# LanceKnight/MolKGNN

Measured on AMD Instinct MI355X. Metric: molecules/sec fwd+bwd, 3-layer MolKGNN on AID 1798, higher is better.
Workload: dtype f32; 1 GPU; AID 1798 full set shape (61832 molecules, ~25 atoms / ~53 directed edges each), 3 layers, hidden_dim 32, kernels 10/20/30/50 per degree, batch 4096 molecules per GPU (102584 atoms), 4 resident batches cycled, fwd+bwd+AdamW, one hipGraph per batch; variant=auto, batch_size_per_gpu=4096, parallelism=dp1

## Files before the change

include/molkgnn_hip.h:

```cpp
#ifndef MOLKGNN_HIP_H
#define MOLKGNN_HIP_H

#include <stddef.h>
#include <stdint.h>

#ifdef __cplusplus
extern "C" {
#endif

#define MKGNN_MAX_DEGREE 4
#define MKGNN_ABI_VERSION 8

#define MKGNN_LOSS_BCE_MEAN 0
#define MKGNN_LOSS_SQERR_MEAN 1
#define MKGNN_LOSS_SQERR_SUM 2

typedef struct mkgnn_kernel_bank {
    int32_t num_kernels;
    int32_t reserved;
    const float* x_center;
    const float* x_support;
    const float* edge_attr_support;
    const float* p_support;
    const float* support_attr_sc_weight;
// ... 14 lines not shown
    int64_t count;
    const int64_t* selected_index;
    const int64_t* nei_index;
    const float* nei_edge_attr;
    const float* p_focal;
    const float* nei_p;
    const float* nei_edge_unit;
} mkgnn_degree_bucket;

typedef struct mkgnn_saved {
    float* pair_state;
    int8_t* chirality;
} mkgnn_saved;

int mkgnn_abi_version(void);
const char* mkgnn_last_error(void);

int mkgnn_row_inv_norm(const float* x, int64_t x_stride, int64_t n_rows, int32_t F,
                       float* inv_norm, void* stream);

int mkgnn_unit_rows8(const float* in, int64_t n_rows, int32_t E, float* out, void* stream);

size_t mkgnn_workspace_bytes(const int32_t num_kernels[MKGNN_MAX_DEGREE], int32_t F, int32_t E,
                             int64_t n_atoms, int64_t n_edges);

#define MKGNN_VARIANT_BLOCK_ROWS 0x100
#define MKGNN_VARIANT_BANK_PREPARED 0x200
#define MKGNN_VARIANT_ROWS_SPLIT 0x400
int mkgnn_rows_presplit(const float* x, int64_t x_stride, int64_t n_rows, int32_t F, float* inv_norm, float* out,
                        int64_t out_stride, void* stream);
int mkgnn_bank_prepare(int32_t count, const mkgnn_kernel_bank* banks, const int32_t* F, int32_t E,
                       void* const* workspaces, const size_t* workspace_bytes, void* stream);
int mkgnn_bank_prepare_deferred(int32_t count, const mkgnn_kernel_bank* banks, const int32_t* F, int32_t E,
                                void* const* workspaces, const size_t* workspace_bytes);
int mkgnn_bank_prepare_flush(void* stream);
int mkgnn_bank_prepare_withdraw(void);
int mkgnn_touch_hint(const void* const* arrays, const size_t* bytes, int32_t count);

int mkgnn_kernelsetconv_forward(const mkgnn_kernel_bank banks[MKGNN_MAX_DEGREE],
                                const mkgnn_degree_bucket buckets[MKGNN_MAX_DEGREE],
                                const float* x, int64_t x_stride, const float* inv_norm,
                                int64_t n_atoms, int32_t F, int32_t E, int32_t is_last_layer,
                                float* out, int64_t out_stride,
                                const mkgnn_saved saved[MKGNN_MAX_DEGREE],
                                void* workspace, size_t workspace_bytes, int32_t variant, void* stream);

#define MKGNN_BACKWARD_DEFER_BANK 0x100
#define MKGNN_BACKWARD_THROUGH_NEIGHBOURS 0x200
#define MKGNN_BACKWARD_ROWS_SPLIT 0x400
int mkgnn_kernelsetconv_backward(const mkgnn_kernel_bank banks[MKGNN_MAX_DEGREE],
                                 const mkgnn_degree_bucket buckets[MKGNN_MAX_DEGREE],
                                 const float* x, int64_t x_stride, const float* inv_norm,
                                 int64_t n_atoms, int32_t F, int32_t E, int32_t is_last_layer,
                                 const float* grad_out, int64_t grad_out_stride,
                                 const mkgnn_saved saved[MKGNN_MAX_DEGREE],
                                 const int32_t* scatter_rowptr, const int32_t* scatter_rows,
                                 float* grad_x, int64_t grad_x_stride,
                                 const mkgnn_kernel_bank_grad grads[MKGNN_MAX_DEGREE],
                                 void* workspace, size_t workspace_bytes, int32_t workspace_from_forward,
                                 int32_t variant, void* stream);

int mkgnn_backward_streams(const mkgnn_kernel_bank banks[MKGNN_MAX_DEGREE],
                           const mkgnn_degree_bucket buckets[MKGNN_MAX_DEGREE],
                           const float* x, int64_t x_stride, int64_t n_atoms, int32_t F, int32_t E);

int mkgnn_rows_split_supported(const mkgnn_kernel_bank banks[MKGNN_MAX_DEGREE],
                               const mkgnn_degree_bucket buckets[MKGNN_MAX_DEGREE],
                               int64_t x_stride, int64_t out_stride, int64_t n_atoms, int32_t F, int32_t E);

int mkgnn_backward_join(void* stream);

int mkgnn_segment_sum_rows(const float* in, int64_t in_stride, const int32_t* rowptr,
                           const int32_t* col, int64_t n_rows, int32_t width,
                           float* out, int64_t out_stride, float* inv_norm, void* stream);

int mkgnn_segment_sum_block_rows(const float* in, int64_t in_stride, const int32_t* rowptr, const int32_t* col,
                                 const int8_t* degree, int64_t n_rows, const int32_t num_kernels[MKGNN_MAX_DEGREE],
                                 int32_t mode, float* out, int64_t out_stride, float* inv_norm, void* stream);

typedef struct mkgnn_readout_params {
    const float* lin1_weight;
    const float* lin1_bias;
    const float* lin2_weight;
    const float* lin2_bias;
    int32_t F, H, G;
} mkgnn_readout_params;

int32_t mkgnn_readout_hidden_stride(int32_t H);
size_t mkgnn_readout_workspace_bytes(int32_t F, int32_t H, int32_t G, int64_t n_atoms, int64_t n_mols);

int mkgnn_readout_forward(const mkgnn_readout_params* params, const float* h, int64_t h_stride,
                          int64_t n_atoms, const int32_t* mol_ptr, int64_t n_mols,
                          const float* keep_scale, float* pre, float* pooled,
                          float* out, int64_t out_stride, void* stream);

int mkgnn_readout_backward(const mkgnn_readout_params* params, const float* h, int64_t h_stride,
                           int64_t n_atoms, const int32_t* mol_ptr, const int32_t* atom_mol, int64_t n_mols,
                           const float* keep_scale, const float* pre, const float* pooled,
                           const float* grad_out, int64_t grad_out_stride,
                           float* grad_h, int64_t grad_h_stride,
                           float* grad_lin1_weight, float* grad_lin1_bias,
                           float* grad_lin2_weight, float* grad_lin2_bias,
                           void* workspace, size_t workspace_bytes, void* stream);

size_t mkgnn_readout_blocks_workspace_bytes(int32_t K, int32_t H, int32_t G, int64_t n_mols);
int mkgnn_readout_blocks_supported(int32_t F, int32_t H, int32_t G, const int32_t num_kernels[MKGNN_MAX_DEGREE]);
int mkgnn_readout_blocks_forward(const mkgnn_readout_params* params, const float* sim, int64_t sim_stride,
                                 const int32_t num_kernels[MKGNN_MAX_DEGREE],
                                 const mkgnn_degree_bucket buckets[MKGNN_MAX_DEGREE], int64_t n_atoms,
                                 const int32_t* in_rowptr, const int32_t* in_col, const int32_t* mol_ptr, int64_t n_mols,
                                 const float* keep_scale, float* z, float* pre, float* pooled, float* gate_sum,
                                 float* out, int64_t out_stride, void* stream);
int mkgnn_readout_blocks_backward(const mkgnn_readout_params* params, const float* sim, int64_t sim_stride,
                                  const int32_t num_kernels[MKGNN_MAX_DEGREE],
                                  const mkgnn_degree_bucket buckets[MKGNN_MAX_DEGREE], int64_t n_atoms,
                                  const int32_t* out_rowptr, const int32_t* out_col, const int32_t* mol_ptr,
                                  const int32_t* atom_mol, int64_t n_mols, const float* gate, const float* gate_sum,
                                  const float* pooled, const float* grad_out, int64_t grad_out_stride,
                                  float* dz, float* grad_sim, int64_t grad_sim_stride,
                                  float* grad_lin1_weight, float* grad_lin1_bias, float* grad_lin2_weight,
                                  float* grad_lin2_bias, void* workspace, size_t workspace_bytes, void* stream);

#define MKGNN_TAIL_MAX_ATOMS 128
#define MKGNN_TAIL_MAX_EDGES 512
typedef struct mkgnn_tail_args {
    const float* sim; int64_t sim_stride;
    int32_t num_kernels[MKGNN_MAX_DEGREE];
    const mkgnn_degree_bucket* buckets;
    const int32_t* in_rowptr; const int32_t* in_col;
    const int32_t* out_rowptr; const int32_t* out_col;
    const int32_t* mol_ptr; const int32_t* atom_mol;
    int64_t n_atoms, n_mols, n_loss_mols;
    mkgnn_readout_params readout;
    const float* head_weight;
    const float* head_bias;
    const float* target;
    float dropout_p;
    int64_t* rng_state; int64_t* rng_used;
    float* emb; int64_t emb_stride;
    float* pred; float* loss;
    float* grad_sim; int64_t grad_sim_stride;
    float *grad_lin1_weight, *grad_lin1_bias, *grad_lin2_weight, *grad_lin2_bias, *grad_head_weight, *grad_head_bias;
    int32_t defer_reduce;
    int32_t loss_kind;
} mkgnn_tail_args;
int mkgnn_tail_supported(int32_t K, int32_t H, int32_t G, const int32_t num_kernels[MKGNN_MAX_DEGREE]);
size_t mkgnn_tail_workspace_bytes(int32_t K, int32_t H, int32_t G, int64_t n_atoms, int64_t n_mols);
int mkgnn_tail_fused(const mkgnn_tail_args* args, void* workspace, size_t workspace_bytes, void* stream);
int mkgnn_tail_fused_readout_dropout(const mkgnn_tail_args* args, float readout_dropout_p, void* workspace, size_t workspace_bytes,
                                     void* stream);
int mkgnn_readout_dropout_mask(const int64_t* rng_pair, int64_t n_rows, int32_t H, float p, float* keep, int64_t keep_stride,
                               void* stream);
int mkgnn_tail_flush(void* stream);
size_t mkgnn_tail_score_workspace_bytes(int32_t K, int32_t H, int32_t G, int64_t n_atoms, int64_t n_mols);
int mkgnn_tail_score(const mkgnn_tail_args* args, void* workspace, size_t workspace_bytes, void* stream);

#define MKGNN_ATOM_CONTRIB_MAX_TASKS 32
typedef struct mkgnn_atom_contrib_args {
    const float* sim; int64_t sim_stride;
    int32_t num_kernels[MKGNN_MAX_DEGREE];
    const mkgnn_degree_bucket* buckets;
    const int32_t* in_rowptr; const int32_t* in_col;
    int64_t n_atoms;
    mkgnn_readout_params readout;
    const float* head_weight; int64_t head_stride; int32_t T;
    float* contrib; int64_t contrib_stride;
} mkgnn_atom_contrib_args;
size_t mkgnn_atom_contributions_workspace_bytes(int32_t K, int32_t H, int32_t G, int64_t n_atoms);
int mkgnn_atom_contributions(const mkgnn_atom_contrib_args* args, void* workspace, size_t workspace_bytes, void* stream);

#define MKGNN_BN_SPLIT_ROWS 2
size_t mkgnn_batchnorm_workspace_bytes(int32_t C);
int mkgnn_batchnorm_forward(const float* x, int64_t x_stride, int64_t n_rows, int32_t C,
                            const float* weight, const float* bias,
                            float* running_mean, float* running_var, float momentum, float eps,
                            int32_t training, float* out, int64_t out_stride,
                            float* save_mean, float* save_invstd, float* inv_norm, int64_t* num_batches_tracked,
                            const int64_t* n_valid_rows, void* workspace, size_t workspace_bytes, void* stream);
typedef struct mkgnn_bn_stats {
    const float* x; int64_t x_stride; int64_t n_rows; int32_t C;
    float* running_mean; float* running_var;
    float momentum;
    int64_t* num_batches_tracked;
    const int64_t* row_key; const int64_t* key_limit;
} mkgnn_bn_stats;
size_t mkgnn_batchnorm_stats_workspace_bytes(int32_t C);
int mkgnn_batchnorm_update_stats(const mkgnn_bn_stats* stats, void* workspace, size_t workspace_bytes, void* stream);
int mkgnn_batchnorm_forward_with_stats(const float* x, int64_t x_stride, int64_t n_rows, int32_t C,
                            const float* weight, const float* bias,
                            float* running_mean, float* running_var, float momentum, float eps,
                            int32_t training, float* out, int64_t out_stride,
                            float* save_mean, float* save_invstd, float* inv_norm, int64_t* num_batches_tracked,
                            const int64_t* n_valid_rows, void* workspace, size_t workspace_bytes,
                            const mkgnn_bn_stats* companion, void* companion_workspace, size_t companion_workspace_bytes,
                            void* stream);
int mkgnn_batchnorm_backward(const float* grad_out, int64_t grad_out_stride, const float* x, int64_t x_stride,
                             int64_t n_rows, int32_t C, const float* weight,
                             const float* save_mean, const float* save_invstd, int32_t training,
                             float* grad_x, int64_t grad_x_stride, float* grad_weight, float* grad_bias,
                             const int64_t* n_valid_rows, void* workspace, size_t workspace_bytes, void* stream);

size_t mkgnn_rf_workspace_bytes(int64_t n_atoms);
int mkgnn_rf_count(const int64_t* edge_index, int64_t n_atoms, int64_t n_edges,
                   void* workspace, size_t workspace_bytes, int64_t* counts, void* stream);
int mkgnn_rf_fill(const int64_t* edge_index, const float* p, const float* edge_attr,
                  int64_t n_atoms, int64_t n_edges, int32_t E, const void* workspace,
                  const mkgnn_degree_bucket out[MKGNN_MAX_DEGREE], void* stream);

size_t mkgnn_plan_workspace_bytes(int64_t n_atoms, int64_t n_edges, int64_t n_rows);

size_t mkgnn_index_workspace_bytes(int64_t n_atoms, int64_t n_edges, int64_t n_rows);
int mkgnn_index_build(const int64_t* edge_index, const float* p, const float* edge_attr, int64_t n_atoms, int64_t n_edges,
                      int32_t E, const mkgnn_degree_bucket out[MKGNN_MAX_DEGREE],
                      int32_t* scatter_rowptr, int32_t* scatter_rows, int32_t* in_rowptr, int32_t* in_col,
                      int32_t* in_col_packed, int32_t* out_rowptr, int32_t* out_col, int8_t* deg8, int64_t* counts,
                      void* workspace, size_t workspace_bytes, void* rf_ready_event, void* stream);

int mkgnn_expand_batch(const int32_t* bond_ij, const uint8_t* bond_attr, int64_t n_bonds, int32_t E,
                       const int32_t* mol_ptr, int64_t n_molecules, int64_t n_atoms,
                       int64_t* edge_index, float* edge_attr, int64_t* batch, int32_t* atom_molecule, void* stream);
int mkgnn_plan_build(const mkgnn_degree_bucket buckets[MKGNN_MAX_DEGREE], int64_t n_atoms, const int64_t* edge_index,
                     int64_t n_edges, int32_t* scatter_rowptr, int32_t* scatter_rows, int32_t* in_rowptr, int32_t* in_col,
                     int32_t* in_col_packed, int32_t* out_rowptr, int32_t* out_col, int8_t* deg8, void* workspace,
                     size_t workspace_bytes, void* stream);

size_t mkgnn_bce_head_workspace_bytes(int64_t n_rows, int32_t H);
int mkgnn_bce_head_forward(const float* emb, int64_t emb_stride, int64_t n_rows, int32_t H,
                           const float* weight, const float* bias, const float* target,
                           float* pred, float* loss, void* workspace, size_t workspace_bytes, void* stream);
int mkgnn_bce_head_backward(const float* emb, int64_t emb_stride, int64_t n_rows, int32_t H,
                            const float* weight, const float* target, const float* pred, const float* grad_loss,
                            float* grad_emb, int64_t grad_emb_stride, float* grad_weight, float* grad_bias,
                            void* workspace, size_t workspace_bytes, void* stream);

int mkgnn_bce_head_dropout_forward(const float* emb, int64_t emb_stride, int64_t n_rows, int32_t H,
                                   const float* weight, const float* bias, const float* target, float dropout_p,
                                   int64_t* rng_state, int64_t* rng_used, float* pred, float* loss,
                                   void* workspace, size_t workspace_bytes, void* stream);
int mkgnn_bce_head_dropout_backward(const float* emb, int64_t emb_stride, int64_t n_rows, int32_t H,
                                    const float* weight, const float* target, const float* pred,
                                    const float* grad_loss, float dropout_p, const int64_t* rng_used,
                                    float* grad_emb, int64_t grad_emb_stride, float* grad_weight, float* grad_bias,
                                    void* workspace, size_t workspace_bytes, void* stream);

int mkgnn_bce_head_fused(const float* emb, int64_t emb_stride, int64_t n_rows, int32_t H,
                         const float* weight, const float* bias, const float* target, float dropout_p,
                         int64_t* rng_state, int64_t* rng_used, float* pred, float* loss,
                         float* grad_emb, int64_t grad_emb_stride, float* grad_weight, float* grad_bias,
                         void* workspace, size_t workspace_bytes, void* stream);

int mkgnn_head_loss_forward(int32_t loss_kind, const float* emb, int64_t emb_stride, int64_t n_rows, int32_t H,
                            const float* weight, const float* bias, const float* target,
                            float* pred, float* loss, void* workspace, size_t workspace_bytes, void* stream);
int mkgnn_head_loss_backward(int32_t loss_kind, const float* emb, int64_t emb_stride, int64_t n_rows, int32_t H,
                             const float* weight, const float* target, const float* pred, const float* grad_loss,
                             float* grad_emb, int64_t grad_emb_stride, float* grad_weight, float* grad_bias,
                             void* workspace, size_t workspace_bytes, void* stream);
int mkgnn_head_loss_dropout_forward(int32_t loss_kind, const float* emb, int64_t emb_stride, int64_t n_rows, int32_t H,
                                    const float* weight, const float* bias, const float* target, float dropout_p,
                                    int64_t* rng_state, int64_t* rng_used, float* pred, float* loss,
                                    void* workspace, size_t workspace_bytes, void* stream);
int mkgnn_head_loss_dropout_backward(int32_t loss_kind, const float* emb, int64_t emb_stride, int64_t n_rows, int32_t H,
                                     const float* weight, const float* target, const float* pred,
                                     const float* grad_loss, float dropout_p, const int64_t* rng_used,
                                     float* grad_emb, int64_t grad_emb_stride, float* grad_weight, float* grad_bias,
                                     void* workspace, size_t workspace_bytes, void* stream);
int mkgnn_head_loss_fused(int32_t loss_kind, const float* emb, int64_t emb_stride, int64_t n_rows, int32_t H,
                          const float* weight, const float* bias, const float* target, float dropout_p,
                          int64_t* rng_state, int64_t* rng_used, float* pred, float* loss,
                          float* grad_emb, int64_t grad_emb_stride, float* grad_weight, float* grad_bias,
                          void* workspace, size_t workspace_bytes, void* stream);

#define MKGNN_TASK_HEAD_MAX_TASKS 32
size_t mkgnn_task_head_workspace_bytes(int64_t n_rows, int32_t H, int32_t T);
int mkgnn_task_head_forward(int32_t loss_kind, const float* emb, int64_t emb_stride, int64_t n_rows, int32_t H, int32_t T,
                            const float* weight, const float* bias, const float* target, const int32_t* task,
                            const int32_t* row_ids, int64_t n_task, float dropout_p, int64_t* rng_state, int64_t* rng_used,
                            float* pred, float* loss, void* workspace, size_t workspace_bytes, void* stream);
int mkgnn_task_head_backward(int32_t loss_kind, const float* emb, int64_t emb_stride, int64_t n_rows, int32_t H, int32_t T,
                             const float* weight, const float* target, const int32_t* task, const int32_t* row_ids,
                             int64_t n_task, const float* pred, const float* grad_loss, float dropout_p,
                             const int64_t* rng_used, float* grad_emb, int64_t grad_emb_stride, float* grad_weight,
                             float* grad_bias, void* workspace, size_t workspace_bytes, void* stream);
int mkgnn_task_head_fused(int32_t loss_kind, const float* emb, int64_t emb_stride, int64_t n_rows, int32_t H, int32_t T,
                          const float* weight, const float* bias, const float* target, const int32_t* task,
                          const int32_t* row_ids, int64_t n_task, float dropout_p, int64_t* rng_state, int64_t* rng_used,
                          float* pred, float* loss, float* grad_emb, int64_t grad_emb_stride, float* grad_weight,
                          float* grad_bias, void* workspace, size_t workspace_bytes, void* stream);

int mkgnn_task_scores(const float* emb, int64_t emb_stride, int64_t n_rows, int32_t H, int32_t T,
                      const float* weight, const float* bias, float* pred, int64_t pred_row_stride, int64_t pred_task_stride,
                      void* stream);

#define MKGNN_EMBED_COSINE_MAX_QUERIES 32
int mkgnn_embed_cosine(const float* emb, int64_t emb_stride, int64_t n_rows, int32_t H, const float* queries, int64_t query_stride,
                       int32_t Q, float* sim, int64_t sim_row_stride, int64_t sim_query_stride, void* stream);

typedef struct mkgnn_copy_item { float* dst; const float* src; int64_t numel; } mkgnn_copy_item;
int mkgnn_flat_copy(const mkgnn_copy_item* items, int32_t n_items, void* stream);

typedef struct mkgnn_adamw_tensor {
    float* param;
    const float* grad;
    float* state;
    int64_t numel;
    int32_t group;
// ... 150 lines not shown
```

molkgnn_amd/_lib.py:

```python
from __future__ import annotations

import ctypes as C
import os
from typing import Optional, Sequence

import torch

_HERE = os.path.dirname(os.path.abspath(__file__))
LIB_PATH = os.environ.get("MKGNN_LIB") or os.path.join(_HERE, "libmolkgnn_hip.so")
MAX_DEGREE = 4
ABI_VERSION = 8
LOSS_BCE_MEAN, LOSS_SQERR_MEAN, LOSS_SQERR_SUM = 0, 1, 2
TASK_HEAD_MAX_TASKS, TASK_HEAD_MAX_H = 32, 64
EMBED_COSINE_MAX_QUERIES, EMBED_COSINE_MAX_H = 32, 64
MAX_COSINE_MAX_REFS, MAX_COSINE_MAX_H = 1 << 20, 64
MAX_COSINE_ROWS, MAX_COSINE_TILE, MAX_COSINE_MAX_PARTS, MAX_COSINE_TARGET_BLOCKS = 128, 32, 256, 2048
SELECT_ROWS_PASS = 1024


def max_cosine_split(n_rows: int, R: int):
    row_blocks = -(-int(n_rows) // MAX_COSINE_ROWS)
    tiles = -(-int(R) // MAX_COSINE_TILE)
    want = min(-(-MAX_COSINE_TARGET_BLOCKS // row_blocks), tiles, MAX_COSINE_MAX_PARTS)
    per_part = -(-tiles // want)
# ... 3 lines not shown
class KernelBank(C.Structure):
    _fields_ = [("num_kernels", C.c_int32), ("reserved", C.c_int32),
                ("x_center", C.c_void_p), ("x_support", C.c_void_p),
                ("edge_attr_support", C.c_void_p), ("p_support", C.c_void_p),
                ("support_attr_sc_weight", C.c_void_p), ("center_attr_sc_weight", C.c_void_p),
                ("edge_attr_support_sc_weight", C.c_void_p)]


class KernelBankGrad(C.Structure):
    _fields_ = [("x_center", C.c_void_p), ("x_support", C.c_void_p), ("edge_attr_support", C.c_void_p),
                ("support_attr_sc_weight", C.c_void_p), ("center_attr_sc_weight", C.c_void_p),
                ("edge_attr_support_sc_weight", C.c_void_p)]


class DegreeBucket(C.Structure):
    _fields_ = [("count", C.c_int64), ("selected_index", C.c_void_p), ("nei_index", C.c_void_p),
                ("nei_edge_attr", C.c_void_p), ("p_focal", C.c_void_p), ("nei_p", C.c_void_p), ("nei_edge_unit", C.c_void_p)]


class Saved(C.Structure):
    _fields_ = [("pair_state", C.c_void_p), ("chirality", C.c_void_p)]


class ReadoutParams(C.Structure):
    _fields_ = [("lin1_weight", C.c_void_p), ("lin1_bias", C.c_void_p), ("lin2_weight", C.c_void_p),
                ("lin2_bias", C.c_void_p), ("F", C.c_int32), ("H", C.c_int32), ("G", C.c_int32)]


class TailArgs(C.Structure):
    _fields_ = [("sim", C.c_void_p), ("sim_stride", C.c_int64), ("num_kernels", C.c_int32 * 4), ("buckets", C.c_void_p),
                ("in_rowptr", C.c_void_p), ("in_col", C.c_void_p), ("out_rowptr", C.c_void_p), ("out_col", C.c_void_p),
                ("mol_ptr", C.c_void_p), ("atom_mol", C.c_void_p), ("n_atoms", C.c_int64), ("n_mols", C.c_int64),
                ("n_loss_mols", C.c_int64), ("readout", ReadoutParams), ("head_weight", C.c_void_p), ("head_bias", C.c_void_p),
                ("target", C.c_void_p), ("dropout_p", C.c_float), ("rng_state", C.c_void_p), ("rng_used", C.c_void_p),
                ("emb", C.c_void_p), ("emb_stride", C.c_int64), ("pred", C.c_void_p), ("loss", C.c_void_p),
                ("grad_sim", C.c_void_p), ("grad_sim_stride", C.c_int64), ("grad_lin1_weight", C.c_void_p),
                ("grad_lin1_bias", C.c_void_p), ("grad_lin2_weight", C.c_void_p), ("grad_lin2_bias", C.c_void_p),
                ("grad_head_weight", C.c_void_p), ("grad_head_bias", C.c_void_p), ("defer_reduce", C.c_int32),
                ("loss_kind", C.c_int32)]


TAIL_MAX_ATOMS, TAIL_MAX_EDGES = 128, 512
ATOM_CONTRIB_MAX_TASKS = 32


class AtomContribArgs(C.Structure):
    _fields_ = [("sim", C.c_void_p), ("sim_stride", C.c_int64), ("num_kernels", C.c_int32 * 4), ("buckets", C.c_void_p),
                ("in_rowptr", C.c_void_p), ("in_col", C.c_void_p), ("n_atoms", C.c_int64), ("readout", ReadoutParams),
                ("head_weight", C.c_void_p), ("head_stride", C.c_int64), ("T", C.c_int32), ("contrib", C.c_void_p),
                ("contrib_stride", C.c_int64)]


class CopyItem(C.Structure):
    _fields_ = [("dst", C.c_void_p), ("src", C.c_void_p), ("numel", C.c_int64)]


class AdamWTensor(C.Structure):
    _fields_ = [("param", C.c_void_p), ("grad", C.c_void_p), ("state", C.c_void_p), ("numel", C.c_int64),
                ("group", C.c_int32), ("reserved", C.c_int32), ("active", C.c_void_p)]


class AdamWGroup(C.Structure):
    _fields_ = [("lr_device", C.c_void_p), ("lr", C.c_float), ("beta1", C.c_float), ("beta2", C.c_float),
                ("eps", C.c_float), ("weight_decay", C.c_float), ("maximize", C.c_int32), ("grad_scale", C.c_float)]


class ShardView(C.Structure):
    _fields_ = [("x", C.c_void_p), ("p", C.c_void_p), ("edge_src", C.c_void_p), ("edge_dst", C.c_void_p),
                ("edge_attr", C.c_void_p), ("y", C.c_void_p), ("mol_atom_ptr", C.c_void_p), ("mol_edge_ptr", C.c_void_p),
                ("mol_deg_ptr", C.c_void_p), ("n_molecules", C.c_int64), ("x_dim", C.c_int32), ("p_dim", C.c_int32),
                ("e_dim", C.c_int32), ("reserved", C.c_int32)]


class ResidentShardView(C.Structure):
    _fields_ = [("x", C.c_void_p), ("p", C.c_void_p), ("bond_ij", C.c_void_p), ("bond_attr", C.c_void_p), ("y", C.c_void_p),
                ("mol_atom_ptr", C.c_void_p), ("mol_bond_ptr", C.c_void_p), ("mol_deg", C.c_void_p), ("n_molecules", C.c_int64),
                ("x_dim", C.c_int32), ("p_dim", C.c_int32), ("e_dim", C.c_int32), ("reserved", C.c_int32)]


class ResidentShardPackedView(C.Structure):
    _fields_ = [("x_rec", C.c_void_p), ("x_col", C.c_void_p), ("p", C.c_void_p), ("bond_ij", C.c_void_p), ("bond_attr", C.c_void_p),
                ("y", C.c_void_p), ("mol_atom_ptr", C.c_void_p), ("mol_bond_ptr", C.c_void_p), ("mol_deg", C.c_void_p),
                ("n_molecules", C.c_int64), ("x_dim", C.c_int32), ("p_dim", C.c_int32), ("e_dim", C.c_int32), ("rec_bytes", C.c_int32)]


PACKED_MAX_X_DIM = 160
TOPK_MAX_K = 1024
GATHER_BAD_ID, GATHER_MISFIT = 1, 2
Int64x6 = C.c_int64 * 6
Banks4 = KernelBank * MAX_DEGREE
BankGrads4 = KernelBankGrad * MAX_DEGREE
Buckets4 = DegreeBucket * MAX_DEGREE
Saved4 = Saved * MAX_DEGREE
Int32x4 = C.c_int32 * MAX_DEGREE

MOLECULE_MAX_LAYERS = 4
MOLECULE_MAX_ATOMS = 64
MOLECULE_MAX_MOLS = 16
MOLECULE_HEAD, MOLECULE_BACKWARD, MOLECULE_GRAD_EMB, MOLECULE_SQERR, MOLECULE_SUM = 1, 2, 4, 8, 16
MOLECULE_READOUT_DROPOUT = 32


class MoleculeLayer(C.Structure):
    _fields_ = [("bank", Banks4), ("grad", BankGrads4), ("saved", Saved4), ("F", C.c_int32), ("reserved", C.c_int32),
                ("sim_out", C.c_void_p), ("sim_stride", C.c_int64)]


class BnStats(C.Structure):
    _fields_ = [("x", C.c_void_p), ("x_stride", C.c_int64), ("n_rows", C.c_int64), ("C", C.c_int32),
                ("running_mean", C.c_void_p), ("running_var", C.c_void_p), ("momentum", C.c_float),
                ("num_batches_tracked", C.c_void_p), ("row_key", C.c_void_p), ("key_limit", C.c_void_p)]


class MoleculeNet(C.Structure):
    _fields_ = [("num_layers", C.c_int32), ("E", C.c_int32), ("layer", MoleculeLayer * MOLECULE_MAX_LAYERS),
                ("bn_weight", C.c_void_p), ("bn_bias", C.c_void_p), ("bn_running_mean", C.c_void_p),
                ("bn_running_var", C.c_void_p), ("bn_num_batches_tracked", C.c_void_p),
                ("bn_eps", C.c_float), ("bn_momentum", C.c_float), ("bn_training", C.c_int32), ("reserved", C.c_int32),
                ("grad_bn_weight", C.c_void_p), ("grad_bn_bias", C.c_void_p),
                ("readout", ReadoutParams),
                ("grad_lin1_weight", C.c_void_p), ("grad_lin1_bias", C.c_void_p), ("grad_lin2_weight", C.c_void_p),
                ("grad_lin2_bias", C.c_void_p),
                ("ffn_weight", C.c_void_p), ("ffn_bias", C.c_void_p), ("grad_ffn_weight", C.c_void_p),
                ("grad_ffn_bias", C.c_void_p), ("head_dropout", C.c_float), ("readout_dropout", C.c_float),
                ("rng_state", C.c_void_p), ("rng_used", C.c_void_p), ("edge_stats", C.POINTER(BnStats))]


class MoleculeBatch(C.Structure):
    _fields_ = [("n_atoms", C.c_int64), ("n_mols", C.c_int64), ("n_chunks", C.c_int64), ("max_chunk_atoms", C.c_int64),
                ("chunk_mol_ptr", C.c_void_p), ("mol_atom_ptr", C.c_void_p), ("atom_degree", C.c_void_p),
                ("atom_rank", C.c_void_p), ("buckets", Buckets4), ("x", C.c_void_p), ("x_stride", C.c_int64)]


EXPORTS = ("mkgnn_abi_version", "mkgnn_last_error", "mkgnn_row_inv_norm", "mkgnn_unit_rows8", "mkgnn_workspace_bytes",
           "mkgnn_kernelsetconv_forward", "mkgnn_kernelsetconv_backward", "mkgnn_segment_sum_rows",
           "mkgnn_readout_hidden_stride", "mkgnn_readout_workspace_bytes", "mkgnn_readout_forward",
           "mkgnn_readout_backward", "mkgnn_batchnorm_workspace_bytes", "mkgnn_batchnorm_forward",
           "mkgnn_batchnorm_backward", "mkgnn_bce_head_workspace_bytes", "mkgnn_bce_head_forward",
           "mkgnn_bce_head_backward", "mkgnn_rf_workspace_bytes", "mkgnn_rf_count", "mkgnn_rf_fill", "mkgnn_adamw_step", "mkgnn_adamw_state_floats",
           "mkgnn_bce_head_dropout_forward", "mkgnn_bce_head_dropout_backward", "mkgnn_segment_sum_block_rows",
           "mkgnn_plan_workspace_bytes", "mkgnn_plan_build", "mkgnn_backward_join", "mkgnn_backward_streams", "mkgnn_bank_prepare", "mkgnn_bank_prepare_deferred", "mkgnn_bank_prepare_flush", "mkgnn_bank_prepare_withdraw", "mkgnn_touch_hint", "mkgnn_expand_batch", "mkgnn_bce_head_fused", "mkgnn_collate_compact", "mkgnn_collate_compact_bytes",
           "mkgnn_readout_blocks_supported", "mkgnn_readout_blocks_forward", "mkgnn_readout_blocks_backward",
           "mkgnn_readout_blocks_workspace_bytes", "mkgnn_molecule_supported", "mkgnn_molecule_workspace_bytes",
           "mkgnn_molecule_step", "mkgnn_batchnorm_stats_workspace_bytes", "mkgnn_batchnorm_update_stats",
           "mkgnn_batchnorm_forward_with_stats", "mkgnn_index_workspace_bytes", "mkgnn_index_build",
           "mkgnn_rows_split_supported", "mkgnn_rows_presplit", "mkgnn_tail_supported", "mkgnn_tail_workspace_bytes", "mkgnn_tail_fused", "mkgnn_tail_flush", "mkgnn_flat_copy",
           "mkgnn_tail_fused_readout_dropout", "mkgnn_readout_dropout_mask", "mkgnn_tail_score", "mkgnn_tail_score_workspace_bytes",
           "mkgnn_head_loss_forward", "mkgnn_head_loss_backward", "mkgnn_head_loss_dropout_forward",
           "mkgnn_head_loss_dropout_backward", "mkgnn_head_loss_fused", "mkgnn_gather_compact",
           "mkgnn_gather_compact_workspace_bytes", "mkgnn_gather_compact_packed", "mkgnn_topk_update", "mkgnn_topk_workspace_bytes",
           "mkgnn_task_head_workspace_bytes", "mkgnn_task_head_forward", "mkgnn_task_head_backward", "mkgnn_task_head_fused",
           "mkgnn_task_scores", "mkgnn_topk_tasks_workspace_bytes", "mkgnn_topk_update_tasks", "mkgnn_embed_cosine",
           "mkgnn_atom_contributions", "mkgnn_atom_contributions_workspace_bytes", "mkgnn_embed_max_cosine",
           "mkgnn_embed_max_cosine_workspace_bytes", "mkgnn_select_rows")

_lib: Optional[C.CDLL] = None
TORCH_LIB_PATH = os.path.join(os.path.dirname(LIB_PATH), "libmolkgnn_torch.so")
_torch_ops_loaded = False


def load_torch_ops():
    global _torch_ops_loaded
    import torch
    if not _torch_ops_loaded:
        load()
        if not os.path.exists(TORCH_LIB_PATH):
            raise MolKGNNLibraryError(f"{TORCH_LIB_PATH} is missing: build it with `make -C molkgnn_amd/csrc torch`")
        torch.ops.load_library(TORCH_LIB_PATH)
        if int(torch.ops.molkgnn.abi_version()) != ABI_VERSION:
            raise MolKGNNLibraryError("libmolkgnn_torch.so was built against another ABI version")
        _torch_ops_loaded = True
    return torch.ops.molkgnn


class MolKGNNLibraryError(RuntimeError):
    pass


def load() -> C.CDLL:
    global _lib
    if _lib is not None:
        return _lib
    if not os.path.exists(LIB_PATH):
        raise MolKGNNLibraryError(
            f"{LIB_PATH} is missing: build it with `make -C molkgnn_amd/csrc` "
            "(python -c 'import __graft_entry__ as g; g.build()'). There is no fallback path.")
    lib = C.CDLL(LIB_PATH)
    for name in EXPORTS:
        if not hasattr(lib, name):
            raise MolKGNNLibraryError(f"{LIB_PATH} does not export {name}")
    lib.mkgnn_abi_version.restype = C.c_int
    lib.mkgnn_last_error.restype = C.c_char_p
    lib.mkgnn_row_inv_norm.restype = C.c_int
    lib.mkgnn_row_inv_norm.argtypes = [C.c_void_p, C.c_int64, C.c_int64, C.c_int32, C.c_void_p, C.c_void_p]
    lib.mkgnn_unit_rows8.restype = C.c_int
    lib.mkgnn_unit_rows8.argtypes = [C.c_void_p, C.c_int64, C.c_int32, C.c_void_p, C.c_void_p]
    lib.mkgnn_workspace_bytes.restype = C.c_size_t
    lib.mkgnn_workspace_bytes.argtypes = [Int32x4, C.c_int32, C.c_int32, C.c_int64, C.c_int64]
    lib.mkgnn_kernelsetconv_forward.restype = C.c_int
    lib.mkgnn_kernelsetconv_forward.argtypes = [
        Banks4, Buckets4, C.c_void_p, C.c_int64, C.c_void_p, C.c_int64, C.c_int32, C.c_int32, C.c_int32,
        C.c_void_p, C.c_int64, Saved4, C.c_void_p, C.c_size_t, C.c_int32, C.c_void_p]
    lib.mkgnn_kernelsetconv_backward.restype = C.c_int
    lib.mkgnn_kernelsetconv_backward.argtypes = [
        Banks4, Buckets4, C.c_void_p, C.c_int64, C.c_void_p, C.c_int64, C.c_int32, C.c_int32, C.c_int32,
        C.c_void_p, C.c_int64, Saved4, C.c_void_p, C.c_void_p, C.c_void_p, C.c_int64, BankGrads4,
        C.c_void_p, C.c_size_t, C.c_int32, C.c_int32, C.c_void_p]
    lib.mkgnn_backward_streams.restype = C.c_int
    lib.mkgnn_backward_streams.argtypes = [Banks4, Buckets4, C.c_void_p, C.c_int64, C.c_int64, C.c_int32, C.c_int32]
    lib.mkgnn_tail_supported.restype = C.c_int
    lib.mkgnn_tail_supported.argtypes = [C.c_int32, C.c_int32, C.c_int32, Int32x4]
    lib.mkgnn_tail_workspace_bytes.restype = C.c_size_t
    lib.mkgnn_tail_workspace_bytes.argtypes = [C.c_int32, C.c_int32, C.c_int32, C.c_int64, C.c_int64]
    lib.mkgnn_tail_fused.restype = C.c_int
    lib.mkgnn_tail_fused.argtypes = [C.POINTER(TailArgs), C.c_void_p, C.c_size_t, C.c_void_p]
    lib.mkgnn_tail_score_workspace_bytes.restype = C.c_size_t
    lib.mkgnn_tail_score_workspace_bytes.argtypes = [C.c_int32, C.c_int32, C.c_int32, C.c_int64, C.c_int64]
    lib.mkgnn_tail_score.restype = C.c_int
    lib.mkgnn_tail_score.argtypes = [C.POINTER(TailArgs), C.c_void_p, C.c_size_t, C.c_void_p]
    lib.mkgnn_atom_contributions_workspace_bytes.restype = C.c_size_t
    lib.mkgnn_atom_contributions_workspace_bytes.argtypes = [C.c_int32, C.c_int32, C.c_int32, C.c_int64]
    lib.mkgnn_atom_contributions.restype = C.c_int
    lib.mkgnn_atom_contributions.argtypes = [C.POINTER(AtomContribArgs), C.c_void_p, C.c_size_t, C.c_void_p]
    lib.mkgnn_tail_fused_readout_dropout.restype = C.c_int
    lib.mkgnn_tail_fused_readout_dropout.argtypes = [C.POINTER(TailArgs), C.c_float, C.c_void_p, C.c_size_t, C.c_void_p]
    lib.mkgnn_readout_dropout_mask.restype = C.c_int
    lib.mkgnn_readout_dropout_mask.argtypes = [C.c_void_p, C.c_int64, C.c_int32, C.c_float, C.c_void_p, C.c_int64, C.c_void_p]
    lib.mkgnn_flat_copy.restype = C.c_int
    lib.mkgnn_flat_copy.argtypes = [C.c_void_p, C.c_int32, C.c_void_p]
    lib.mkgnn_tail_flush.restype = C.c_int
    lib.mkgnn_tail_flush.argtypes = [C.c_void_p]
    lib.mkgnn_rows_presplit.restype = C.c_int
    lib.mkgnn_rows_presplit.argtypes = [C.c_void_p, C.c_int64, C.c_int64, C.c_int32, C.c_void_p, C.c_void_p, C.c_int64, C.c_void_p]
    lib.mkgnn_rows_split_supported.restype = C.c_int
    lib.mkgnn_rows_split_supported.argtypes = [Banks4, Buckets4, C.c_int64, C.c_int64, C.c_int64, C.c_int32, C.c_int32]
    lib.mkgnn_bank_prepare.restype = C.c_int
    lib.mkgnn_bank_prepare.argtypes = [C.c_int32, C.c_void_p, C.c_void_p, C.c_int32, C.c_void_p, C.c_void_p, C.c_void_p]
    lib.mkgnn_bank_prepare_deferred.restype = C.c_int
    lib.mkgnn_bank_prepare_deferred.argtypes = [C.c_int32, C.c_void_p, C.c_void_p, C.c_int32, C.c_void_p, C.c_void_p]
    lib.mkgnn_bank_prepare_flush.restype = C.c_int
    lib.mkgnn_bank_prepare_flush.argtypes = [C.c_void_p]
    lib.mkgnn_bank_prepare_withdraw.restype = C.c_int
    lib.mkgnn_bank_prepare_withdraw.argtypes = []
    lib.mkgnn_touch_hint.restype = C.c_int
    lib.mkgnn_touch_hint.argtypes = [C.c_void_p, C.c_void_p, C.c_int32]
    lib.mkgnn_collate_compact_bytes.restype = C.c_size_t
    lib.mkgnn_collate_compact_bytes.argtypes = [Int64x6, C.c_int64, C.c_int32, C.c_int32, C.c_int32, C.c_int32]
    lib.mkgnn_collate_compact.restype = C.c_int
    lib.mkgnn_collate_compact.argtypes = [C.POINTER(ShardView), C.c_int64, C.c_int64, Int64x6, C.c_int32, C.c_void_p, C.c_size_t]
    lib.mkgnn_gather_compact_workspace_bytes.restype = C.c_size_t
    lib.mkgnn_gather_compact_workspace_bytes.argtypes = [C.c_int64]
    lib.mkgnn_gather_compact.restype = C.c_int
    lib.mkgnn_gather_compact.argtypes = [C.POINTER(ResidentShardView), C.c_void_p, C.c_int64, Int64x6, C.c_int32, C.c_void_p,
                                         C.c_size_t, C.c_void_p, C.c_void_p]
    lib.mkgnn_gather_compact_packed.restype = C.c_int
    lib.mkgnn_gather_compact_packed.argtypes = [C.POINTER(ResidentShardPackedView), C.c_void_p, C.c_int64, Int64x6, C.c_int32,
                                                C.c_void_p, C.c_size_t, C.c_void_p, C.c_void_p]
    lib.mkgnn_topk_workspace_bytes.restype = C.c_size_t
    lib.mkgnn_topk_workspace_bytes.argtypes = [C.c_int32, C.c_int32]
    lib.mkgnn_topk_update.restype = C.c_int
    lib.mkgnn_topk_update.argtypes = [C.c_void_p, C.c_void_p, C.c_int32, C.c_void_p, C.c_void_p, C.c_int32, C.c_void_p, C.c_void_p,
                                      C.c_void_p, C.c_void_p, C.c_size_t, C.c_void_p]
    lib.mkgnn_topk_tasks_workspace_bytes.restype = C.c_size_t
    lib.mkgnn_topk_tasks_workspace_bytes.argtypes = [C.c_int32, C.c_int32, C.c_int32]
    lib.mkgnn_topk_update_tasks.restype = C.c_int
    lib.mkgnn_topk_update_tasks.argtypes = [C.c_void_p, C.c_int64, C.c_int64, C.c_void_p, C.c_int32, C.c_int32, C.c_void_p, C.c_void_p,
                                            C.c_int32, C.c_void_p, C.c_void_p, C.c_void_p, C.c_void_p, C.c_size_t, C.c_void_p]
    lib.mkgnn_expand_batch.restype = C.c_int
    lib.mkgnn_expand_batch.argtypes = [C.c_void_p, C.c_void_p, C.c_int64, C.c_int32, C.c_void_p, C.c_int64, C.c_int64,
                                       C.c_void_p, C.c_void_p, C.c_void_p, C.c_void_p, C.c_void_p]
    lib.mkgnn_backward_join.restype = C.c_int
    lib.mkgnn_backward_join.argtypes = [C.c_void_p]
    lib.mkgnn_segment_sum_rows.restype = C.c_int
    lib.mkgnn_segment_sum_rows.argtypes = [C.c_void_p, C.c_int64, C.c_void_p, C.c_void_p, C.c_int64, C.c_int32,
                                           C.c_void_p, C.c_int64, C.c_void_p, C.c_void_p]
    P, I64, I32, F32 = C.c_void_p, C.c_int64, C.c_int32, C.c_float
    lib.mkgnn_readout_hidden_stride.restype = I32
    lib.mkgnn_readout_hidden_stride.argtypes = [I32]
    lib.mkgnn_readout_workspace_bytes.restype = C.c_size_t
    lib.mkgnn_readout_workspace_bytes.argtypes = [I32, I32, I32, I64, I64]
    lib.mkgnn_readout_forward.restype = C.c_int
    lib.mkgnn_readout_forward.argtypes = [C.POINTER(ReadoutParams), P, I64, I64, P, I64, P, P, P, P, I64, P]
    lib.mkgnn_readout_backward.restype = C.c_int
    lib.mkgnn_readout_backward.argtypes = [C.POINTER(ReadoutParams), P, I64, I64, P, P, I64, P, P, P, P, I64, P, I64,
                                           P, P, P, P, P, C.c_size_t, P]
    lib.mkgnn_readout_blocks_workspace_bytes.restype = C.c_size_t
    lib.mkgnn_readout_blocks_workspace_bytes.argtypes = [I32, I32, I32, I64]
    lib.mkgnn_readout_blocks_supported.restype = C.c_int
    lib.mkgnn_readout_blocks_supported.argtypes = [I32, I32, I32, Int32x4]
    lib.mkgnn_readout_blocks_forward.restype = C.c_int
    lib.mkgnn_readout_blocks_forward.argtypes = [C.POINTER(ReadoutParams), P, I64, Int32x4, Buckets4, I64, P, P, P, I64, P, P, P, P, P, P, I64, P]
    lib.mkgnn_readout_blocks_backward.restype = C.c_int
    lib.mkgnn_readout_blocks_backward.argtypes = [C.POINTER(ReadoutParams), P, I64, Int32x4, Buckets4, I64, P, P, P, P, I64, P, P, P,
                                                  P, I64, P, P, I64, P, P, P, P, P, C.c_size_t, P]
    lib.mkgnn_batchnorm_workspace_bytes.restype = C.c_size_t
    lib.mkgnn_batchnorm_workspace_bytes.argtypes = [I32]
    lib.mkgnn_batchnorm_forward.restype = C.c_int
    lib.mkgnn_batchnorm_forward.argtypes = [P, I64, I64, I32, P, P, P, P, F32, F32, I32, P, I64, P, P, P, P, P, P, C.c_size_t, P]
    lib.mkgnn_batchnorm_stats_workspace_bytes.restype = C.c_size_t
    lib.mkgnn_batchnorm_stats_workspace_bytes.argtypes = [I32]
    lib.mkgnn_batchnorm_update_stats.restype = C.c_int
    lib.mkgnn_batchnorm_update_stats.argtypes = [C.POINTER(BnStats), P, C.c_size_t, P]
    lib.mkgnn_batchnorm_forward_with_stats.restype = C.c_int
    lib.mkgnn_batchnorm_forward_with_stats.argtypes = [P, I64, I64, I32, P, P, P, P, F32, F32, I32, P, I64, P, P, P, P, P, P, C.c_size_t,
                                                       C.POINTER(BnStats), P, C.c_size_t, P]
    lib.mkgnn_batchnorm_backward.restype = C.c_int
    lib.mkgnn_batchnorm_backward.argtypes = [P, I64, P, I64, I64, I32, P, P, P, I32, P, I64, P, P, P, P, C.c_size_t, P]
    lib.mkgnn_bce_head_forward.restype = C.c_int
    lib.mkgnn_bce_head_forward.argtypes = [P, I64, I64, I32, P, P, P, P, P, P, C.c_size_t, P]
    lib.mkgnn_bce_head_backward.restype = C.c_int
    lib.mkgnn_bce_head_backward.argtypes = [P, I64, I64, I32, P, P, P, P, P, I64, P, P, P, C.c_size_t, P]
    lib.mkgnn_bce_head_dropout_forward.restype = C.c_int
    lib.mkgnn_bce_head_dropout_forward.argtypes = [P, I64, I64, I32, P, P, P, C.c_float, P, P, P, P, P, C.c_size_t, P]
    lib.mkgnn_bce_head_dropout_backward.restype = C.c_int
    lib.mkgnn_bce_head_dropout_backward.argtypes = [P, I64, I64, I32, P, P, P, P, C.c_float, P, P, I64, P, P, P, C.c_size_t, P]
    lib.mkgnn_bce_head_fused.restype = C.c_int
    lib.mkgnn_bce_head_fused.argtypes = [P, I64, I64, I32, P, P, P, C.c_float, P, P, P, P, P, I64, P, P, P, C.c_size_t, P]
    for name, args in (("mkgnn_head_loss_forward", lib.mkgnn_bce_head_forward.argtypes),
                       ("mkgnn_head_loss_backward", lib.mkgnn_bce_head_backward.argtypes),
                       ("mkgnn_head_loss_dropout_forward", lib.mkgnn_bce_head_dropout_forward.argtypes),
                       ("mkgnn_head_loss_dropout_backward", lib.mkgnn_bce_head_dropout_backward.argtypes),
                       ("mkgnn_head_loss_fused", lib.mkgnn_bce_head_fused.argtypes)):
        getattr(lib, name).restype = C.c_int
        getattr(lib, name).argtypes = [I32] + list(args)
    lib.mkgnn_bce_head_workspace_bytes.restype = C.c_size_t
    lib.mkgnn_bce_head_workspace_bytes.argtypes = [I64, I32]
    lib.mkgnn_task_head_workspace_bytes.restype = C.c_size_t
    lib.mkgnn_task_head_workspace_bytes.argtypes = [I64, I32, I32]
    lib.mkgnn_task_head_forward.restype = C.c_int
    lib.mkgnn_task_head_forward.argtypes = [I32, P, I64, I64, I32, I32, P, P, P, P, P, I64, C.c_float, P, P, P, P, P, C.c_size_t, P]
    lib.mkgnn_task_head_backward.restype = C.c_int
    lib.mkgnn_task_head_backward.argtypes = [I32, P, I64, I64, I32, I32, P, P, P, P, I64, P, P, C.c_float, P, P, I64, P, P, P,
                                             C.c_size_t, P]
    lib.mkgnn_task_head_fused.restype = C.c_int
    lib.mkgnn_task_head_fused.argtypes = [I32, P, I64, I64, I32, I32, P, P, P, P, P, I64, C.c_float, P, P, P, P, P, I64, P, P, P,
                                          C.c_size_t, P]
    lib.mkgnn_task_scores.restype = C.c_int
    lib.mkgnn_task_scores.argtypes = [P, I64, I64, I32, I32, P, P, P, I64, I64, P]
    lib.mkgnn_embed_cosine.restype = C.c_int
    lib.mkgnn_embed_cosine.argtypes = [P, I64, I64, I32, P, I64, I32, P, I64, I64, P]
    lib.mkgnn_embed_max_cosine_workspace_bytes.restype = C.c_size_t
    lib.mkgnn_embed_max_cosine_workspace_bytes.argtypes = [I64, I32]
    lib.mkgnn_embed_max_cosine.restype = C.c_int
    lib.mkgnn_embed_max_cosine.argtypes = [P, I64, I64, I32, P, I64, I32, P, P, P, C.c_size_t, P]
    lib.mkgnn_select_rows.restype = C.c_int
    lib.mkgnn_select_rows.argtypes = [P, P, P, I32, P, P, P, P, P, P]
    lib.mkgnn_rf_workspace_bytes.restype = C.c_size_t
    lib.mkgnn_rf_workspace_bytes.argtypes = [I64]
    lib.mkgnn_rf_count.restype = C.c_int
    lib.mkgnn_rf_count.argtypes = [P, I64, I64, P, C.c_size_t, P, P]
    lib.mkgnn_rf_fill.restype = C.c_int
    lib.mkgnn_rf_fill.argtypes = [P, P, P, I64, I64, I32, P, Buckets4, P]
    lib.mkgnn_segment_sum_block_rows.restype = C.c_int
    lib.mkgnn_segment_sum_block_rows.argtypes = [P, I64, P, P, P, I64, Int32x4, I32, P, I64, P, P]
    lib.mkgnn_plan_workspace_bytes.restype = C.c_size_t
    lib.mkgnn_plan_workspace_bytes.argtypes = [I64, I64, I64]
    lib.mkgnn_plan_build.restype = C.c_int
    lib.mkgnn_plan_build.argtypes = [Buckets4, I64, P, I64, P, P, P, P, P, P, P, P, P, C.c_size_t, P]
    lib.mkgnn_index_workspace_bytes.restype = C.c_size_t
    lib.mkgnn_index_workspace_bytes.argtypes = [I64, I64, I64]
    lib.mkgnn_index_build.restype = C.c_int
    lib.mkgnn_index_build.argtypes = [P, P, P, I64, I64, I32, Buckets4, P, P, P, P, P, P, P, P, P, P, C.c_size_t, P, P]
    lib.mkgnn_adamw_step.restype = C.c_int
    lib.mkgnn_adamw_state_floats.restype = C.c_int64
    lib.mkgnn_adamw_state_floats.argtypes = [I64]
    lib.mkgnn_adamw_step.argtypes = [P, I32, P, I32, P]
    lib.mkgnn_molecule_supported.restype = C.c_int
    lib.mkgnn_molecule_supported.argtypes = [C.POINTER(MoleculeNet), I32]
    lib.mkgnn_molecule_workspace_bytes.restype = C.c_size_t
    lib.mkgnn_molecule_workspace_bytes.argtypes = [C.POINTER(MoleculeNet), I32, I64, I64]
    lib.mkgnn_molecule_step.restype = C.c_int
    lib.mkgnn_molecule_step.argtypes = [C.POINTER(MoleculeNet), C.POINTER(MoleculeBatch), I32, P, P, P, P, P, P, C.c_size_t, P]
    if lib.mkgnn_abi_version() != ABI_VERSION:
        raise MolKGNNLibraryError(f"ABI version {lib.mkgnn_abi_version()} != {ABI_VERSION}: rebuild the library")
    _lib = lib
    return lib


def check(rc: int, what: str) -> None:
    if rc != 0:
        msg = load().mkgnn_last_error()
        raise MolKGNNLibraryError(f"{what}: {msg.decode() if msg else 'error'}")


# ... 13 lines not shown
```

molkgnn_amd/csrc/kgnn_bwd_stream.hip:

```cpp
#include <stdio.h>
#include <stdlib.h>
#include <string.h>

#include <type_traits>

#include "kgnn_launch.h"
#include "kgnn_split.h"

namespace mkgnn {

typedef float f32x4 __attribute__((ext_vector_type(4)));

#ifdef MKGNN_BWD_STAMPS
__device__ unsigned long long* g_bank_stream_stamps = nullptr;
#define MKGNN_BPHASE(i) do { __builtin_amdgcn_sched_barrier(0); const unsigned long long t_ = __builtin_readcyclecounter(); phase[i] += t_ - t_phase; t_phase = t_; __builtin_amdgcn_sched_barrier(0); } while (0)
#else
#define MKGNN_BPHASE(i) do { } while (0)
#endif

namespace bs {

template <int I> using IC = std::integral_constant<int, I>;
template <int B, int E, typename Fn> __device__ __forceinline__ void static_for(Fn&& fn) {
    if constexpr (B < E) { fn(IC<B>{}); static_for<B + 1, E>(fn); }
}
template <int N> __device__ __forceinline__ void wait_vmcnt() {
    static_assert(N >= 0 && N <= 63, "s_waitcnt vmcnt is a 6-bit field");
    asm volatile("s_waitcnt vmcnt(%0)" ::"n"(N) : "memory");
}
#define MKGNN_DMA_CASE(SZ, O) else if constexpr (OFF == O) __builtin_amdgcn_global_load_lds(g, l, SZ, O, 0)
template <int OFF> __device__ __forceinline__ void dma16(const void* src, float* lds_wave_base) {
    const auto g = (const __attribute__((address_space(1))) void*)((const char*)src - OFF);
    const auto l = (__attribute__((address_space(3))) void*)((char*)lds_wave_base - OFF);
    if constexpr (OFF == 0) __builtin_amdgcn_global_load_lds(g, l, 16, 0, 0);
    MKGNN_DMA_CASE(16, 16); MKGNN_DMA_CASE(16, 32); MKGNN_DMA_CASE(16, 48);
    else static_assert(OFF < 0, "add the offset to the list");
}
template <int OFF> __device__ __forceinline__ void dma4(const void* src, float* lds_wave_base) {
    const auto g = (const __attribute__((address_space(1))) void*)((const char*)src - OFF);
    const auto l = (__attribute__((address_space(3))) void*)((char*)lds_wave_base - OFF);
    if constexpr (OFF == 0) __builtin_amdgcn_global_load_lds(g, l, 4, 0, 0);
    MKGNN_DMA_CASE(4, 4); MKGNN_DMA_CASE(4, 8); MKGNN_DMA_CASE(4, 12);
    else static_assert(OFF < 0, "add the offset to the list");
}
constexpr int SITE_ROWS = 0, SITE_BONDS = 16, SITE_COEF_G = 32, SITE_COEF_I = 48;
constexpr int SITE_IDS = 0, SITE_IDS4 = 4, SITE_INV = 8, SITE_INV4 = 12;
__device__ __forceinline__ float lds_read_raw(uint32_t byte_addr) {
    float v;
    asm volatile("ds_read_b32 %0, %1" : "=v"(v) : "v"(byte_addr) : "memory");
    return v;
}
template <int OFF> __device__ __forceinline__ float lds_read_raw_at(uint32_t byte_addr) {
    static_assert(OFF >= 0 && OFF < 65536, "ds_read offset field");
    float v;
    asm volatile("ds_read_b32 %0, %1 offset:%2" : "=v"(v) : "v"(byte_addr), "n"(OFF) : "memory");
    return v;
}

template <int OFF> __device__ __forceinline__ void lds_read_h16(uint32_t& dst, uint32_t byte_addr) {
    static_assert(OFF >= 0 && OFF < 65536, "ds_read offset field");
    asm volatile("ds_read_u16 %0, %1 offset:%2" : "=v"(dst) : "v"(byte_addr), "n"(OFF) : "memory");
}

template <typename V> __device__ __forceinline__ void lds_fence(V& v) { asm volatile("s_waitcnt lgkmcnt(0)" : "+v"(v) : : "memory"); }

template <int D, int A> __device__ __forceinline__ int perm_entry(int p) {
    if constexpr (D == 1) return 0;
    else {
        constexpr uint32_t packed = [] {
            uint32_t v = 0;
            for (int q = 0; q < PermC<D>::P; ++q) v |= (uint32_t)PermC<D>::t[q][A] << (2 * q);
            return v;
        }();
        return (int)((packed >> (2 * p)) & 3u);
    }
}

template <int D> struct Traits {
    static constexpr int NS = (D == 1) ? 1 : (D == 4 ? 4 : 2);
    static constexpr int NSTREAM = 4 / NS;
    static constexpr int RING = (D == 1) ? 2 : (D == 2 ? 3 : (D == 3 ? 4 : 5));
    static constexpr int S1 = D + 1;
    static constexpr int OFF_INV = 16 * S1, OFF_BOND = 32 * S1, META = OFF_BOND + 128 * D;
    static constexpr int COEF = 512;
};

__host__ __device__ constexpr int lds_floats(int D, int KC) {
    const int NS = (D == 1) ? 1 : (D == 4 ? 4 : 2);
    const int RING = (D == 1) ? 2 : (D == 2 ? 3 : (D == 3 ? 4 : 5));
    const int META = 32 * (D + 1) + 128 * D;
    const int FPC = 4 * KC;
    return (4 / NS) * (RING * 16 * FPC * 4 + 2 * META) + 4 * 512;
}

template <int KC, int NS> constexpr int pieces_of(int role) { return (KC - role + NS - 1) / NS; }

template <int D, int KC> constexpr int batch_size(int sd, int role) {
    using T = Traits<D>;
    int n = pieces_of<KC, T::NS>(role);
    if (sd == 0) n += 2;
    if (role == 0) {
        if (sd < D) n += 1;
        if (sd == 0) n += 2 * (T::S1 == 5 ? 2 : 1);
    }
    return n;
}
template <int D, int KC> constexpr int young_batches(int s, int role) {
    using T = Traits<D>;
    int n = 0;
    for (int j = 1; j <= T::RING - 2; ++j) n += batch_size<D, KC>((s + 64 * T::S1 - j + T::RING) % T::S1, role);
    return n;
}

}

typedef unsigned short pk_u16 __attribute__((ext_vector_type(2)));
#ifndef MKGNN_PREP_RPB
#define MKGNN_PREP_RPB 4
#endif
constexpr int PREP_RPB = MKGNN_PREP_RPB;
template <int NSRC, bool CH>
__device__ __forceinline__ void coef_prepare_body(const BankStreamArgs& a, const int di) {
    const BankStreamDeg& g = a.deg[di];
    const int tid = threadIdx.x;
    const int64_t blk = (int64_t)blockIdx.x - g.prep_blk0;
    const int64_t nrec = ((g.n + 15) / 16) * g.nct;
    const int atom = tid >> 4, k = tid & 15;
    const float w_s = g.mix[0], w_c = g.mix[1], w_e = g.mix[2], w_sum = g.mix[3];
    const int8_t* chp = g.chir ? g.chir : (const int8_t*)g.pair;
    float gv[PREP_RPB], S[PREP_RPB], C[PREP_RPB], Ed[PREP_RPB];
    int idx[PREP_RPB], ch[PREP_RPB];
    bool ok[PREP_RPB];
    const int D = di + 1;
    constexpr int nsrc = NSRC;
    int64_t src[PREP_RPB][NSRC];
#pragma unroll
    for (int r = 0; r < PREP_RPB; ++r) {
        const int64_t rec = blk * PREP_RPB + r;
        const int64_t rc = rec < nrec ? rec : nrec - 1;
        const int64_t tile = rc / g.nct;
        const int ct = (int)(rc - tile * g.nct);
        const int64_t n = tile * 16 + atom;
        const int64_t nc = n < g.n ? n : g.n - 1;
        const int l = ct * g.kpt + k;
        ok[r] = rec < nrec && n < g.n && k < g.kpt && l < g.L;
#pragma unroll
        for (int s = 0; s < NSRC; ++s) src[r][s] = a.through_nei ? g.nei[nc * D + s] : g.sel[nc];
    }
#pragma unroll
    for (int r = 0; r < PREP_RPB; ++r) {
        const int64_t rec = blk * PREP_RPB + r;
        const int64_t rc = rec < nrec ? rec : nrec - 1;
        const int64_t tile = rc / g.nct;
        const int ct = (int)(rc - tile * g.nct);
        const int64_t n = tile * 16 + atom;
        const int64_t nc = n < g.n ? n : g.n - 1;
        const int l = ct * g.kpt + k, lc = l < g.L ? l : g.L - 1;
        const size_t o = (size_t)nc * g.L + lc;
        float gs4[NSRC];
#pragma unroll
        for (int s = 0; s < NSRC; ++s) gs4[s] = a.gout[src[r][s] * a.gs + g.off + lc];
        gv[r] = gs4[0];
#pragma unroll
        for (int s = 1; s < NSRC; ++s) gv[r] += gs4[s];
        const mkgnn_f32x4 pr = pair_load(g.pair, o);
        idx[r] = pair_index(pr);
        ch[r] = CH ? (int)chp[o] : 1;
        S[r] = pr[0]; C[r] = pr[1]; Ed[r] = pr[2];
    }
    float p0 = 0.f, p1 = 0.f, p2 = 0.f;
    constexpr int NEM = (PREP_RPB + 1) / 2;
    pk_u16 em[NEM];
#pragma unroll
    for (int i = 0; i < NEM; ++i) em[i] = pk_u16{0, 0};
#pragma unroll
    for (int r = 0; r < PREP_RPB; ++r) {
        const int64_t rec = blk * PREP_RPB + r;
        float gg = ok[r] ? (CH ? gv[r] * (float)ch[r] : gv[r]) : 0.f;
        if (rec < nrec) {
            float* out = g.coefq + (size_t)rec * 512;
            out[tid] = gg;
        }
        const unsigned short eb = (unsigned short)((__float_as_uint(gg) >> 23) & 0xffu);
        em[r >> 1][r & 1] = eb;
        if (ok[r]) {
            const float sc = (S[r] * w_s + C[r] * w_c + Ed[r] * w_e) / w_sum;
            p0 = fmaf(gg * (w_s / w_sum), S[r] - sc, p0);
            p1 = fmaf(gg * (w_c / w_sum), C[r] - sc, p1);
            p2 = fmaf(gg * (w_e / w_sum), Ed[r] - sc, p2);
        }
    }
    __shared__ float red[3][4];
    __shared__ uint32_t emx[NEM][4][16];
    p0 = wave_sum(p0); p1 = wave_sum(p1); p2 = wave_sum(p2);
#pragma unroll
    for (int o = 32; o >= 16; o >>= 1)
#pragma unroll
        for (int i = 0; i < NEM; ++i)
            em[i] = __builtin_elementwise_max(em[i], __builtin_bit_cast(pk_u16, __shfl_xor(__builtin_bit_cast(uint32_t, em[i]), o, 64)));
    if ((tid & 63) == 0) { red[0][tid >> 6] = p0; red[1][tid >> 6] = p1; red[2][tid >> 6] = p2; }
    if ((tid & 63) < 16) {
#pragma unroll
        for (int i = 0; i < NEM; ++i) emx[i][tid >> 6][tid & 15] = __builtin_bit_cast(uint32_t, em[i]);
    }
    __syncthreads();
    {
        pk_u16 mx[NEM];
#pragma unroll
        for (int i = 0; i < NEM; ++i) {
            mx[i] = __builtin_bit_cast(pk_u16, emx[i][0][k]);
#pragma unroll
            for (int w = 1; w < 4; ++w) mx[i] = __builtin_elementwise_max(mx[i], __builtin_bit_cast(pk_u16, emx[i][w][k]));
        }
#pragma unroll
        for (int r = 0; r < PREP_RPB; ++r) {
            const int64_t rec = blk * PREP_RPB + r;
            const int me = mx[r >> 1][r & 1];
            if (rec < nrec) ((int*)(g.coefq + (size_t)rec * 512))[256 + tid] = (ok[r] ? idx[r] : 0) | (me << 8);
        }
    }
    if (tid < 3) g.theta_slab[(size_t)blk * 4 + tid] = (red[tid][0] + red[tid][1]) + (red[tid][2] + red[tid][3]);
}

__global__ void __launch_bounds__(256) coef_prepare_kernel(BankStreamArgs a) {
    int di = 0;
#pragma unroll
    for (int k = 1; k < 4; ++k) if (a.deg[k].prep_blocks > 0 && (int)blockIdx.x >= a.deg[k].prep_blk0) di = k;
    const int nsrc = a.through_nei ? di + 1 : 1;
    if (a.deg[di].chir) {
        switch (nsrc) {
            case 1: coef_prepare_body<1, true>(a, di); break;
            case 2: coef_prepare_body<2, true>(a, di); break;
            case 3: coef_prepare_body<3, true>(a, di); break;
            default: coef_prepare_body<4, true>(a, di); break;
        }
        return;
    }
    switch (nsrc) {
        case 1: coef_prepare_body<1, false>(a, di); break;
        case 2: coef_prepare_body<2, false>(a, di); break;
        case 3: coef_prepare_body<3, false>(a, di); break;
        default: coef_prepare_body<4, false>(a, di); break;
    }
}

constexpr int BANK_COEF_EXP = 18;
template <int D, int KC, int SP>
__device__ __forceinline__ void bank_stream_body(const BankStreamArgs& a, const BankStreamDeg& dg, const int cp, const int rank,
                                                 const int count, float* lds) {
    using namespace bs;
    using T = Traits<D>;
    constexpr int NS = T::NS, NSTREAM = T::NSTREAM, RING = T::RING, S1 = T::S1, META = T::META;
    constexpr int FPC = 4 * KC;
    constexpr bool SWZ = (KC % 2 == 0);
    constexpr int RF = 4 * FPC;
    constexpr int SLOT = 16 * RF;
    constexpr int NP = SLOT / 256;
    static_assert(NP == KC, "piece count");
    constexpr bool HS = (D == 4);
    constexpr int NBS = HS ? 2 : D;
    const int tid = threadIdx.x, lane = tid & 63;
    const int wave = __builtin_amdgcn_readfirstlane(tid >> 6);
    const int stream = wave / NS, role = wave % NS;
    const int half = HS ? (role & 1) : 0;
    const int ct = HS ? cp * 2 + (role >> 1) : cp * NS + role;
    const bool ct_ok = ct < dg.nct;
    const int ctc = ct_ok ? ct : dg.nct - 1;
    const int ci = lane & 15, kq = lane >> 4;
    const int L = dg.L, kpt = dg.kpt;
    float* const ring = lds + (size_t)stream * (RING * SLOT + 2 * META);
    float* const meta = ring + RING * SLOT;
    float* const cbuf = lds + (size_t)NSTREAM * (RING * SLOT + 2 * META) + (size_t)wave * T::COEF;

    const int64_t ntiles = (dg.n + 15) / 16;
    const int64_t nstreams = (int64_t)count * NSTREAM;
    const int64_t sg = (int64_t)rank * NSTREAM + stream;
    const int64_t tile_first = sg * ntiles / nstreams;
    const int64_t tile_end = (sg + 1) * ntiles / nstreams;
    const int64_t iters = (ntiles + nstreams - 1) / nstreams;
    const int64_t tile_hi = (tile_end > tile_first ? tile_end : (tile_first + 1 < ntiles ? tile_first + 1 : ntiles)) - 1;
    auto tile_at = [&](int64_t i) -> int64_t {
        const int64_t t = tile_first + i;
        return t > tile_hi ? tile_hi : t;
    };
    const float w_s = dg.mix[0], w_c = dg.mix[1], w_e = dg.mix[2], w_sum = dg.mix[3];
    const float ws_n = w_s / w_sum / (float)D, wc_n = w_c / w_sum, we_n = w_e / w_sum / (float)D;
    const uint32_t xs = (uint32_t)a.xs;
    const int F = a.F;

    auto issue_rows = [&](auto sdc, const float* drec, float* buf) {
        constexpr int sd = decltype(sdc)::value;
        const uint32_t ids_b = (uint32_t)(uintptr_t)(drec + 16 * sd);
        static_for<0, NS>([&](auto rc) {
            constexpr int r = decltype(rc)::value;
            constexpr int NMINE = pieces_of<KC, NS>(r);
            if constexpr (NMINE > 0) if (role == r) {
                uint32_t id[NMINE];
                int cc[NMINE];
                static_for<0, NMINE>([&](auto kc) {
                    constexpr int k = decltype(kc)::value;
                    const int g = 64 * (r + NS * k) + lane;
                    const int row = g / FPC;
                    int c = g - row * FPC;
                    if constexpr (SWZ) c ^= (row & 1) * 4;
                    cc[k] = c;
                    id[k] = __float_as_uint(lds_read_raw(ids_b + 4u * row));
                });
                static_for<0, NMINE>([&](auto kc) { lds_fence(id[decltype(kc)::value]); });
                static_for<0, NMINE>([&](auto kc) {
                    constexpr int k = decltype(kc)::value;
                    dma16<SITE_ROWS>(a.x + (id[k] * xs + (4 * cc[k] < F ? 4u * cc[k] : 0u)), buf + (r + NS * k) * 256);
                });
            }
        });
    };
    auto issue_bonds = [&](int64_t t, int sd, float* mrec) {
        if (lane < 32) {
            int64_t n = t * 16 + (lane >> 1);
            if (n >= dg.n) n = dg.n - 1;
            dma16<SITE_BONDS>(dg.e_unit + ((uint32_t)(n * D + sd) * 8u + 4u * (lane & 1)), mrec + T::OFF_BOND + sd * 128);
        }
    };
    auto issue_ids = [&](int64_t t, float* mrec) {
        int64_t n = t * 16 + ci;
        if (n >= dg.n) n = dg.n - 1;
        const void* src = (kq < D) ? (const void*)(dg.nei + n * D + kq) : (const void*)(dg.sel + n);
        if (S1 >= 4 || kq < S1) dma4<SITE_IDS>(src, mrec);
        if constexpr (S1 == 5) {
            if (kq == 0) dma4<SITE_IDS4>(dg.sel + n, mrec + 64);
        }
    };
    auto issue_inv = [&](float* mrec) {
        const uint32_t rec_b = (uint32_t)(uintptr_t)mrec;
        uint32_t idq = __float_as_uint(lds_read_raw(rec_b + 4u * (16 * ((S1 >= 4 || kq < S1) ? kq : 0) + ci)));
        [[maybe_unused]] uint32_t id4 = 0;
        if constexpr (S1 == 5) id4 = __float_as_uint(lds_read_raw(rec_b + 4u * (64 + ci)));
        lds_fence(idq);
        if constexpr (S1 == 5) lds_fence(id4);
        if (S1 >= 4 || kq < S1) dma4<SITE_INV>(a.inv + idq, mrec + T::OFF_INV);
        if constexpr (S1 == 5) {
            if (kq == 0) dma4<SITE_INV4>(a.inv + id4, mrec + T::OFF_INV + 64);
        }
    };
    auto issue_coef = [&](int64_t t, float* cb) {
        const float* src = dg.coefq + ((size_t)(t * dg.nct + ctc) * 512 + 4 * lane);
        dma16<SITE_COEF_G>(src, cb);
        dma16<SITE_COEF_I>(src + 256, cb + 256);
    };

    f32x4 acc[NBS][KC];
    f32x4 accC[KC];
    f32x4 accE[NBS];
#pragma unroll
    for (int t = 0; t < KC; ++t) {
        accC[t] = f32x4{0.f, 0.f, 0.f, 0.f};
#pragma unroll
        for (int b = 0; b < NBS; ++b) acc[b][t] = f32x4{0.f, 0.f, 0.f, 0.f};
    }
#pragma unroll
    for (int b = 0; b < NBS; ++b) accE[b] = f32x4{0.f, 0.f, 0.f, 0.f};

    [[maybe_unused]] float G = __uint_as_float(230u << 23);
    [[maybe_unused]] const int wexp = (int)((__float_as_uint(fmaxf(fabsf(ws_n), fabsf(wc_n))) >> 23) & 0xffu) + 1 - 127;

    if (role == 0) issue_ids(tile_at(0), meta);
    wait_vmcnt<0>();
    __syncthreads();
    static_for<0, RING>([&](auto kc) {
        constexpr int k = decltype(kc)::value;
        issue_rows(kc, meta, ring + k * SLOT);
        if (role == 0 && k < D) issue_bonds(tile_at(0), k, meta);
    });
    issue_coef(tile_at(0), cbuf);
    if (role == 0) {
        issue_inv(meta);
        issue_ids(tile_at(1), meta + META);
    }
    wait_vmcnt<0>();
    __builtin_amdgcn_s_barrier();

    int buf = 0;
#ifdef MKGNN_BWD_STAMPS
    const unsigned long long t_start = __builtin_readcyclecounter();
    unsigned long long phase[8] = {0, 0, 0, 0, 0, 0, 0, 0}, t_phase = t_start;
#endif
    for (int64_t it = 0; it < iters; ++it) {
        const bool real = tile_first + it < tile_end;
        const uint32_t mrec_b = (uint32_t)(uintptr_t)(meta + (it & 1) * META);
        const uint32_t cb_b = (uint32_t)(uintptr_t)cbuf;
        float gq[4];
        int iq[4];
        [[maybe_unused]] int rec_exp = 0;
        {
            float raw[8];
            const uint32_t cl_b = cb_b + 4u * (kq * 16 + ci);
            static_for<0, 4>([&](auto qc) {
// ... 127 lines not shown
                        xb.lo = __builtin_bit_cast(h16x4, u32x2{hx[4] | (hx[5] << 16), hx[6] | (hx[7] << 16)});
                        if constexpr (s < D) {
#pragma unroll
                            for (int b = 0; b < NBS; ++b) acc[b][t] = __builtin_amdgcn_mfma_f32_16x16x16f16(avs[b].lo, xb.hi, acc[b][t], 0, 0, 0);
#pragma unroll
                            for (int b = 0; b < NBS; ++b) acc[b][t] = __builtin_amdgcn_mfma_f32_16x16x16f16(avs[b].hi, xb.lo, acc[b][t], 0, 0, 0);
#pragma unroll
                            for (int b = 0; b < NBS; ++b) acc[b][t] = __builtin_amdgcn_mfma_f32_16x16x16f16(avs[b].hi, xb.hi, acc[b][t], 0, 0, 0);
                        } else {
                            accC[t] = split_mfma(avs[0], xb, accC[t]);
                        }
                    });
                } else if constexpr (SP) {
                    float bxp[2][4];
                    read_bx(IC<0>{}, bxp[0]);
                    static_for<0, KC>([&](auto tc) {
                        constexpr int t = decltype(tc)::value;
                        float (&bx)[4] = bxp[t & 1];
                        asm volatile("s_waitcnt lgkmcnt(0)" : "+v"(bx[0]), "+v"(bx[1]), "+v"(bx[2]), "+v"(bx[3]) : : "memory");
                        if constexpr (t + 1 < KC) read_bx(IC<t + 1>{}, bxp[(t + 1) & 1]);
                        const SplitReg xb = split_scaled(f32x4{bx[0], bx[1], bx[2], bx[3]}, rsc);
                        if constexpr (s < D) {
#pragma unroll
                            for (int b = 0; b < NBS; ++b) acc[b][t] = __builtin_amdgcn_mfma_f32_16x16x16f16(avs[b].lo, xb.hi, acc[b][t], 0, 0, 0);
#pragma unroll
                            for (int b = 0; b < NBS; ++b) acc[b][t] = __builtin_amdgcn_mfma_f32_16x16x16f16(avs[b].hi, xb.lo, acc[b][t], 0, 0, 0);
#pragma unroll
                            for (int b = 0; b < NBS; ++b) acc[b][t] = __builtin_amdgcn_mfma_f32_16x16x16f16(avs[b].hi, xb.hi, acc[b][t], 0, 0, 0);
                        } else {
                            accC[t] = split_mfma(avs[0], xb, accC[t]);
                        }
                    });
                } else {
                    static_for<0, KC>([&](auto tc) {
                        constexpr int t = decltype(tc)::value;
                        float bx[4];
                        read_bx(tc, bx);
                        asm volatile("s_waitcnt lgkmcnt(0)" : "+v"(bx[0]), "+v"(bx[1]), "+v"(bx[2]), "+v"(bx[3]) : : "memory");
                        if constexpr (s < D) {
#pragma unroll
                            for (int b = 0; b < NBS; ++b)
#pragma unroll
                                for (int q = 0; q < 4; ++q) acc[b][t] = __builtin_amdgcn_mfma_f32_16x16x4f32(av[b][q], bx[q], acc[b][t], 0, 0, 0);
                        } else {
#pragma unroll
                            for (int q = 0; q < 4; ++q) accC[t] = __builtin_amdgcn_mfma_f32_16x16x4f32(ac[q], bx[q], accC[t], 0, 0, 0);
                        }
                    });
                }
            }
            MKGNN_BPHASE(2);
            if constexpr (RING == 2) {
                wait_vmcnt<0>();
            } else {
                static_for<0, NS>([&](auto rc) {
                    constexpr int r = decltype(rc)::value;
                    constexpr int n_young = young_batches<D, KC>(s, r);
                    if (role == r) wait_vmcnt<n_young>();
                });
            }
            MKGNN_BPHASE(3);
            if constexpr (NS > 1) __builtin_amdgcn_s_barrier();
            MKGNN_BPHASE(4);
            constexpr int sd = (s + RING) % S1;
            const int64_t itd = it + (s + RING) / S1;
            float* const drec = meta + (itd & 1) * META;
            issue_rows(IC<sd>{}, drec, ring + buf * SLOT);
            if constexpr (sd == 0) issue_coef(tile_at(itd), cbuf);
            if (role == 0) {
                if constexpr (sd < D) issue_bonds(tile_at(itd), sd, drec);
                if constexpr (sd == 0) {
                    issue_inv(drec);
                    issue_ids(tile_at(itd + 1), meta + ((itd + 1) & 1) * META);
                }
            }
            buf = (buf + 1 == RING) ? 0 : buf + 1;
            MKGNN_BPHASE(5);
        });
    }
    wait_vmcnt<0>();
    MKGNN_BPHASE(3);

    if constexpr (SP) {
        const float ug_col = split_unscale_of<0>(G);
        float ug[4];
#pragma unroll
        for (int r = 0; r < 4; ++r) ug[r] = __shfl(ug_col, 4 * kq + r, 64);
#pragma unroll
        for (int t = 0; t < KC; ++t)
#pragma unroll
            for (int r = 0; r < 4; ++r) {
                accC[t][r] *= ug[r];
#pragma unroll
                for (int b = 0; b < NBS; ++b) acc[b][t][r] *= ug[r];
            }
    }
    float* const slab = dg.slab + (size_t)sg * bank_floats(D, L, F, a.E);
    const size_t o_sup = (size_t)L * F, o_edg = o_sup + (size_t)L * D * F;
#pragma unroll
    for (int r = 0; r < 4; ++r) {
        const int i = kq * 4 + r, l = ct * kpt + i;
        if (ct_ok && i < kpt && l < L) {
#pragma unroll
            for (int t = 0; t < KC; ++t) {
                const int f = 16 * t + ci;
                if (f < F) {
                    if (!HS || half == 0) slab[(size_t)l * F + f] = accC[t][r];
#pragma unroll
                    for (int b = 0; b < NBS; ++b) slab[o_sup + (size_t)(l * D + (HS ? 2 * half + b : b)) * F + f] = acc[b][t][r];
                }
            }
            if (ci < a.E) {
#pragma unroll
                for (int b = 0; b < NBS; ++b) slab[o_edg + (size_t)(l * D + (HS ? 2 * half + b : b)) * a.E + ci] = accE[b][r];
            }
        }
    }
#ifdef MKGNN_BWD_STAMPS
    MKGNN_BPHASE(6);
    if (g_bank_stream_stamps && lane == 0) {
        unsigned long long* o = g_bank_stream_stamps + ((size_t)blockIdx.x * 4 + wave) * 16;
        o[0] = t_start; o[1] = __builtin_readcyclecounter(); o[2] = (unsigned long long)(D * 16 + cp); o[3] = (unsigned long long)iters;
        for (int i = 0; i < 8; ++i) o[4 + i] = phase[i];
    }
#endif
}

template <int KC, int SP = 0>
__global__ void __launch_bounds__(256, (KC >= 8 ? 1 : 2)) kc_backward_bank_stream(BankStreamArgs a) {
    extern __shared__ __align__(16) float lds[];
    const int grp = a.blk_group[blockIdx.x];
    const int rank = a.blk_rank[blockIdx.x];
    const int di = a.grp_degree[grp];
    const int cp = a.grp_cp[grp];
    const int count = a.grp_count[grp];
    switch (di) {
        case 0: bank_stream_body<1, KC, SP>(a, a.deg[0], cp, rank, count, lds); break;
        case 1: bank_stream_body<2, KC, SP>(a, a.deg[1], cp, rank, count, lds); break;
        case 2: bank_stream_body<3, KC, SP>(a, a.deg[2], cp, rank, count, lds); break;
        default: bank_stream_body<4, KC, SP>(a, a.deg[3], cp, rank, count, lds); break;
    }
}

extern "C" int mkgnn_debug_set_bank_stream_stamps(void* device_ptr) {
#ifdef MKGNN_BWD_STAMPS
    return (int)hipMemcpyToSymbol(HIP_SYMBOL(g_bank_stream_stamps), &device_ptr, sizeof(void*));
#else
    (void)device_ptr;
    return -1;
#endif
}

bool bank_stream_rows_split_supported(int F) { return (F + 15) / 16 <= 7 && bwd_split_mode() != 0; }
bool bank_stream_supported(int d, int F, int E, int L, int64_t n_atoms, int64_t x_stride, const float* e_unit) {
    return stream_forward_supported(d, F, E, L, n_atoms, x_stride, x_stride, e_unit);
}

void plan_backward_bank_stream(const BwdArgs a4[4], const bool use[4], const float* const e_unit[4], float* const coefq[4],
                               int nchunk_out[4], int ntheta_out[4], bool through_nei, BankStreamLaunch* out) {
    BankStreamArgs& a = out->a;
    memset(out, 0, sizeof(*out));
    int KC = 0, ng = 0, prep_blocks = 0;
    constexpr int MG = FUSED_MAX_GROUPS;
    double cost[MG];
    int64_t tiles_of[MG], cap[MG];
    int nstream_of[MG], deg_of[MG];
    size_t lds_fl = 0;
    for (int i = 0; i < 4; ++i) {
        nchunk_out[i] = 0; ntheta_out[i] = 0;
        if (!use[i]) continue;
        const BwdArgs& s = a4[i];
        const int d = i + 1;
        a.x = s.x; a.xs = s.xs; a.inv = s.inv; a.gout = s.gout; a.gs = s.gs; a.F = s.F; a.E = s.E;
        a.through_nei = through_nei ? 1 : 0;
        KC = (s.F + 15) / 16;
        BankStreamDeg& g = a.deg[i];
        g.sel = s.sel; g.nei = s.nei; g.e_unit = e_unit[i]; g.pair = s.pair; g.chir = s.chir; g.mix = s.mix;
        g.coefq = coefq[i]; g.slab = s.slab; g.theta_slab = s.theta_slab;
        g.n = s.n; g.L = s.L; g.off = s.off;
        g.nct = (s.L + 15) / 16;
        g.kpt = (s.L + g.nct - 1) / g.nct;
        g.cs = stream_column_parts(d, s.L);
        const int64_t ntiles = (s.n + 15) / 16;
        g.prep_blk0 = prep_blocks;
        g.prep_blocks = (int)((ntiles * g.nct + PREP_RPB - 1) / PREP_RPB);
        prep_blocks += g.prep_blocks;
        ntheta_out[i] = g.prep_blocks;
        const int nstream = d == 1 ? 4 : (d == 4 ? 1 : 2);
        const size_t fl = (size_t)bs::lds_floats(d, KC);
        if (fl > lds_fl) lds_fl = fl;
        for (int cp = 0; cp < g.cs; ++cp) {
            const int nbs = d == 4 ? 2 : d;
            cost[ng] = (d * nbs + 1) * 4.0 * KC + 4.0 * d * nbs + 12.0 * d + 60.0;
            if (KC <= 7 && bwd_split_mode() != 0) {
                static const double sp7[4] = {196.0, 317.0, 503.0, 535.0}, sp2[4] = {126.0, 193.0, 298.0, 338.0};
                cost[ng] = sp2[i] + (sp7[i] - sp2[i]) * (KC - 2) / 5.0;
            }
            tiles_of[ng] = ntiles;
            cap[ng] = (ntiles + nstream - 1) / nstream;
            nstream_of[ng] = nstream;
            deg_of[ng] = i;
            a.grp_degree[ng] = (uint8_t)i;
            a.grp_cp[ng] = (uint8_t)cp;
            ++ng;
        }
    }
    if (ng == 0) return;
    auto finish = [&](int g, int blocks) {
        const int64_t streams = (int64_t)blocks * nstream_of[g];
        return 40.0 + (double)((tiles_of[g] + streams - 1) / streams) * cost[g];
    };
    int count[MG], nb = 0;
    for (int g = 0; g < ng; ++g) { count[g] = 1; ++nb; }
    auto parts_of = [&](int g) {
        int n = 0;
        for (int h = 0; h < ng; ++h) if (deg_of[h] == deg_of[g]) ++n;
        return n;
    };
    const int env_blocks = switches().bank_stream_blocks;
    const int max_blocks = grid_cap(g_grid_caps.bank, env_blocks > 8 && env_blocks <= FUSED_MAX_BLOCKS ? env_blocks : 320);
    while (nb < max_blocks) {
        int worst = -1;
        double t_worst = -1.0;
        for (int g = 0; g < ng; ++g) {
            if (count[g] >= cap[g] || (int64_t)(count[g] + 1) * nstream_of[g] > SLAB_CHUNKS) continue;
            const double t = finish(g, count[g]);
            if (t > t_worst) { t_worst = t; worst = g; }
        }
        if (worst < 0) break;
        const int np = parts_of(worst);
        if (nb + np > max_blocks) break;
        for (int h = 0; h < ng; ++h) if (deg_of[h] == deg_of[worst]) ++count[h];
        nb += np;
    }
    int given[MG] = {};
    for (int b = 0; b < nb; ++b) {
        int pick = -1;
        double best = -1e30;
        for (int g = 0; g < ng; ++g) {
            if (given[g] >= count[g]) continue;
            const double lag = (double)count[g] * (b + 1) / nb - given[g];
            if (lag > best) { best = lag; pick = g; }
        }
        a.blk_group[b] = (uint8_t)pick;
        ++given[pick];
    }
    {
        int per_xcd[MG][8] = {};
        for (int b = 0; b < nb; ++b) ++per_xcd[a.blk_group[b]][b & 7];
        int next[MG][8];
        for (int g = 0; g < ng; ++g) {
            int run = 0;
            for (int x = 0; x < 8; ++x) { next[g][x] = run; run += per_xcd[g][x]; }
        }
        for (int b = 0; b < nb; ++b) a.blk_rank[b] = (uint16_t)next[a.blk_group[b]][b & 7]++;
    }
    for (int g = 0; g < ng; ++g) {
        a.grp_count[g] = (uint16_t)count[g];
        nchunk_out[deg_of[g]] = count[g] * nstream_of[g];
    }
    note_plan(2, nb, ng, tiles_of, count, nstream_of);
    out->nb = nb; out->prep_blocks = prep_blocks; out->KC = KC; out->lds_bytes = lds_fl * 4;
}

hipError_t launch_coef_prepare(const BankStreamLaunch& p, hipStream_t st) {
    if (p.prep_blocks == 0) return hipSuccess;
    coef_prepare_kernel<<<p.prep_blocks, 256, 0, st>>>(p.a);
    return hipGetLastError();
}

template <int KC, int SP = 0> static hipError_t launch_bank_kc(const BankStreamLaunch& p, hipStream_t st) {
    if (p.lds_bytes > 64 * 1024) {
        static PerDeviceOnce attr_set;
        if (const int slot = attr_set.pending(); slot >= 0) {
            hipError_t e = hipFuncSetAttribute((const void*)kc_backward_bank_stream<KC, SP>, hipFuncAttributeMaxDynamicSharedMemorySize,
                                               (KC >= 8 ? 128 : 80) * 1024);
            if (e != hipSuccess) return e;
            attr_set.set(slot);
        }
    }
    kc_backward_bank_stream<KC, SP><<<p.nb, 256, p.lds_bytes, st>>>(p.a);
    return hipGetLastError();
}

hipError_t launch_backward_bank_stream(const BankStreamLaunch& p, hipStream_t st) {
    if (p.nb == 0) return hipSuccess;
    if (p.lds_bytes > (size_t)(p.KC >= 8 ? 128 : 80) * 1024) return hipErrorInvalidValue;
    g_last_plan[2].launches.fetch_add(1);
    if (p.x_split) {
        if (!(p.KC <= 7 && bwd_split_mode() != 0)) return hipErrorInvalidValue;
        switch (p.KC) {
            case 1: return launch_bank_kc<1, 2>(p, st);
            case 2: return launch_bank_kc<2, 2>(p, st);
            case 3: return launch_bank_kc<3, 2>(p, st);
            case 4: return launch_bank_kc<4, 2>(p, st);
            case 5: return launch_bank_kc<5, 2>(p, st);
            case 6: return launch_bank_kc<6, 2>(p, st);
            default: return launch_bank_kc<7, 2>(p, st);
        }
    }
    if (p.KC <= 7 && bwd_split_mode() != 0) {
        switch (p.KC) {
            case 1: return launch_bank_kc<1, true>(p, st);
            case 2: return launch_bank_kc<2, true>(p, st);
            case 3: return launch_bank_kc<3, true>(p, st);
            case 4: return launch_bank_kc<4, true>(p, st);
            case 5: return launch_bank_kc<5, true>(p, st);
            case 6: return launch_bank_kc<6, true>(p, st);
            default: return launch_bank_kc<7, true>(p, st);
        }
    }
    switch (p.KC) {
        case 1: return launch_bank_kc<1>(p, st);
        case 2: return launch_bank_kc<2>(p, st);
        case 3: return launch_bank_kc<3>(p, st);
        case 4: return launch_bank_kc<4>(p, st);
        case 5: return launch_bank_kc<5>(p, st);
        case 6: return launch_bank_kc<6>(p, st);
        case 7: return launch_bank_kc<7>(p, st);
        case 8: return launch_bank_kc<8>(p, st);
        case 9: return launch_bank_kc<9>(p, st);
        case 10: return launch_bank_kc<10>(p, st);
        default: return hipErrorInvalidValue;
    }
}

}
```

molkgnn_amd/csrc/kgnn_capi.hip:

```cpp
#include <stdarg.h>
#include <stdio.h>
#include <string.h>

#include <mutex>

#include "kgnn_launch.h"
#include "kgnn_split.h"

using namespace mkgnn;

static thread_local char g_err[512] = "";

namespace mkgnn {
int api_fail(const char* fmt, ...) {
    va_list ap;
    va_start(ap, fmt);
    vsnprintf(g_err, sizeof(g_err), fmt, ap);
    va_end(ap);
    return 1;
}
int api_hip_fail(const char* what, hipError_t e) { return api_fail("%s: %s", what, hipGetErrorString(e)); }
}

struct DegreeStreams {
// ... 475 lines not shown
        return api_fail("%s: workspace of %zu bytes, need %zu", who, workspace_bytes, w.fwd_end);
    const bool block_rows_only = (variant & MKGNN_VARIANT_BLOCK_ROWS) != 0;
    const bool bank_prepared = (variant & MKGNN_VARIANT_BANK_PREPARED) != 0;
    const bool rows_split = (variant & MKGNN_VARIANT_ROWS_SPLIT) != 0;
    variant &= ~(MKGNN_VARIANT_BLOCK_ROWS | MKGNN_VARIANT_BANK_PREPARED | MKGNN_VARIANT_ROWS_SPLIT);
    if (variant < 0 || variant > 3) return api_fail("%s: variant %d", who, variant);
    const ConvShape shape = conv_shape(banks, buckets, F, E, n_atoms, x, x_stride, out_stride);
    const FwdDispatch plan = plan_conv_forward(shape, variant);
    if (rows_split && (variant == 1 || variant == 3 || !rows_split_covered(shape, plan)))
        return api_fail("%s: MKGNN_VARIANT_ROWS_SPLIT needs the streamed kernels with split-fp16 products for every degree "
                        "(mkgnn_rows_split_supported(..) tells)", who);
    if (const int g = plan.overflow_groups)
        return api_fail("%s: the banks need %d column groups, the %s launch holds %d", who, g, plan.overflow_launch, FUSED_MAX_GROUPS);
    if (const int d = plan.refused_degree)
        return api_fail("%s: MFMA variant does not cover degree %d with F=%d E=%d L=%d stride=%lld", who, d, F, E, L[d - 1], (long long)x_stride);
    hipStream_t st = (hipStream_t)stream; char* ws = (char*)workspace;
    hipError_t e = bank_prepared ? hipSuccess : launch_bank_prepare(banks, w, ws, F, E, st);
    if (e != hipSuccess) return api_hip_fail("bank_prepare", e);
    if (n_atoms > 0 && K > 0 && !block_rows_only) {
        const int64_t K4 = (K + 3) / 4 * 4;
        if (K4 == out_stride) e = hipMemsetAsync(out, 0, (size_t)n_atoms * out_stride * 4, st);
        else e = hipMemset2DAsync(out, (size_t)out_stride * 4, 0, (size_t)(K4 <= out_stride ? K4 : K) * 4, (size_t)n_atoms, st);
        if (e != hipSuccess) return api_hip_fail("output memset", e);
    }
    FusedFwdArgs fa; memset(&fa, 0, sizeof(fa));
    fa.x = x; fa.xs = x_stride; fa.inv = inv_norm; fa.out = out; fa.os = out_stride;
    fa.K = K; fa.F = F; fa.E = E; fa.last = is_last_layer ? 1 : 0; fa.n_atoms = n_atoms;
    fa.bf16 = variant == 3 ? 1 : 0;
    fa.x_split = rows_split ? 1 : 0;
    bool use_stream[4], use_bank[4], any_fused = false;
    int off = 0;
    for (int i = 0; i < 4; ++i) {
        const int d = i + 1; FwdArgs a;
        a.x = x; a.xs = x_stride; a.inv = inv_norm;
        a.sel = buckets[i].selected_index; a.nei = buckets[i].nei_index; a.e_nei = buckets[i].nei_edge_attr;
        a.p_focal = buckets[i].p_focal; a.p_nei = buckets[i].nei_p;
        a.n = buckets[i].count; a.F = F; a.E = E; a.L = L[i]; a.last = is_last_layer ? 1 : 0;
        a.cen = (const float*)(ws + w.bank[i].cen); a.sup = (const float*)(ws + w.bank[i].sup);
        a.edg = (const float*)(ws + w.bank[i].edg); a.chir = (const int8_t*)(ws + w.bank[i].chir);
        a.mix = (const float*)(ws + w.bank[i].mix);
        a.padded = (const float*)(ws + w.bank[i].padded); a.edge_padded = (const float*)(ws + w.bank[i].edge_padded);
        a.n_atoms = n_atoms;
        a.out = out; a.os = out_stride; a.off = off; a.K = K;
        a.pair = saved ? saved[i].pair_state : nullptr;
        a.chir_out = (saved && d == 4 && is_last_layer) ? saved[i].chirality : nullptr;
        off += L[i];
        use_stream[i] = plan.deg[i] == FWD_STREAMED; use_bank[i] = plan.deg[i] == FWD_LDS_BANK;
        if (use_stream[i] || use_bank[i]) {
            FusedDeg& g = fa.deg[i];
            g.sel = a.sel; g.nei = a.nei; g.e_nei = a.e_nei; g.e_unit = buckets[i].nei_edge_unit; g.p_focal = a.p_focal; g.p_nei = a.p_nei;
            g.padded = a.padded; g.edge_padded = a.edge_padded; g.chir = a.chir; g.mix = a.mix;
            g.eqflag = (const int8_t*)(ws + w.eqflag);
            g.signflag = (const int8_t*)(ws + w.signflag);
            g.pair = a.pair; g.chir_out = a.chir_out;
            g.n = a.n; g.L = a.L; g.off = a.off;
            any_fused = true;
        } else if (plan.deg[i] == FWD_GENERIC) {
            e = launch_forward_generic(d, a, st);
            if (e != hipSuccess) return api_hip_fail("kernelconv forward launch", e);
        }
    }
    if (any_fused) {
        e = launch_forward_fused(fa, use_stream, use_bank, st);
        if (e != hipSuccess) return api_hip_fail("fused kernelconv forward launch", e);
    }
    return 0;
}

int mkgnn_kernelsetconv_backward(const mkgnn_kernel_bank banks[MKGNN_MAX_DEGREE],
                                 const mkgnn_degree_bucket buckets[MKGNN_MAX_DEGREE], const float* x, int64_t x_stride,
                                 const float* inv_norm, int64_t n_atoms, int32_t F, int32_t E, int32_t is_last_layer,
                                 const float* grad_out, int64_t grad_out_stride,
                                 const mkgnn_saved saved[MKGNN_MAX_DEGREE], const int32_t* scatter_rowptr,
                                 const int32_t* scatter_rows, float* grad_x, int64_t grad_x_stride,
                                 const mkgnn_kernel_bank_grad grads[MKGNN_MAX_DEGREE], void* workspace,
                                 size_t workspace_bytes, int32_t workspace_from_forward, int32_t variant, void* stream) {
    const char* who = "mkgnn_kernelsetconv_backward";
    const bool defer_bank = (variant & MKGNN_BACKWARD_DEFER_BANK) != 0;
    const bool through_nei = (variant & MKGNN_BACKWARD_THROUGH_NEIGHBOURS) != 0;
    const bool rows_split = (variant & MKGNN_BACKWARD_ROWS_SPLIT) != 0;
    variant &= ~(MKGNN_BACKWARD_DEFER_BANK | MKGNN_BACKWARD_THROUGH_NEIGHBOURS | MKGNN_BACKWARD_ROWS_SPLIT);
    if (variant < 0 || variant > 2) return api_fail("%s: variant %d (0 = automatic, 1 = generic kernels, 2 = fast kernels)", who, variant);
    int64_t n_edges = 0;
    if (int rc = check_common(who, banks, buckets, x, x_stride, inv_norm, n_atoms, F, E, 0, &n_edges)) return rc;
    if (!saved || !grads) return api_fail("%s: saved/grads is null", who);
    int32_t L[4], K = 0;
    for (int i = 0; i < 4; ++i) { L[i] = banks[i].num_kernels; K += L[i]; }
    if (grad_out_stride < K || (n_atoms && !grad_out)) return api_fail("%s: bad grad_out", who);
    if (grad_x && grad_x_stride < F) return api_fail("%s: bad grad_x stride", who);
    if (grad_x && n_atoms && n_edges > 0 && (!scatter_rowptr || !scatter_rows)) return api_fail("%s: scatter CSR is null", who);
    WorkspaceLayout w = make_layout(L, F, E, n_atoms, n_edges);
    if (workspace_bytes < w.total || !workspace) return api_fail("%s: workspace of %zu bytes, need %zu", who, workspace_bytes, w.total);
    for (int i = 0; i < 4; ++i) {
        if (buckets[i].count > 0 && L[i] > 0 && !saved[i].pair_state) return api_fail("%s: degree %d has no saved forward state", who, i + 1);
        if (i == 3 && is_last_layer && buckets[i].count > 0 && !saved[i].chirality)
            return api_fail("%s: degree-4 chirality signs were not saved", who);
    }
    const BwdDispatch plan = plan_conv_backward(conv_shape(banks, buckets, F, E, n_atoms, x, x_stride, 0, grad_x, grad_x_stride), variant);
    if (const int d = plan.refused_degree)
        return api_fail("%s: the fast kernels do not cover degree %d with F=%d E=%d L=%d stride=%lld", who, d, F, E, L[d - 1], (long long)x_stride);
    if (through_nei && !plan.through_nei_ok)
        return api_fail("%s: MKGNN_BACKWARD_THROUGH_NEIGHBOURS needs the streamed kernels for every degree "
                        "(mkgnn_backward_streams(..) tells)", who);
    if (rows_split && !plan.rows_split_ok)
        return api_fail("%s: MKGNN_BACKWARD_ROWS_SPLIT needs the streamed kernels with split-fp16 products for every degree "
                        "(mkgnn_rows_split_supported(..) tells)", who);
    const bool fuse_bank = plan.bank_fused, rows_streamed = plan.rows_streamed, streamed = plan.bank_streamed;
    hipStream_t st = (hipStream_t)stream; char* ws = (char*)workspace;
    BwdArgs bank_a[4];
    BankReduceArgs reduce[4];
    bool bank_use[4];
    const float* e_unit4[4]; float* coefq4[4];
    int off = 0; int64_t base = 0;
    size_t coef_off = w.coefq_off[0];
    for (int i = 0; i < 4; ++i) {
        BwdArgs& a = bank_a[i];
        a.x = x; a.xs = x_stride; a.inv = inv_norm;
        a.sel = buckets[i].selected_index; a.nei = buckets[i].nei_index; a.e_nei = buckets[i].nei_edge_attr;
        a.n = buckets[i].count; a.F = F; a.E = E; a.L = L[i];
        a.cen = (const float*)(ws + w.bank[i].cen); a.sup = (const float*)(ws + w.bank[i].sup);
        a.edg = (const float*)(ws + w.bank[i].edg); a.mix = (const float*)(ws + w.bank[i].mix);
        a.gout = grad_out; a.gs = grad_out_stride; a.off = off;
        a.pair = saved[i].pair_state;
        a.chir = (i == 3 && is_last_layer) ? saved[i].chirality : nullptr;
        a.contrib = (float*)(ws + w.contrib); a.contrib_base = base; a.CS = (F + 3) / 4 * 4;
        a.slab = (float*)(ws + w.slab_off[i]);
        a.padded = (const float*)(ws + w.bank[i].padded);
        a.nchunk = (int)(a.n < BWD_BANK_BLOCKS ? (a.n > 0 ? a.n : 1) : BWD_BANK_BLOCKS);
        a.theta_slab = (float*)(ws + w.theta_off[i]);
        BankReduceArgs& r = reduce[i];
        r.slab = a.slab; r.F = F; r.E = E; r.L = L[i];
        r.cen = a.cen; r.sup = a.sup; r.edg = a.edg;
        r.icen = (const float*)(ws + w.bank[i].icen); r.isup = (const float*)(ws + w.bank[i].isup);
        r.iedg = (const float*)(ws + w.bank[i].iedg);
        r.g = grads[i];
        off += L[i]; base += buckets[i].count * (i + 2);
        bank_use[i] = fuse_bank && plan.deg[i] >= BWD_MFMA_LDS;
        e_unit4[i] = buckets[i].nei_edge_unit; coefq4[i] = nullptr;
        if (!bank_use[i]) continue;
        coefq4[i] = (float*)(ws + coef_off);
        coef_off += (size_t)((buckets[i].count + 15) / 16) * ((L[i] + 15) / 16) * 512 * 4;
    }
    const bool any_bank = bank_use[0] || bank_use[1] || bank_use[2] || bank_use[3];
    hipError_t e = hipSuccess;
    if (!workspace_from_forward) {
        e = launch_bank_prepare(banks, w, ws, F, E, st);
        if (e != hipSuccess) return api_hip_fail("bank_prepare", e);
    }
    int slot_of[4];
    degree_slots(banks, buckets, slot_of);
    ForkJoin fj;
    e = fj.begin(st, !g_time_bwd.load());
    if (e != hipSuccess) return api_hip_fail("stream fork", e);
    bool bank_on_main = false;
    for (int i = 0; i < 4; ++i) {
        const int d = i + 1;
        const BwdArgs& a = bank_a[i];
        hipStream_t dst = fj.stream(fj.two_way ? 0 : slot_of[i], &e);
        if (e != hipSuccess) return api_hip_fail("stream fork", e);
        int nchunk = a.n > 0 ? a.nchunk : 0;
        int ntheta = -1;
        if (plan.deg[i] == BWD_ZERO_FILL) {
            e = hipMemsetAsync(a.contrib + (size_t)a.contrib_base * a.CS, 0, (size_t)a.n * (d + 1) * a.CS * sizeof(float), dst);
            if (e != hipSuccess) return api_hip_fail("contribution rows memset", e);
        } else if (plan.deg[i] == BWD_GENERIC) {
            e = launch_backward_generic(d, a, dst);
            bank_on_main = true;
        } else if (plan.deg[i] >= BWD_LDS_PAIR) {
            const bool rows_mfma = plan.deg[i] != BWD_LDS_PAIR;
            hipStream_t st_rows = dst, st_bank = dst;
            if (fj.two_way && !rows_mfma) bank_on_main = true;
            if (fj.two_way && rows_mfma) {
                st_rows = st;
                if (!fuse_bank) {
                    st_bank = fj.stream(1, &e);
                    if (e != hipSuccess) return api_hip_fail("stream fork", e);
                }
            }
            if (rows_mfma && !rows_streamed && (grad_x || !fuse_bank)) {
                e = launch_backward_rows_mfma(d, a, &ntheta, st_rows);
                if (e != hipSuccess) return api_hip_fail("kernelconv backward launch", e);
            }
            if (!fuse_bank) e = launch_backward_lds(d, a, &nchunk, &ntheta, !rows_mfma, st_bank);
        }
        if (e != hipSuccess) return api_hip_fail("kernelconv backward launch", e);
        BankReduceArgs& r = reduce[i];
        r.nchunk = nchunk;
        if (ntheta >= 0) { r.theta_src = a.theta_slab; r.theta_stride = 4; r.theta_count = ntheta; }
        else {
            r.theta_src = a.slab + (size_t)L[i] * F + (size_t)L[i] * d * F + (size_t)L[i] * d * E;
            r.theta_stride = bank_floats(d, L[i], F, E); r.theta_count = nchunk;
        }
    }
    BankStreamLaunch bsl;
    int nchunk4[4] = {0, 0, 0, 0}, ntheta4[4] = {0, 0, 0, 0};
    if (streamed) {
        plan_backward_bank_stream(bank_a, bank_use, e_unit4, coefq4, nchunk4, ntheta4, through_nei, &bsl);
        bsl.x_split = rows_split ? 1 : 0;
        { BwdTimer t(st, 0); e = launch_coef_prepare(bsl, st); }
        if (e != hipSuccess) return api_hip_fail("coefficient pre-pass launch", e);
        e = fj.refork(1);
        if (e != hipSuccess) return api_hip_fail("stream fork", e);
    }
    if (rows_streamed && any_bank && grad_x) {
        BwdTimer t(st, 1);
        e = launch_backward_rows_stream(bank_a, bank_use, streamed ? coefq4 : nullptr, st);
        if (e != hipSuccess) return api_hip_fail("streamed rows launch", e);
    }
    if (any_bank) {
        hipStream_t st_bank = fj.stream(1, &e);
        if (e != hipSuccess) return api_hip_fail("stream fork", e);
        if (st_bank != st) {
            e = launch_pending_tail_reduce(st_bank);
            if (e != hipSuccess) return api_hip_fail("deferred tail reduction launch", e);
        }
        {
            BwdTimer t(st_bank, 2);
            if (streamed) e = launch_backward_bank_stream(bsl, st_bank);
            else e = launch_backward_bank_fused(bank_a, bank_use, nchunk4, ntheta4, st_bank);
        }
        if (e != hipSuccess) return api_hip_fail("fused bank gradient launch", e);
        for (int i = 0; i < 4; ++i)
            if (bank_use[i]) {
                reduce[i].nchunk = nchunk4[i];
                reduce[i].theta_src = bank_a[i].theta_slab; reduce[i].theta_stride = 4; reduce[i].theta_count = ntheta4[i];
            }
    }
    const bool split = fj.two_way && !bank_on_main && fj.used[0];
    if (!split) {
        e = fj.end();
        if (e != hipSuccess) return api_hip_fail("stream join", e);
    }
    hipStream_t st_reduce = st;
    if (split) {
        st_reduce = fj.stream(1, &e);
        if (e != hipSuccess) return api_hip_fail("stream fork", e);
    }
    { BwdTimer t(st_reduce, 3); e = launch_bank_reduce_all(reduce, st_reduce); }
    if (e != hipSuccess) return api_hip_fail("bank gradient reduce launch", e);
    if (grad_x && n_edges == 0) {
        if (n_atoms) e = hipMemset2DAsync(grad_x, (size_t)grad_x_stride * sizeof(float), 0, (size_t)F * sizeof(float), (size_t)n_atoms, st);
        if (e != hipSuccess) return api_hip_fail("zero input gradient", e);
    } else if (grad_x) {
        BwdTimer t(st, 4);
        e = launch_backward_gather((const float*)(ws + w.contrib), (F + 3) / 4 * 4, base, scatter_rowptr, scatter_rows, x,
                                   x_stride, inv_norm, n_atoms, F, grad_x, grad_x_stride, variant != 1, st, rows_split);
        if (e != hipSuccess) return api_hip_fail("backward gather launch", e);
    }
    if (split && defer_bank && fj.used[0] && !fj.used[1] && !fj.used[2]) {
        fj.p->deferred = true;
    } else if (split) {
        e = fj.end();
        if (e != hipSuccess) return api_hip_fail("stream join", e);
    }
    return 0;
}

int mkgnn_backward_streams(const mkgnn_kernel_bank banks[MKGNN_MAX_DEGREE], const mkgnn_degree_bucket buckets[MKGNN_MAX_DEGREE],
                           const float* x, int64_t x_stride, int64_t n_atoms, int32_t F, int32_t E) {
    if (!banks || !buckets) return 0;
    return plan_conv_backward(conv_shape(banks, buckets, F, E, n_atoms, x, x_stride, 0), 0).covers ? 1 : 0;
}

int mkgnn_rows_split_supported(const mkgnn_kernel_bank banks[MKGNN_MAX_DEGREE], const mkgnn_degree_bucket buckets[MKGNN_MAX_DEGREE],
                               int64_t x_stride, int64_t out_stride, int64_t n_atoms, int32_t F, int32_t E) {
    if (!banks || !buckets || F < 1 || E < 1) return 0;
    const ConvShape s = conv_shape(banks, buckets, F, E, n_atoms, nullptr, x_stride, out_stride);
    return rows_split_covered(s, plan_conv_forward(s, 0)) ? 1 : 0;
}

int mkgnn_backward_join(void* stream) {
    DegreeStreams* p = degree_streams();
    if (!p || !p->deferred) return 0;
    p->deferred = false;
    hipError_t e = hipEventRecord(p->join[0], p->aux[0]);
    if (e == hipSuccess) e = hipStreamWaitEvent((hipStream_t)stream, p->join[0], 0);
    return e == hipSuccess ? 0 : api_hip_fail("mkgnn_backward_join", e);
}

int mkgnn_segment_sum_rows(const float* in, int64_t in_stride, const int32_t* rowptr, const int32_t* col, int64_t n_rows,
                           int32_t width, float* out, int64_t out_stride, float* inv_norm, void* stream) {
    if (n_rows < 0 || width <= 0 || width > 16384 || in_stride < width || out_stride < width)
        return api_fail("mkgnn_segment_sum_rows: bad shape");
    if (n_rows && (!in || !rowptr || !out)) return api_fail("mkgnn_segment_sum_rows: null pointer");
    hipError_t e = launch_segment_sum(in, in_stride, rowptr, col, n_rows, width, out, out_stride, inv_norm, (hipStream_t)stream);
    return e == hipSuccess ? 0 : api_hip_fail("mkgnn_segment_sum_rows", e);
}

int mkgnn_segment_sum_block_rows(const float* in, int64_t in_stride, const int32_t* rowptr, const int32_t* col,
                                 const int8_t* degree, int64_t n_rows, const int32_t num_kernels[MKGNN_MAX_DEGREE],
                                 int32_t mode, float* out, int64_t out_stride, float* inv_norm, void* stream) {
    const char* who = "mkgnn_segment_sum_block_rows";
    if (mode < 1 || mode > 3) return api_fail("%s: mode %d (1 = block-row sources, 2 = block-row destinations, 3 = 1 with pre-split output)", who, mode);
    if (mode == 3 && !inv_norm) return api_fail("%s: mode 3 (pre-split rows) needs inv_norm", who);
    if (!num_kernels) return api_fail("%s: num_kernels is null", who);
    int width = 0;
    for (int i = 0; i < MKGNN_MAX_DEGREE; ++i) {
        if (num_kernels[i] < 0 || num_kernels[i] > 255) return api_fail("%s: num_kernels[%d] = %d outside 0..255", who, i, num_kernels[i]);
        width += num_kernels[i];
    }
    if (n_rows < 0 || width <= 0 || in_stride < width || out_stride < width) return api_fail("%s: bad shape", who);
    if (n_rows == 0) return 0;
    if (!in || !rowptr || !col || !out || (mode == 2 && !degree)) return api_fail("%s: null pointer", who);
    if (!segment_sum_blocks_supported(in, in_stride, n_rows, width, out, out_stride))
        return api_fail("%s: needs 16-byte aligned rows (strides multiples of 4 floats), at most 255 columns and fewer than 2^28 rows", who);
    hipError_t e = launch_segment_sum_blocks(in, in_stride, rowptr, col, degree, n_rows, width, num_kernels, mode, out, out_stride,
                                             inv_norm, (hipStream_t)stream);
    return e == hipSuccess ? 0 : api_hip_fail(who, e);
}

}
```

molkgnn_amd/csrc/kgnn_launch.h:

```cpp
#pragma once
#include "kgnn_common.h"
#include "kgnn_switches.h"

#include <atomic>

namespace mkgnn {

struct PrepArgs {
    mkgnn_kernel_bank bank[MKGNN_MAX_DEGREE];
    float* cen[MKGNN_MAX_DEGREE];
    float* sup[MKGNN_MAX_DEGREE];
    float* edg[MKGNN_MAX_DEGREE];
    float* icen[MKGNN_MAX_DEGREE];
    float* isup[MKGNN_MAX_DEGREE];
    float* iedg[MKGNN_MAX_DEGREE];
    int8_t* chir[MKGNN_MAX_DEGREE];
    float* mix[MKGNN_MAX_DEGREE];
    float* padded[MKGNN_MAX_DEGREE];
    float* edge_padded[MKGNN_MAX_DEGREE];
    int row_start[MKGNN_MAX_DEGREE + 1];
    int F, E;
};

struct FwdArgs {
    const float* x; int64_t xs; const float* inv;
    const int64_t* sel; const int64_t* nei; const float* e_nei; const float* p_focal; const float* p_nei;
    int64_t n; int F, E, L, last;
    const float* cen; const float* sup; const float* edg; const int8_t* chir; const float* mix;
    float* out; int64_t os; int off, K;
    float* pair; int8_t* chir_out;
    const float* padded; const float* edge_padded;
    int64_t n_atoms;
};

#ifdef MKGNN_EXP_MAX_BLOCKS
constexpr int FUSED_MAX_BLOCKS = MKGNN_EXP_MAX_BLOCKS;
#else
constexpr int FUSED_MAX_BLOCKS = 512;
#endif
constexpr int FUSED_MAX_GROUPS = 16;

struct FusedDeg {
    const int64_t* sel; const int64_t* nei; const float* e_nei; const float* e_unit; const float* p_focal; const float* p_nei;
    const float* padded; const float* edge_padded; const int8_t* chir; const float* mix; const int8_t* eqflag; const int8_t* signflag;
    float* pair; int8_t* chir_out;
    int64_t n;
    int L, off;
    int nct;
    int kpt;
    int cs;
    int nloc;
    int ics;
};

struct FusedFwdArgs {
    const float* x; int64_t xs; const float* inv;
    float* out; int64_t os;
    int K, F, E, last;
    int64_t n_atoms;
    int bf16;
    int x_split;
    int FPB;
    FusedDeg deg[MKGNN_MAX_DEGREE];
    uint8_t grp_degree[FUSED_MAX_GROUPS];
    uint8_t grp_cp[FUSED_MAX_GROUPS];
    uint16_t grp_count[FUSED_MAX_GROUPS];
    uint8_t blk_group[FUSED_MAX_BLOCKS];
    uint16_t blk_rank[FUSED_MAX_BLOCKS];
    unsigned long long* stamps;
};

struct BwdArgs {
    const float* x; int64_t xs; const float* inv;
    const int64_t* sel; const int64_t* nei; const float* e_nei;
    int64_t n; int F, E, L;
    const float* cen; const float* sup; const float* edg; const float* mix;
    const float* gout; int64_t gs; int off;
    const float* pair; const int8_t* chir;
    float* contrib; int64_t contrib_base;
    int CS;
    float* slab; int nchunk;
    const float* padded;
    float* theta_slab;
    int theta_in_bank;
};

struct BankReduceArgs {
    const float* slab; int nchunk; int F, E, L;
    const float* theta_src; size_t theta_stride; int theta_count;
    const float* cen; const float* sup; const float* edg;
    const float* icen; const float* isup; const float* iedg;
    mkgnn_kernel_bank_grad g;
};

hipError_t launch_row_inv_norm(const float* x, int64_t stride, int64_t n, int F, float* inv, hipStream_t st);
constexpr int PREP_MANY_MAX = 4;
constexpr int TOUCH_MAX = 16, TOUCH_BLOCKS = 512;
struct TouchArgs { const char* ptr[TOUCH_MAX]; uint32_t bytes[TOUCH_MAX]; int count; };
bool take_touch_hint(TouchArgs& out);
#ifdef __HIPCC__
__device__ __forceinline__ void touch_body(const TouchArgs& t, uint32_t b, uint32_t nb) {
    uint32_t acc = 0;
    const uint32_t stride = nb * 256u;
    for (int k = 0; k < t.count; ++k) {
        const uint4* const p = (const uint4*)t.ptr[k];
        const uint32_t n16 = t.bytes[k] >> 4;
        for (uint32_t i = b * 256u + threadIdx.x; i < n16; i += 8u * stride) {
            uint4 v[8];
#pragma unroll
            for (int u = 0; u < 8; ++u) {
                const uint32_t j = i + (uint32_t)u * stride;
                v[u] = p[j < n16 ? j : n16 - 1u];
            }
#pragma unroll
            for (int u = 0; u < 8; ++u) acc ^= v[u].x ^ v[u].y ^ v[u].z ^ v[u].w;
        }
    }
    asm volatile("" :: "v"(acc));
}
#endif
struct PrepManyArgs { PrepArgs layer[PREP_MANY_MAX]; int task_start[PREP_MANY_MAX + 1]; int count; int prep_blocks; TouchArgs touch; };
hipError_t launch_bank_prepare_many(int count, const mkgnn_kernel_bank* banks , const WorkspaceLayout* w,
                                    char* const* ws, const int* F, int E, hipStream_t st, const TouchArgs* touch = nullptr);
void build_bank_prepare_many(int count, const mkgnn_kernel_bank* banks, const WorkspaceLayout* w, char* const* ws, const int* F,
                             int E, PrepManyArgs* out);
hipError_t launch_bank_prepare_args(const PrepManyArgs& m, hipStream_t st);
bool take_pending_prepare(PrepManyArgs& out);
hipError_t launch_bank_prepare(const mkgnn_kernel_bank banks[4], const WorkspaceLayout& w, char* ws, int F, int E,
                               hipStream_t st);
hipError_t launch_forward_generic(int d, const FwdArgs& a, hipStream_t st);
bool mfma_forward_supported(int d, int F, int E, int L);
int fused_group_count(int d, int F, int L);
hipError_t launch_forward_fused(FusedFwdArgs& a, const bool use_stream[4], const bool use_bank[4], hipStream_t st);
bool stream_forward_supported(int d, int F, int E, int L, int64_t n_atoms, int64_t x_stride, int64_t out_stride, const float* e_unit);
hipError_t launch_forward_stream(FusedFwdArgs& a, const bool use[4], hipStream_t st);
int stream_tiles_per_part(int d);
int stream_column_parts(int d, int L);
bool stream_rows_split_supported(int F);
bool stream_forward_bf16_supported(int F);
int stream_forward_groups(const int L[4], const bool use[4]);
hipError_t launch_unit_rows8(const float* in, int64_t n_rows, int E, float* out, hipStream_t st);
hipError_t launch_backward_generic(int d, const BwdArgs& a, hipStream_t st);
struct BankReduceAllArgs { BankReduceArgs deg[4]; int blk_start[4]; };
hipError_t launch_bank_reduce_all(const BankReduceArgs r[4], hipStream_t st);
bool lds_backward_supported(int d, int F, int E, int L, int64_t xs, bool x_aligned);
hipError_t launch_backward_lds(int d, const BwdArgs& a, int* nchunk_out, int* ntheta_out, bool rows_too, hipStream_t st);
int bank_blocks_for(int d, int64_t n);
hipError_t launch_backward_bank_fused(const BwdArgs a4[4], const bool use[4], int nchunk_out[4], int ntheta_out[4], hipStream_t st);
bool bank_stream_supported(int d, int F, int E, int L, int64_t n_atoms, int64_t x_stride, const float* e_unit);
bool bank_stream_rows_split_supported(int F);
struct BankStreamDeg {
    const int64_t* sel; const int64_t* nei; const float* e_unit;
    const float* pair; const int8_t* chir;
    const float* mix;
    float* coefq;
    float* slab;
    float* theta_slab;
    int64_t n;
    int L, off, nct, kpt, cs;
    int prep_blk0, prep_blocks;
};

struct BankStreamArgs {
    const float* x; int64_t xs; const float* inv;
    const float* gout; int64_t gs;
    int F, E;
    int through_nei;
    BankStreamDeg deg[MKGNN_MAX_DEGREE];
    uint8_t grp_degree[FUSED_MAX_GROUPS];
    uint8_t grp_cp[FUSED_MAX_GROUPS];
    uint16_t grp_count[FUSED_MAX_GROUPS];
    uint8_t blk_group[FUSED_MAX_BLOCKS];
    uint16_t blk_rank[FUSED_MAX_BLOCKS];
};

struct TailMidArgs {
    const float* z; float* dz;
    const int32_t *rin, *cin, *rout, *cout;
    const int32_t *mol_ptr, *atom_mol;
    int64_t n_atoms, n_mols, n_loss;
    const float *b1, *w2, *b2, *wh, *bh, *y;
    int H, G;
    float drop_p; const int64_t* rng;
    float* emb; int64_t es;
    float* pred;
    float* slab; int slab_stride;
    int mg;
    float rdrop_p;
};
constexpr int TAIL_MAX_BLOCKS = 768;
constexpr int TAIL_B1 = 0, TAIL_W2 = 32, TAIL_B2 = 32 + 1024, TAIL_WH = TAIL_B2 + 32, TAIL_BH = TAIL_WH + 32, TAIL_LOSS = TAIL_BH + 1,
              TAIL_SLAB = (TAIL_LOSS + 1 + 3) / 4 * 4;
hipError_t launch_pending_tail_reduce(hipStream_t st, bool* launched = nullptr);
int tail_group_size(int64_t n_loss_mols);
int tail_middle_blocks(int64_t n_loss_mols);
hipError_t launch_tail_middle(const TailMidArgs& a, int nb, int loss_kind, hipStream_t st);
hipError_t launch_tail_score(const TailMidArgs& a, int nb, hipStream_t st);

struct AtomContribArgs {
    const float* z;
    const int32_t *rin, *cin; int64_t n;
    const float *b1, *w2, *b2;
    const float* wh; int64_t wh_stride;
    int H, G, T;
    float* out; int64_t os;
};
constexpr int ATOM_CONTRIB_MAX_BLOCKS = 1024;
hipError_t launch_atom_contrib(const AtomContribArgs& a, hipStream_t st);

struct BankStreamLaunch { BankStreamArgs a; int nb, prep_blocks, KC; size_t lds_bytes; int x_split; };
void plan_backward_bank_stream(const BwdArgs a4[4], const bool use[4], const float* const e_unit[4], float* const coefq[4],
                               int nchunk_out[4], int ntheta_out[4], bool through_nei, BankStreamLaunch* out);
hipError_t launch_coef_prepare(const BankStreamLaunch& p, hipStream_t st);
hipError_t launch_backward_bank_stream(const BankStreamLaunch& p, hipStream_t st);
bool rows_stream_supported(int d, int F, int E, int L);
hipError_t launch_backward_rows_stream(const BwdArgs a4[4], const bool use[4], float* const coefq[4], hipStream_t st);
bool mfma_backward_supported(int d, int F, int E, int L, int64_t xs, bool x_aligned, int64_t n_atoms);
hipError_t launch_backward_rows_mfma(int d, const BwdArgs& a, int* ntheta_out, hipStream_t st);
hipError_t launch_backward_gather(const float* contrib, int64_t cs, int64_t n_contrib_rows, const int32_t* rowptr,
                                  const int32_t* rows, const float* x, int64_t xs, const float* inv, int64_t n, int F,
                                  float* gx, int64_t gxs, bool allow_fast, hipStream_t st, bool x_split = false);
bool segment_sum_blocks_supported(const float* in, int64_t is, int64_t n, int width, const float* out, int64_t os);
hipError_t launch_segment_sum_blocks(const float* in, int64_t is, const int32_t* rowptr, const int32_t* col, const int8_t* deg8,
                                     int64_t n, int width, const int32_t L[4], int mode, float* out, int64_t os,
                                     float* inv_norm, hipStream_t st);
bool try_segment_sum_aligned(const float* in, int64_t is, const int32_t* rowptr, const int32_t* col, int64_t n, int width,
                             float* out, int64_t os, float* inv_norm, hipStream_t st, hipError_t* err);
bool try_backward_gather_aligned(const float* contrib, int64_t cs, const int32_t* rowptr, const int32_t* rows, const float* x,
                                 int64_t xs, const float* inv, int64_t n, int F, float* gx, int64_t gxs, hipStream_t st,
                                 hipError_t* err, bool x_split = false);
bool try_rows_presplit(const float* x, int64_t xs, int64_t n, int width, float* inv, float* out, int64_t os, hipStream_t st, hipError_t* err);
bool try_row_inv_norm_aligned(const float* x, int64_t xs, int64_t n, int width, float* inv, hipStream_t st, hipError_t* err);
hipError_t launch_segment_sum(const float* in, int64_t is, const int32_t* rowptr, const int32_t* col, int64_t n,
                              int width, float* out, int64_t os, float* inv_norm, hipStream_t st);

struct PerDeviceOnce {
    std::atomic<bool> done[16];
    PerDeviceOnce() { for (auto& d : done) d.store(false); }
    int pending() {
        int dev = 0;
        if (hipGetDevice(&dev) != hipSuccess || dev < 0 || dev >= 16) return 0;
        return done[dev].load(std::memory_order_acquire) ? -1 : dev;
    }
    void set(int dev) { if (dev >= 0 && dev < 16) done[dev].store(true, std::memory_order_release); }
};

struct GridCaps { std::atomic<int> fwd{0}, rows{0}, bank{0}; };
extern GridCaps g_grid_caps;
struct PlanInfo { std::atomic<int> blocks{0}, min_iters{0}, max_iters{0}, launches{0}; };
extern PlanInfo g_last_plan[3];
inline int grid_cap(const std::atomic<int>& cap, int dflt) {
    const int c = cap.load(std::memory_order_relaxed);
    return (c >= 8 && c <= FUSED_MAX_BLOCKS) ? c : dflt;
}
inline void note_plan(int which, int blocks, int ng, const int64_t* tiles_of, const int* count, const int* nstream_of) {
    int lo = 1 << 30, hi = 0;
    for (int g = 0; g < ng; ++g) {
        const int64_t streams = (int64_t)count[g] * nstream_of[g];
        const int it = (int)((tiles_of[g] + streams - 1) / streams);
        if (it < lo) lo = it;
        if (it > hi) hi = it;
    }
    g_last_plan[which].blocks.store(blocks); g_last_plan[which].min_iters.store(ng ? lo : 0); g_last_plan[which].max_iters.store(hi);
}

int api_fail(const char* fmt, ...);
int api_hip_fail(const char* what, hipError_t e);

int bwd_split_mode();

}
```

molkgnn_amd/csrc/kgnn_readout.hip:

```cpp
#include <hip/hip_runtime.h>
#include <cstdint>
#include "kgnn_common.h"
#include <mutex>

#include "kgnn_launch.h"
#include "kgnn_philox.h"
#include "../../include/molkgnn_hip.h"

namespace mkgnn {

typedef mkgnn_f32x4 f32x4;

struct ReadoutArgs {
    const float* h; int64_t hs; int64_t n;
    const int32_t* mol_ptr; const int32_t* atom_mol; int64_t nmol;
    const float *w1, *b1, *w2, *b2;
    int F, H, G;
    const float* keep;
    float* pre;
    float* pooled;
    float* out; int64_t os;
    const float* gout; int64_t gos;
    float* dA;
    float* gh; int64_t ghs;
// ... 816 lines not shown
    }
    if (K != p->F) return api_fail("%s: lin1 takes %d columns, the blocks hold %d", who, p->F, K);
    if (sim_stride < K || sim_stride % 4 || !sim || ((uintptr_t)sim & 15)) return api_fail("%s: sim rows must be 16-byte aligned", who);
    if (n_bucketed > n_atoms) return api_fail("%s: the buckets hold more atoms than the batch", who);
    b.w1 = p->lin1_weight; b.H = p->H; b.K = K; b.HP = d.HP; b.FP = d.FP;
    return 0;
}

static hipError_t project_blocks(BlockProjArgs& b, const ReadoutDims& d, int64_t n_focal, const float* sim, int64_t sim_stride,
                                 int64_t n_atoms, float* z, hipStream_t st) {
    b.sim = sim; b.ss = sim_stride; b.n = n_atoms; b.z = z;
    if (n_focal < n_atoms) {
        const hipError_t e = hipMemsetAsync(z, 0, (size_t)n_atoms * d.HP * 4, st);
        if (e != hipSuccess) return e;
    }
    int64_t grid = 0;
    for (int i = 0; i < MKGNN_MAX_DEGREE; ++i) if (b.L[i] > 0) grid += ((b.cnt[i] + 15) / 16 + 3) / 4;
    if (grid > 0) {
        const size_t lds = ((size_t)d.HP * 68 + 4 * 16 * (d.HP + 4)) * 4;
        if (d.NT == 2) block_project_mfma_kernel<2><<<(unsigned)grid, 256, lds, st>>>(b);
        else block_project_mfma_kernel<4><<<(unsigned)grid, 256, lds, st>>>(b);
    }
    return hipSuccess;
}

size_t mkgnn_readout_blocks_workspace_bytes(int32_t K, int32_t H, int32_t G, int64_t n_mols) {
    ReadoutDims d;
    if (!blocks_dims(K, H, G, d) || n_mols < 0) return 0;
    return readout_ws(d, H, G, n_mols).total;
}

int mkgnn_readout_blocks_supported(int32_t F, int32_t H, int32_t G, const int32_t num_kernels[MKGNN_MAX_DEGREE]) {
    ReadoutDims d;
    if (!num_kernels || !blocks_dims(F, H, G, d)) return 0;
    int K = 0;
    for (int i = 0; i < MKGNN_MAX_DEGREE; ++i) { if (num_kernels[i] < 0 || num_kernels[i] > 64) return 0; K += num_kernels[i]; }
    return K == F;
}

int mkgnn_readout_blocks_forward(const mkgnn_readout_params* p, const float* sim, int64_t sim_stride,
                                 const int32_t num_kernels[MKGNN_MAX_DEGREE], const mkgnn_degree_bucket buckets[MKGNN_MAX_DEGREE],
                                 int64_t n_atoms, const int32_t* in_rowptr, const int32_t* in_col, const int32_t* mol_ptr,
                                 int64_t n_mols, const float* keep_scale, float* z, float* pre, float* pooled, float* gate_sum,
                                 float* out, int64_t out_stride, void* stream) {
    const char* who = "mkgnn_readout_blocks_forward";
    ReadoutDims d;
    if (!p || !blocks_dims(p->F, p->H, p->G, d)) return api_fail("%s: shape outside K<=255, H<=64, G<=64", who);
    if (!p->lin1_weight || !p->lin2_weight) return api_fail("%s: weight pointer is null", who);
    if (n_atoms < 1 || n_mols < 1 || n_atoms >= (int64_t)1 << 31) return api_fail("%s: bad sizes", who);
    if (!in_rowptr || !in_col || !mol_ptr || !z || !pre || !pooled || !out || out_stride < p->G)
        return api_fail("%s: null pointer or bad out stride", who);
    BlockProjArgs b{};
    int64_t n_focal = 0;
    if (int rc = check_blocks(who, p, num_kernels, buckets, n_atoms, sim_stride, sim, b, d, &n_focal)) return rc;
    hipStream_t st = (hipStream_t)stream;
    hipError_t e = project_blocks(b, d, n_focal, sim, sim_stride, n_atoms, z, st);
    if (e != hipSuccess) return api_hip_fail(who, e);
    e = launch_segment_sum(z, d.HP, in_rowptr, in_col, n_atoms, d.HP, pre, d.HP, nullptr, st);
    if (e != hipSuccess) return api_hip_fail(who, e);
    ReadoutArgs a = readout_args(p, nullptr, 0, n_atoms, mol_ptr, nullptr, n_mols, keep_scale, pre, pooled);
    a.out = out; a.os = out_stride; a.pre_bias = p->lin1_bias; a.gsum = gate_sum;
    const int pgrid = (int)((n_mols + 3) / 4 < 2048 ? (n_mols + 3) / 4 : 2048);
    readout_pool_kernel<<<pgrid, 256, 0, st>>>(a, d.HP);
    e = hipGetLastError();
    return e == hipSuccess ? 0 : api_hip_fail(who, e);
}

int mkgnn_readout_blocks_backward(const mkgnn_readout_params* p, const float* sim, int64_t sim_stride,
                                  const int32_t num_kernels[MKGNN_MAX_DEGREE], const mkgnn_degree_bucket buckets[MKGNN_MAX_DEGREE],
                                  int64_t n_atoms, const int32_t* out_rowptr, const int32_t* out_col, const int32_t* mol_ptr,
                                  const int32_t* atom_mol, int64_t n_mols, const float* gate, const float* gate_sum,
                                  const float* pooled, const float* grad_out, int64_t grad_out_stride, float* dz,
                                  float* grad_sim, int64_t grad_sim_stride, float* grad_lin1_weight, float* grad_lin1_bias,
                                  float* grad_lin2_weight, float* grad_lin2_bias, void* ws, size_t ws_bytes, void* stream) {
    const char* who = "mkgnn_readout_blocks_backward";
    ReadoutDims d;
    if (!p || !blocks_dims(p->F, p->H, p->G, d)) return api_fail("%s: shape outside K<=255, H<=64, G<=64", who);
    if (n_atoms < 1 || n_mols < 1 || n_atoms >= (int64_t)1 << 31) return api_fail("%s: bad sizes", who);
    if (!out_rowptr || !out_col || !mol_ptr || !atom_mol || !gate || !gate_sum || !pooled || !grad_out || grad_out_stride < p->G || !dz)
        return api_fail("%s: null pointer or bad grad_out stride", who);
    BlockProjArgs b{};
    int64_t n_focal = 0;
    if (int rc = check_blocks(who, p, num_kernels, buckets, n_atoms, sim_stride, sim, b, d, &n_focal)) return rc;
    if (grad_sim && grad_sim_stride < b.K) return api_fail("%s: bad grad_sim stride", who);
    const ReadoutWs w = readout_ws(d, p->H, p->G, n_mols);
    if (!ws || ws_bytes < w.total) return api_fail("%s: workspace too small (%zu < %zu)", who, ws_bytes, w.total);
    hipStream_t st = (hipStream_t)stream;
    ReadoutArgs a = readout_args(p, nullptr, 0, n_atoms, mol_ptr, atom_mol, n_mols, nullptr, (float*)gate, (float*)pooled);
    a.gsum = (float*)gate_sum;
    a.gout = grad_out; a.gos = grad_out_stride;
    a.dA = (float*)((char*)ws + w.dA);
    a.slab_atoms = (float*)((char*)ws + w.slab_atoms); a.slab_atoms_stride = w.slab_atoms_stride;
    a.slab_mol = (float*)((char*)ws + w.slab_mol); a.slab_mol_stride = w.slab_mol_stride;
    a.nblk_mol = (int)((n_mols + 15) / 16 < RO_MOL_BLOCKS ? (n_mols + 15) / 16 : RO_MOL_BLOCKS);
    readout_bwd_mol_kernel<<<a.nblk_mol, 256, 0, st>>>(a, d.HP);
    DzArgs z{};
    z.dA = a.dA; z.gate = gate; z.atom_mol = atom_mol; z.rowptr = out_rowptr; z.col = out_col; z.n = n_atoms; z.dz = dz;
    const int rpb = 256 / (d.HP / 4);
    const int nb_dz = (int)((n_atoms + rpb - 1) / rpb < DZ_BLOCKS ? (n_atoms + rpb - 1) / rpb : DZ_BLOCKS);
    if (d.NT == 2) readout_dz_gather_kernel<8><<<nb_dz, 256, 0, st>>>(z);
    else readout_dz_gather_kernel<16><<<nb_dz, 256, 0, st>>>(z);
    hipError_t e = hipSuccess;
    b.sim = sim; b.ss = sim_stride; b.n = n_atoms; b.dz = dz; b.dsim = grad_sim; b.dss = grad_sim_stride;
    int64_t tiles_all = 0;
    for (int i = 0; i < MKGNN_MAX_DEGREE; ++i) if (b.L[i] > 0) tiles_all += (b.cnt[i] + 15) / 16;
    int tpw = (int)((tiles_all + 4 * (2 * RO_ATOM_BLOCKS - 4) - 1) / (4 * (2 * RO_ATOM_BLOCKS - 4)));
    if (tpw < 1) tpw = 1;
    int64_t nb_of[MKGNN_MAX_DEGREE], nb = 0;
    for (int i = 0; i < MKGNN_MAX_DEGREE; ++i) {
        const int64_t tiles = (b.cnt[i] + 15) / 16, per = 4 * (int64_t)tpw;
        nb_of[i] = b.L[i] > 0 ? (tiles + per - 1) / per : 0;
        nb += nb_of[i];
    }
    if (nb > 2 * RO_ATOM_BLOCKS) return api_fail("%s: internal: %lld blocks for %d slabs", who, (long long)nb, 2 * RO_ATOM_BLOCKS);
    b.slab = a.slab_atoms; b.slab_stride = a.slab_atoms_stride;
    if (nb > 0) {
        const size_t img = (size_t)4 * (16 * (d.HP + 4) + 16 * 68);
        const size_t lds = ((size_t)d.HP * 68 + (img > 4096 ? img : 4096)) * 4;
        if (d.NT == 2) block_project_bwd_mfma_kernel<2><<<(unsigned)nb, 256, lds, st>>>(b, tpw);
        else block_project_bwd_mfma_kernel<4><<<(unsigned)nb, 256, lds, st>>>(b, tpw);
    }
    SlabReduceArgs r{};
    int blk = 0;
    auto add = [&](const float* src, int stride, int count, int src_cols, int rows, int cols, float* dst, int dst_stride) {
        if (!dst || count < 1 || rows * cols < 1) return;
        SlabSeg& sg = r.seg[r.nseg++];
        sg.src = src; sg.stride = stride; sg.count = count; sg.src_cols = src_cols; sg.dst_rows = rows; sg.dst_cols = cols;
        sg.dst = dst; sg.blk_start = blk; sg.dst_stride = dst_stride;
        blk += (rows * cols + 31) / 32;
    };
    bool absent = false;
    {
        int64_t b0 = 0;
        for (int i = 0; i < MKGNN_MAX_DEGREE; ++i) {
            if (b.L[i] > 0 && nb_of[i] == 0) absent = true;
            if (nb_of[i] > 0)
                add(a.slab_atoms + (size_t)b0 * a.slab_atoms_stride + b.off[i], a.slab_atoms_stride, (int)nb_of[i], d.FP, p->H, b.L[i],
                    grad_lin1_weight ? grad_lin1_weight + b.off[i] : nullptr, b.K);
            b0 += nb_of[i];
        }
    }
    if (absent && grad_lin1_weight) {
        e = hipMemsetAsync(grad_lin1_weight, 0, (size_t)p->H * b.K * 4, st);
        if (e != hipSuccess) return api_hip_fail(who, e);
    }
    add(a.slab_mol + p->G * p->H + p->G, a.slab_mol_stride, a.nblk_mol, d.HP, 1, p->H, grad_lin1_bias, 0);
    add(a.slab_mol, a.slab_mol_stride, a.nblk_mol, p->H, p->G, p->H, grad_lin2_weight, 0);
    add(a.slab_mol + p->G * p->H, a.slab_mol_stride, a.nblk_mol, p->G, 1, p->G, grad_lin2_bias, 0);
    if (blk > 0) slab_reduce_kernel<<<blk, 256, 0, st>>>(r);
    e = hipGetLastError();
    return e == hipSuccess ? 0 : api_hip_fail(who, e);
}

struct TailWs { size_t z, dz, slab_atoms, slab_tail, total; int slab_atoms_stride; };
static TailWs tail_ws(const ReadoutDims& d, int64_t n_atoms, int64_t n_mols) {
    TailWs w;
    auto up = [](size_t v) { return (v + 255) / 256 * 256; };
    w.slab_atoms_stride = d.HP * d.FP + d.HP;
    w.z = 0;
    w.dz = up(w.z + (size_t)n_atoms * 32 * 4);
    w.slab_atoms = up(w.dz + (size_t)n_atoms * 32 * 4);
    w.slab_tail = up(w.slab_atoms + (size_t)2 * RO_ATOM_BLOCKS * w.slab_atoms_stride * 4);
    w.total = up(w.slab_tail + (size_t)(n_mols < TAIL_MAX_BLOCKS ? n_mols : TAIL_MAX_BLOCKS) * TAIL_SLAB * 4);
    return w;
}

int mkgnn_tail_supported(int32_t K, int32_t H, int32_t G, const int32_t num_kernels[MKGNN_MAX_DEGREE]) {
    ReadoutDims d;
    if (!num_kernels || !blocks_dims(K, H, G, d) || H > 32 || G > 32) return 0;
    return mkgnn_readout_blocks_supported(K, H, G, num_kernels);
}

size_t mkgnn_tail_workspace_bytes(int32_t K, int32_t H, int32_t G, int64_t n_atoms, int64_t n_mols) {
    ReadoutDims d;
    if (!blocks_dims(K, H, G, d) || n_atoms < 1 || n_mols < 1) return 0;
    return tail_ws(d, n_atoms, n_mols).total;
}

static int project_into_workspace(const char* who, const mkgnn_readout_params* ro, const int32_t num_kernels[MKGNN_MAX_DEGREE],
                                  const mkgnn_degree_bucket* buckets, const float* sim, int64_t sim_stride, int64_t n_atoms,
                                  size_t total, void* ws, size_t ws_bytes, hipStream_t st, BlockProjArgs& b, const ReadoutDims& d) {
    int64_t n_focal = 0;
    if (int rc = check_blocks(who, ro, num_kernels, buckets, n_atoms, sim_stride, sim, b, d, &n_focal)) return rc;
    if (!ws || ws_bytes < total) return api_fail("%s: workspace too small (%zu < %zu)", who, ws_bytes, total);
    hipError_t e = launch_pending_tail_reduce(st);
    if (e == hipSuccess) e = project_blocks(b, d, n_focal, sim, sim_stride, n_atoms, (float*)ws, st);
    return e == hipSuccess ? 0 : api_hip_fail(who, e);
}

extern "C++" template <typename Own>
static int tail_project(const char* who, const mkgnn_tail_args* p, Own&& own, size_t (*need)(int32_t, int32_t, int32_t, int64_t, int64_t),
                        void* ws, size_t ws_bytes, hipStream_t st, BlockProjArgs& b, ReadoutDims& d) {
    if (!p) return api_fail("%s: null argument", who);
    const mkgnn_readout_params* ro = &p->readout;
    if (!mkgnn_tail_supported(ro->F, ro->H, ro->G, p->num_kernels) || !blocks_dims(ro->F, ro->H, ro->G, d))
        return api_fail("%s: K=%d H=%d G=%d outside the fused tail (the block-row readout's shapes with H, G <= 32)", who, ro->F, ro->H, ro->G);
    if (p->n_atoms < 1 || p->n_mols < 1 || p->n_loss_mols < 1 || p->n_loss_mols > p->n_mols || p->n_atoms >= (int64_t)1 << 31)
        return api_fail("%s: bad sizes", who);
    if (int rc = own()) return rc;
    if (p->emb && p->emb_stride < ro->G) return api_fail("%s: bad emb stride", who);
    return project_into_workspace(who, ro, p->num_kernels, p->buckets, p->sim, p->sim_stride, p->n_atoms,
                                  need(ro->F, ro->H, ro->G, p->n_atoms, p->n_mols), ws, ws_bytes, st, b, d);
}

static int tail_fused(const char* who, const mkgnn_tail_args* p, float rp, void* ws, size_t ws_bytes, void* stream) {
    hipStream_t st = (hipStream_t)stream;
    BlockProjArgs b{};
    ReadoutDims d;
    auto own = [&]() {
        const mkgnn_readout_params* ro = &p->readout;
        if (!p->in_rowptr || !p->in_col || !p->out_rowptr || !p->out_col || !p->mol_ptr || !p->atom_mol || !ro->lin1_weight ||
            !ro->lin2_weight || !p->head_weight || !p->target || !p->pred || !p->loss || !p->grad_sim)
            return api_fail("%s: null pointer", who);
        if (p->dropout_p < 0.f || p->dropout_p >= 1.f) return api_fail("%s: dropout probability %g outside [0, 1)", who, (double)p->dropout_p);
        if (p->dropout_p > 0.f && (!p->rng_state || !p->rng_used)) return api_fail("%s: dropout needs rng_state and rng_used", who);
        if (!(rp >= 0.f && rp < 1.f)) return api_fail("%s: readout dropout probability %g outside [0, 1)", who, (double)rp);
        if (rp > 0.f && (!p->rng_state || !p->rng_used)) return api_fail("%s: readout dropout needs rng_state and rng_used", who);
        if (p->loss_kind < MKGNN_LOSS_BCE_MEAN || p->loss_kind > MKGNN_LOSS_SQERR_SUM) return api_fail("%s: unknown loss kind %d", who, (int)p->loss_kind);
        if (p->grad_sim_stride < ro->F) return api_fail("%s: bad grad_sim stride", who);
        return 0;
    };
    if (int rc = tail_project(who, p, own, mkgnn_tail_workspace_bytes, ws, ws_bytes, st, b, d)) return rc;
    const mkgnn_readout_params* ro = &p->readout;
    const TailWs w = tail_ws(d, p->n_atoms, p->n_mols);
    float* const z = (float*)((char*)ws + w.z);
    float* const dz = (float*)((char*)ws + w.dz);
    hipError_t e = hipSuccess;
    TailMidArgs m{};
    m.z = z; m.dz = dz; m.rin = p->in_rowptr; m.cin = p->in_col; m.rout = p->out_rowptr; m.cout = p->out_col;
    m.mol_ptr = p->mol_ptr; m.atom_mol = p->atom_mol; m.n_atoms = p->n_atoms; m.n_mols = p->n_mols; m.n_loss = p->n_loss_mols;
    m.b1 = ro->lin1_bias; m.w2 = ro->lin2_weight; m.b2 = ro->lin2_bias; m.wh = p->head_weight; m.bh = p->head_bias; m.y = p->target;
    m.H = ro->H; m.G = ro->G; m.drop_p = p->dropout_p; m.rng = p->rng_state; m.rdrop_p = rp;
    m.emb = p->emb; m.es = p->emb_stride; m.pred = p->pred;
    m.slab = (float*)((char*)ws + w.slab_tail); m.slab_stride = TAIL_SLAB;
    m.mg = tail_group_size(p->n_loss_mols);
    const int nbm = tail_middle_blocks(p->n_loss_mols);
    e = launch_tail_middle(m, nbm, p->loss_kind, st);
    if (e != hipSuccess) return api_hip_fail(who, e);
    b.dz = dz; b.dsim = p->grad_sim; b.dss = p->grad_sim_stride;
    int64_t tiles_all = 0;
    for (int i = 0; i < MKGNN_MAX_DEGREE; ++i) if (b.L[i] > 0) tiles_all += (b.cnt[i] + 15) / 16;
    int tpw = (int)((tiles_all + 4 * (2 * RO_ATOM_BLOCKS - 4) - 1) / (4 * (2 * RO_ATOM_BLOCKS - 4)));
    if (tpw < 1) tpw = 1;
    int64_t nb_of[MKGNN_MAX_DEGREE], nb = 0;
    for (int i = 0; i < MKGNN_MAX_DEGREE; ++i) {
        const int64_t tiles = (b.cnt[i] + 15) / 16, per = 4 * (int64_t)tpw;
        nb_of[i] = b.L[i] > 0 ? (tiles + per - 1) / per : 0;
        nb += nb_of[i];
    }
    if (nb > 2 * RO_ATOM_BLOCKS) return api_fail("%s: internal: %lld blocks for %d slabs", who, (long long)nb, 2 * RO_ATOM_BLOCKS);
    float* const slab_atoms = (float*)((char*)ws + w.slab_atoms);
    b.slab = slab_atoms; b.slab_stride = w.slab_atoms_stride;
    if (nb > 0) {
        const size_t img = (size_t)4 * (16 * (d.HP + 4) + 16 * 68);
        const size_t lds = ((size_t)d.HP * 68 + (img > 4096 ? img : 4096)) * 4;
        block_project_bwd_mfma_kernel<2><<<(unsigned)nb, 256, lds, st>>>(b, tpw);
    }
    SlabReduceArgs r{};
    int blk = 0;
    auto add = [&](const float* src, int stride, int count, int src_cols, int rows, int cols, float* dst, int dst_stride) {
        if (!dst || count < 1 || rows * cols < 1) return;
        SlabSeg& sg = r.seg[r.nseg++];
        sg.src = src; sg.stride = stride; sg.count = count; sg.src_cols = src_cols; sg.dst_rows = rows; sg.dst_cols = cols;
        sg.dst = dst; sg.blk_start = blk; sg.dst_stride = dst_stride;
        blk += (rows * cols + 31) / 32;
    };
    bool absent = false;
    {
        int64_t b0 = 0;
        for (int i = 0; i < MKGNN_MAX_DEGREE; ++i) {
            if (b.L[i] > 0 && nb_of[i] == 0) absent = true;
            if (nb_of[i] > 0)
                add(slab_atoms + (size_t)b0 * w.slab_atoms_stride + b.off[i], w.slab_atoms_stride, (int)nb_of[i], d.FP, ro->H, b.L[i],
                    p->grad_lin1_weight ? p->grad_lin1_weight + b.off[i] : nullptr, b.K);
            b0 += nb_of[i];
        }
    }
    if (absent && p->grad_lin1_weight) {
        e = hipMemsetAsync(p->grad_lin1_weight, 0, (size_t)ro->H * b.K * 4, st);
        if (e != hipSuccess) return api_hip_fail(who, e);
    }
    add(m.slab + TAIL_B1, TAIL_SLAB, nbm, 32, 1, ro->H, p->grad_lin1_bias, 0);
    add(m.slab + TAIL_W2, TAIL_SLAB, nbm, 32, ro->G, ro->H, p->grad_lin2_weight, 0);
    add(m.slab + TAIL_B2, TAIL_SLAB, nbm, 32, 1, ro->G, p->grad_lin2_bias, 0);
    add(m.slab + TAIL_WH, TAIL_SLAB, nbm, 32, 1, ro->G, p->grad_head_weight, 0);
    add(m.slab + TAIL_BH, TAIL_SLAB, nbm, 1, 1, 1, p->grad_head_bias, 0);
    add(m.slab + TAIL_LOSS, TAIL_SLAB, nbm, 1, 1, 1, p->loss, 0);
    r.drop_p = p->dropout_p > 0.f ? p->dropout_p : rp; r.rng = p->rng_state; r.rng_used = p->rng_used;
    if (p->defer_reduce && blk > 0) {
        e = hipGetLastError();
        if (e != hipSuccess) return api_hip_fail(who, e);
        std::lock_guard<std::mutex> lock(g_pending_reduce_mutex);
        PendingReduce* slot = pending_reduce_slot();
        slot->r = r; slot->blk = blk;
        return 0;
    }
    if (blk > 0) slab_reduce_kernel<<<blk, 256, 0, st>>>(r);
    e = hipGetLastError();
    return e == hipSuccess ? 0 : api_hip_fail(who, e);
}

int mkgnn_tail_fused(const mkgnn_tail_args* p, void* ws, size_t ws_bytes, void* stream) {
    return tail_fused("mkgnn_tail_fused", p, 0.f, ws, ws_bytes, stream);
}

int mkgnn_tail_fused_readout_dropout(const mkgnn_tail_args* p, float readout_dropout_p, void* ws, size_t ws_bytes, void* stream) {
    return tail_fused("mkgnn_tail_fused_readout_dropout", p, readout_dropout_p, ws, ws_bytes, stream);
}

size_t mkgnn_tail_score_workspace_bytes(int32_t K, int32_t H, int32_t G, int64_t n_atoms, int64_t n_mols) {
    ReadoutDims d;
    if (!blocks_dims(K, H, G, d) || n_atoms < 1 || n_mols < 1) return 0;
    return tail_ws(d, n_atoms, n_mols).dz;
}

int mkgnn_tail_score(const mkgnn_tail_args* p, void* ws, size_t ws_bytes, void* stream) {
    const char* who = "mkgnn_tail_score";
    hipStream_t st = (hipStream_t)stream;
    BlockProjArgs b{};
    ReadoutDims d;
    auto own = [&]() {
        const mkgnn_readout_params* ro = &p->readout;
        if (!p->in_rowptr || !p->in_col || !p->mol_ptr || !p->atom_mol || !ro->lin1_weight || !ro->lin2_weight || !p->head_weight || !p->pred)
            return api_fail("%s: null pointer", who);
        return 0;
    };
    if (int rc = tail_project(who, p, own, mkgnn_tail_score_workspace_bytes, ws, ws_bytes, st, b, d)) return rc;
    const mkgnn_readout_params* ro = &p->readout;
    float* const z = (float*)ws;
    TailMidArgs m{};
    m.z = z; m.rin = p->in_rowptr; m.cin = p->in_col; m.mol_ptr = p->mol_ptr; m.atom_mol = p->atom_mol;
    m.n_atoms = p->n_atoms; m.n_mols = p->n_mols; m.n_loss = p->n_loss_mols;
    m.b1 = ro->lin1_bias; m.w2 = ro->lin2_weight; m.b2 = ro->lin2_bias; m.wh = p->head_weight; m.bh = p->head_bias;
    m.H = ro->H; m.G = ro->G;
    m.emb = p->emb; m.es = p->emb_stride; m.pred = p->pred;
    m.mg = tail_group_size(p->n_loss_mols);
    const hipError_t e = launch_tail_score(m, tail_middle_blocks(p->n_loss_mols), st);
    return e == hipSuccess ? 0 : api_hip_fail(who, e);
}

size_t mkgnn_atom_contributions_workspace_bytes(int32_t K, int32_t H, int32_t G, int64_t n_atoms) {
    ReadoutDims d;
    if (!blocks_dims(K, H, G, d) || n_atoms < 1) return 0;
    return tail_ws(d, n_atoms, 1).dz;
}

int mkgnn_atom_contributions(const mkgnn_atom_contrib_args* p, void* ws, size_t ws_bytes, void* stream) {
    const char* who = "mkgnn_atom_contributions";
    if (!p) return api_fail("%s: null argument", who);
    const mkgnn_readout_params* ro = &p->readout;
    ReadoutDims d;
    if (!mkgnn_tail_supported(ro->F, ro->H, ro->G, p->num_kernels) || !blocks_dims(ro->F, ro->H, ro->G, d))
        return api_fail("%s: K=%d H=%d G=%d outside the fused tail's shapes (the block-row readout's with H, G <= 32)", who, ro->F, ro->H, ro->G);
    if (p->T < 1 || p->T > MKGNN_ATOM_CONTRIB_MAX_TASKS)
        return api_fail("%s: %d tasks outside [1, %d]", who, (int)p->T, MKGNN_ATOM_CONTRIB_MAX_TASKS);
    if (p->n_atoms < 0 || p->n_atoms >= (int64_t)1 << 31) return api_fail("%s: bad sizes", who);
    if (p->contrib_stride < p->T) return api_fail("%s: contrib stride %lld below T = %d", who, (long long)p->contrib_stride, (int)p->T);
    if (p->head_stride < ro->G) return api_fail("%s: head stride %lld below G = %d", who, (long long)p->head_stride, ro->G);
    if (p->n_atoms == 0) return 0;
    if (!p->in_rowptr || !p->in_col || !ro->lin1_weight || !ro->lin2_weight || !p->head_weight || !p->contrib)
        return api_fail("%s: null pointer", who);
    hipStream_t st = (hipStream_t)stream;
    BlockProjArgs b{};
    if (int rc = project_into_workspace(who, ro, p->num_kernels, p->buckets, p->sim, p->sim_stride, p->n_atoms,
                                        mkgnn_atom_contributions_workspace_bytes(ro->F, ro->H, ro->G, p->n_atoms), ws, ws_bytes, st, b, d))
        return rc;
    AtomContribArgs a{};
    a.z = (const float*)ws; a.rin = p->in_rowptr; a.cin = p->in_col; a.n = p->n_atoms;
    a.b1 = ro->lin1_bias; a.w2 = ro->lin2_weight; a.b2 = ro->lin2_bias; a.wh = p->head_weight; a.wh_stride = p->head_stride;
    a.H = ro->H; a.G = ro->G; a.T = p->T;
    a.out = p->contrib; a.os = p->contrib_stride;
    const hipError_t e = launch_atom_contrib(a, st);
    return e == hipSuccess ? 0 : api_hip_fail(who, e);
}

struct ReadoutMaskArgs { const int64_t* rng; int64_t n; int H; float p; float* keep; int64_t ks; };
__global__ void __launch_bounds__(256) readout_dropout_mask_kernel(ReadoutMaskArgs a) {
    const int64_t total = a.n * a.H;
    const uint64_t seed = (uint64_t)a.rng[0], offset = (uint64_t)a.rng[1];
    for (int64_t i = (int64_t)blockIdx.x * 256 + threadIdx.x; i < total; i += (int64_t)gridDim.x * 256) {
        const int64_t r = i / a.H;
        const int h = (int)(i - r * a.H);
        a.keep[r * a.ks + h] = keep_scale_of(seed, offset, readout_drop_element(r, a.H, h), a.p);
    }
}

int mkgnn_readout_dropout_mask(const int64_t* rng_pair, int64_t n_rows, int32_t H, float p, float* keep, int64_t keep_stride, void* stream) {
    const char* who = "mkgnn_readout_dropout_mask";
    if (!rng_pair || !keep) return api_fail("%s: null pointer", who);
    if (n_rows < 0 || H < 1 || keep_stride < H) return api_fail("%s: bad sizes", who);
    if (!(p >= 0.f && p < 1.f)) return api_fail("%s: dropout probability %g outside [0, 1)", who, (double)p);
    if (n_rows == 0) return 0;
    ReadoutMaskArgs a{rng_pair, n_rows, H, p, keep, keep_stride};
    const int64_t blocks = (n_rows * H + 255) / 256;
    readout_dropout_mask_kernel<<<(unsigned)(blocks < 4096 ? blocks : 4096), 256, 0, (hipStream_t)stream>>>(a);
    const hipError_t e = hipGetLastError();
    return e == hipSuccess ? 0 : api_hip_fail(who, e);
}

extern "C++" {
namespace mkgnn {
hipError_t launch_pending_tail_reduce(hipStream_t st, bool* launched) {
    if (launched) *launched = false;
    std::lock_guard<std::mutex> lock(g_pending_reduce_mutex);
    PendingReduce* slot = pending_reduce_slot();
    if (slot->blk <= 0) return hipSuccess;
    const int blk = slot->blk;
    slot->blk = 0;
    slab_reduce_kernel<<<blk, 256, 0, st>>>(slot->r);
    if (launched) *launched = true;
    return hipGetLastError();
}
}
}

extern "C" int mkgnn_tail_flush(void* stream) {
    const hipError_t e = launch_pending_tail_reduce((hipStream_t)stream);
    return e == hipSuccess ? 0 : api_hip_fail("mkgnn_tail_flush", e);
}

}
```

molkgnn_amd/csrc/kgnn_switches.h:

```cpp
#pragma once
#include <stdio.h>
#include <stdlib.h>

#ifndef MKGNN_FWD_PP_DEFAULT
#define MKGNN_FWD_PP_DEFAULT 0
#endif
#ifndef MKGNN_FWD_PAIR_DEFAULT
#define MKGNN_FWD_PAIR_DEFAULT 0
#endif
#ifndef MKGNN_FWD_SPLIT_DEFAULT
#define MKGNN_FWD_SPLIT_DEFAULT 1
#endif
#ifndef MKGNN_BWD_SPLIT_DEFAULT
#define MKGNN_BWD_SPLIT_DEFAULT 1
#endif

namespace mkgnn {

struct Switches {
    bool serial;
    bool fork_in_graph;
    bool no_mfma_bwd;
    bool fork_mode;
    bool bank_fused;
    bool rows_stream;
    bool bank_stream;
    bool fwd_stream;
    bool bf16_stream;
    bool rows_split;
    bool bn_one_launch;
    char helper_priority;
    int fwd_pp;
    bool fwd_pp_env;
    int fwd_split;
    int bwd_split;
    int fwd_pair;
    int rows_stream_blocks;
    int bank_stream_blocks;
    int bank_blocks;
    int csr_blocks;
    int csr_fixed4;
    int csr_cpl;
    bool stream_cost_set;
    double stream_cost[4];
};

inline const Switches& switches() {
    static const Switches table = [] {
        auto is_set = [](const char* name) { return getenv(name) != nullptr; };
        auto not_0 = [](const char* name) { const char* e = getenv(name); return !(e && e[0] == '0'); };
        auto number = [](const char* name, int unset) { const char* e = getenv(name); return e ? atoi(e) : unset; };
        Switches s{};
        s.serial = is_set("MKGNN_SERIAL"); s.fork_in_graph = is_set("MKGNN_FORK_IN_GRAPH"); s.no_mfma_bwd = is_set("MKGNN_NO_MFMA_BWD");
        s.fork_mode = not_0("MKGNN_FORK_MODE"); s.bank_fused = not_0("MKGNN_BANK_FUSED"); s.rows_stream = not_0("MKGNN_ROWS_STREAM");
        s.bank_stream = not_0("MKGNN_BANK_STREAM"); s.fwd_stream = not_0("MKGNN_FWD_STREAM"); s.bf16_stream = not_0("MKGNN_BF16_STREAM");
        s.rows_split = not_0("MKGNN_ROWS_SPLIT");
        if (const char* e = getenv("MKGNN_BN_ONE_LAUNCH")) s.bn_one_launch = e[0] == '1';
        if (const char* e = getenv("MKGNN_HELPER_PRIORITY")) s.helper_priority = e[0];
        s.fwd_pp = number("MKGNN_FWD_PP", MKGNN_FWD_PP_DEFAULT); s.fwd_pp_env = number("MKGNN_FWD_PP", 0) != 0;
        s.fwd_split = number("MKGNN_FWD_SPLIT", MKGNN_FWD_SPLIT_DEFAULT); s.bwd_split = number("MKGNN_BWD_SPLIT", MKGNN_BWD_SPLIT_DEFAULT);
        s.fwd_pair = number("MKGNN_FWD_PAIR", MKGNN_FWD_PAIR_DEFAULT); s.bank_blocks = number("MKGNN_BANK_BLOCKS", 0);
        s.rows_stream_blocks = number("MKGNN_ROWS_STREAM_BLOCKS", 0); s.bank_stream_blocks = number("MKGNN_BANK_STREAM_BLOCKS", 0);
        s.csr_blocks = number("MKGNN_CSR_BLOCKS", 256 * 16); s.csr_fixed4 = number("MKGNN_CSR_FIXED4", 0);
        s.csr_cpl = number("MKGNN_CSR_CPL", 0);
        if (const char* e = getenv("MKGNN_STREAM_COST"))
            s.stream_cost_set = sscanf(e, "%lf,%lf,%lf,%lf", &s.stream_cost[0], &s.stream_cost[1], &s.stream_cost[2], &s.stream_cost[3]) == 4;
        return s;
    }();
    return table;
}

}
```

molkgnn_amd/readout.py:

```python
from __future__ import annotations

import ctypes

import weakref
from typing import Optional, Tuple

import os

import torch

from . import _lib
from .functional import _aligned_rows, _row_major, _stride0

_SEG_CACHE: dict = {}
_SEG_CACHE_MAX = 32


class MoleculeSegments:

    @classmethod
    def from_tensors(cls, mol_ptr: torch.Tensor, atom_mol: torch.Tensor, max_atoms: Optional[int] = None,
                     max_edges: Optional[int] = None) -> "MoleculeSegments":
        if mol_ptr.dtype != torch.int32 or atom_mol.dtype != torch.int32:
            raise TypeError("mol_ptr and atom_mol must be int32")
# ... 770 lines not shown
    return 1 <= R <= _lib.MAX_COSINE_MAX_REFS and 1 <= H <= _lib.MAX_COSINE_MAX_H


MAX_COSINE_TORCH_CHUNK = 4096


def _first_max(sim: torch.Tensor):
    c = sim.shape[1]
    nan = torch.isnan(sim)
    clean = torch.where(nan, torch.full_like(sim, float("-inf")), sim)
    best = clean.max(dim=1, keepdim=True).values
    col = torch.arange(c, device=sim.device)[None, :].expand_as(sim)
    arg = torch.where((clean == best) & ~nan, col, torch.full_like(col, c)).min(dim=1).values
    none = arg == c
    arg = torch.where(none, torch.zeros_like(arg), arg)
    value = sim.gather(1, arg[:, None])[:, 0]
    return torch.where(none, torch.full_like(value, float("nan")), value), arg


_MAX_COSINE_WS: dict = {}


def _max_cosine_workspace(dev, nbytes: int, given: Optional[torch.Tensor]) -> torch.Tensor:
    if given is not None:
        if not torch.is_tensor(given) or given.dtype != torch.uint8 or given.device != dev or not given.is_contiguous() \
                or given.numel() < nbytes:
            raise ValueError(f"workspace: a contiguous uint8 tensor of at least {nbytes} bytes on {dev}")
        return given
    if torch.cuda.is_current_stream_capturing():
        return torch.empty(nbytes, dtype=torch.uint8, device=dev)
    held = _MAX_COSINE_WS.get(str(dev))
    if held is None or held.numel() < nbytes:
        held = _MAX_COSINE_WS[str(dev)] = torch.empty(max(nbytes, 1 << 16), dtype=torch.uint8, device=dev)
    return held


def embedding_max_cosine(emb: torch.Tensor, refs: torch.Tensor, n_rows: Optional[int] = None, out=None,
                         workspace: Optional[torch.Tensor] = None):
    if not (torch.is_tensor(emb) and torch.is_tensor(refs)) or emb.dim() != 2 or refs.dim() != 2 \
            or emb.dtype != torch.float32 or refs.dtype != torch.float32 or refs.shape[1] != emb.shape[1]:
        raise ValueError("embedding_max_cosine needs a float32 [n, H] embedding and float32 [R, H] references")
    R, H = refs.shape
    if R < 1 or H < 1:
        raise ValueError(f"embedding_max_cosine needs at least one reference and one column, not {R} x {H}")
    if not emb.is_cuda or refs.device != emb.device:
        raise ValueError(f"embedding_max_cosine runs on the GPU: emb is on {emb.device}, refs on {refs.device} (there is no CPU "
                         "path; screening.max_cosine_reference is the host form)")
    if torch.is_grad_enabled() and (emb.requires_grad or refs.requires_grad):
        raise RuntimeError("embedding_max_cosine is forward only: call it under torch.no_grad() (or on detached inputs)")
    n = emb.shape[0] if n_rows is None else int(n_rows)
    if not 0 <= n <= emb.shape[0]:
        raise ValueError(f"n_rows = {n_rows} outside [0, {emb.shape[0]}]")
    dev = emb.device
    if out is None:
        out = (torch.empty(n, dtype=torch.float32, device=dev), torch.empty(n, dtype=torch.int32, device=dev))
    else:
        ok = isinstance(out, (tuple, list)) and len(out) == 2 and all(torch.is_tensor(o) for o in out)
        if not ok or out[0].dtype != torch.float32 or out[1].dtype != torch.int32 \
                or any(o.device != dev or tuple(o.shape) != (n,) or not o.is_contiguous() for o in out):
            raise ValueError(f"out: a pair of contiguous tensors (float32 [{n}], int32 [{n}]) on {dev}")
    max_sim, arg_ref = out
    if n == 0:
        return max_sim, arg_ref
    if not embedding_max_cosine_supported(R, H):
        e, eps = emb[:n].detach().double(), float(torch.tensor(COSINE_EPS, dtype=torch.float32))
        ie = 1.0 / e.square().sum(dim=1).sqrt().clamp_min(eps)
        best = arg = None
        for a in range(0, R, MAX_COSINE_TORCH_CHUNK):
            q = refs[a:a + MAX_COSINE_TORCH_CHUNK].detach().double()
            iq = 1.0 / q.square().sum(dim=1).sqrt().clamp_min(eps)
            value, index = _first_max(((e @ q.t() + 0.0) * ie[:, None] * iq[None, :]).float())
            if best is None:
                best, arg = value, index
            else:
                take = ~torch.isnan(value) & (torch.isnan(best) | (value > best))
                best, arg = torch.where(take, value, best), torch.where(take, index + a, arg)
        max_sim.copy_(best)
        arg_ref.copy_(arg)
        return max_sim, arg_ref
    emb, refs = _row_major(emb.detach()), _row_major(refs.detach())
    lib = _lib.load()
    ws = _max_cosine_workspace(dev, int(lib.mkgnn_embed_max_cosine_workspace_bytes(n, R)), workspace)
    with torch.cuda.device(dev):
        _lib.check(lib.mkgnn_embed_max_cosine(emb.data_ptr(), _stride0(emb), n, H, refs.data_ptr(), _stride0(refs), R,
                                              max_sim.data_ptr(), arg_ref.data_ptr(), ws.data_ptr(), ws.numel(),
                                              _lib.stream_ptr(dev)), "mkgnn_embed_max_cosine")
    return max_sim, arg_ref


def select_rows(scores: torch.Tensor, ids: torch.Tensor, key: torch.Tensor, n_valid, bounds: torch.Tensor, out=None):
    tensors = (scores, ids, key, bounds)
    if not all(torch.is_tensor(t) for t in tensors) or scores.dtype != torch.float32 or key.dtype != torch.float32 \
            or ids.dtype != torch.int32 or bounds.dtype != torch.float32:
        raise ValueError("select_rows needs float32 scores and key, int32 ids and float32 bounds")
    B = scores.numel()
    if B < 1 or scores.dim() != 1 or tuple(ids.shape) != (B,) or tuple(key.shape) != (B,) or tuple(bounds.shape) != (2,) \
            or not all(t.is_contiguous() for t in tensors):
        raise ValueError("select_rows needs contiguous scores, ids and key of one length B >= 1 and bounds [2]")
    dev = scores.device
    if dev.type != "cuda" or any(t.device != dev for t in tensors):
        raise ValueError(f"select_rows runs on the GPU: scores are on {dev} (there is no CPU path; screening.select_rows_reference "
                         "is the host form)")
    if torch.is_tensor(n_valid):
        if n_valid.dtype != torch.int32 or n_valid.numel() != 1 or n_valid.device != dev:
            raise ValueError("n_valid: one int32 on the scores' device, or an int")
    else:
        n_valid = torch.tensor([int(n_valid)], dtype=torch.int32, device=dev)
    if out is None:
        out = (torch.empty(B, dtype=torch.float32, device=dev), torch.empty(B, dtype=torch.int32, device=dev),
               torch.empty(1, dtype=torch.int32, device=dev))
    else:
        ok = isinstance(out, (tuple, list)) and len(out) == 3 and all(torch.is_tensor(o) and o.device == dev and o.is_contiguous()
                                                                      for o in out)
        if not ok or out[0].dtype != torch.float32 or out[1].dtype != torch.int32 or out[2].dtype != torch.int32 \
                or tuple(out[0].shape) != (B,) or tuple(out[1].shape) != (B,) or out[2].numel() != 1:
            raise ValueError(f"out: contiguous (float32 [{B}], int32 [{B}], int32 [1]) on {dev}")
    with torch.cuda.device(dev):
        _lib.check(_lib.load().mkgnn_select_rows(scores.data_ptr(), ids.data_ptr(), key.data_ptr(), B, n_valid.data_ptr(),
                                                 bounds.data_ptr(), out[0].data_ptr(), out[1].data_ptr(), out[2].data_ptr(),
                                                 _lib.stream_ptr(dev)), "mkgnn_select_rows")
    return tuple(out)


_FUSED_TAIL = os.environ.get("MKGNN_FUSED_TAIL", "1") != "0"
_TAIL_WS: dict = {}


def _tail_workspace(dev, nbytes: int) -> torch.Tensor:
    held = _TAIL_WS.setdefault(str(dev), [])
    if not held or held[-1].numel() < nbytes:
        held.append(torch.empty(max(nbytes, 1 << 20), dtype=torch.uint8, device=dev))
    return held[-1]


def _tail_limits_ok(seg: "MoleculeSegments", plan) -> bool:
    ma, me = getattr(seg, "max_atoms", None), getattr(seg, "max_edges", None)
    if ma is None or me is None:
        if getattr(seg, "from_loader", False) or torch.cuda.is_current_stream_capturing():
            return False
        ptr = seg.mol_ptr.long()
        sizes = ptr[1:] - ptr[:-1]
        rin, rout = plan.csr_in[0].long(), plan.csr_out[0].long()
        ein, eout = rin[ptr[1:]] - rin[ptr[:-1]], rout[ptr[1:]] - rout[ptr[:-1]]
        ma, me = int(sizes.max().item()), int(torch.maximum(ein.max(), eout.max()).item())
        seg.max_atoms, seg.max_edges = ma, me
    return ma <= _lib.TAIL_MAX_ATOMS and me <= _lib.TAIL_MAX_EDGES


def tail_supported(K: int, H: int, G: int, blocks) -> bool:
    return bool(_lib.load().mkgnn_tail_supported(int(K), int(H), int(G), _lib.Int32x4(*[int(b) for b in blocks])))


_DEFER_TAIL_REDUCE = False
_TAIL_HELD: list = []


def tail_flush(device) -> None:
    try:
        with torch.cuda.device(device):
            _lib.check(_lib.load().mkgnn_tail_flush(_lib.stream_ptr(device)), "mkgnn_tail_flush")
    finally:
        _TAIL_HELD.clear()


class deferred_tail_reduce:

    def __init__(self, device):
        self.device = device

    def __enter__(self):
        global _DEFER_TAIL_REDUCE
        self.prev, _DEFER_TAIL_REDUCE = _DEFER_TAIL_REDUCE, _TAIL_DEFER_ENABLED
        return self

    def __exit__(self, *exc):
        global _DEFER_TAIL_REDUCE
        _DEFER_TAIL_REDUCE = self.prev
        if not self.prev and self.device is not None and torch.device(self.device).type == "cuda":
            tail_flush(self.device)
        return False


_TAIL_DEFER_ENABLED = os.environ.get("MKGNN_TAIL_DEFER", "1") != "0"


def _tail_grads_adopted(params) -> bool:
    return all(p is None or (not p._backward_hooks and not getattr(p, "_post_accumulate_grad_hooks", None) and p.is_contiguous())
               for p in params)


def _tail_args(sim, plan, blocks, seg, n_rows, w1c, b1, w2c, b2, whc, bh):
    a = _lib.TailArgs()
    a.sim, a.sim_stride = sim.data_ptr(), _stride0(sim)
    for i, L in enumerate(blocks):
        a.num_kernels[i] = int(L)
    bk = _sel_buckets(plan)
    a.buckets = ctypes.cast(bk, ctypes.c_void_p)
    rin, cin = plan.csr_in
    a.in_rowptr, a.in_col = rin.data_ptr(), cin.data_ptr()
    a.mol_ptr, a.atom_mol = seg.mol_ptr.data_ptr(), seg.atom_mol.data_ptr()
    a.n_atoms, a.n_mols, a.n_loss_mols = sim.shape[0], seg.size, n_rows
    a.readout = _params(w1c, b1, w2c, b2)
    a.head_weight, a.head_bias = whc.data_ptr(), _lib.ptr(bh)
    return a, (bk,)


class _TailFn(torch.autograd.Function):

    @staticmethod
    def forward(ctx, sim, w1, b1, w2, b2, wh, bh, target, seg, plan, blocks, p_drop, n_rows, kind=_lib.LOSS_BCE_MEAN, p_readout=0.0):
        lib = _lib.load()
        _lib.require_gpu_tensor(sim, "sim_sc")
        n, K = sim.shape
        dev = sim.device
        w1c, w2c = w1.contiguous(), w2.contiguous()
        H, G = w1c.shape[0], w2c.shape[0]
        whc = wh.reshape(-1).contiguous()
        y = target.reshape(-1).float().contiguous()
        B = int(n_rows)
        pred = torch.empty(B, dtype=torch.float32, device=dev)
        loss = torch.empty((), dtype=torch.float32, device=dev)
        K4 = K + (-K) % 4
        gsim = torch.empty((n, K4), dtype=torch.float32, device=dev)[:, :K]
        gw1, gw2, gwh = torch.empty_like(w1c), torch.empty_like(w2c), torch.empty_like(whc)
        gb1 = torch.empty_like(b1) if b1 is not None else None
        gb2 = torch.empty_like(b2) if b2 is not None else None
        gbh = torch.empty(1, dtype=torch.float32, device=dev) if bh is not None else None
        drop = p_drop > 0.0 or p_readout > 0.0
        rng = head_rng_state(dev) if drop else None
        used = torch.empty(2, dtype=torch.int64, device=dev) if drop else None
        a, keep = _tail_args(sim, plan, blocks, seg, B, w1c, b1, w2c, b2, whc, bh)
        rout, cout = plan.csr_out
        a.out_rowptr, a.out_col = rout.data_ptr(), cout.data_ptr()
        a.target = y.data_ptr()
        a.dropout_p, a.rng_state, a.rng_used = float(p_drop), _lib.ptr(rng), _lib.ptr(used)
        a.pred, a.loss = pred.data_ptr(), loss.data_ptr()
        a.grad_sim, a.grad_sim_stride = gsim.data_ptr(), K4
        a.grad_lin1_weight, a.grad_lin1_bias = gw1.data_ptr(), _lib.ptr(gb1)
        a.grad_lin2_weight, a.grad_lin2_bias = gw2.data_ptr(), _lib.ptr(gb2)
        a.grad_head_weight, a.grad_head_bias = gwh.data_ptr(), _lib.ptr(gbh)
        ctx.deferred = bool(_DEFER_TAIL_REDUCE and ctx.needs_input_grad[0] and _tail_grads_adopted((w1, b1, w2, b2, wh, bh)))
        a.defer_reduce = 1 if ctx.deferred else 0
        a.loss_kind = int(kind)
        ctx.params = (w1, b1, w2, b2, wh, bh)
        ctx.dev = dev
        with torch.cuda.device(dev):
            ws = _tail_workspace(dev, int(lib.mkgnn_tail_workspace_bytes(K, H, G, n, seg.size)))
            if p_readout > 0.0:
                _lib.check(lib.mkgnn_tail_fused_readout_dropout(ctypes.byref(a), float(p_readout), ws.data_ptr(), ws.numel(),
                                                                _lib.stream_ptr(dev)), "mkgnn_tail_fused_readout_dropout")
            else:
                _lib.check(lib.mkgnn_tail_fused(ctypes.byref(a), ws.data_ptr(), ws.numel(), _lib.stream_ptr(dev)), "mkgnn_tail_fused")
        del keep
        if ctx.deferred:
            _TAIL_HELD.extend(t.untyped_storage() for t in (loss, gw1, gb1, gw2, gb2, gwh, gbh, rng, used, ws) if t is not None)
        ctx.unit = (gsim, gw1, gb1, gw2, gb2, gwh.reshape(wh.shape), gbh)
        ctx.pred, ctx.rng_used = pred, used
        return loss

    @staticmethod
    def backward(ctx, grad_loss):
        if ctx.unit is None:
            raise RuntimeError("the fused tail keeps its gradients for ONE backward (retain_graph is not supported: "
                               "MKGNN_FUSED_TAIL=0 runs the separate operators)")
        grads, ctx.unit = ctx.unit, None
        params, ctx.params = ctx.params, None
        if ctx.deferred and (not _is_unit_seed(grad_loss) or torch.is_grad_enabled()
                             or any(p is not None and p.grad is not None for p in params)):
            tail_flush(ctx.dev)
        if not _is_unit_seed(grad_loss):
            gl = grad_loss.reshape(()).float()
            grads = tuple(None if g is None else g * gl for g in grads)
        return (*grads, None, None, None, None, None, None, None, None)


def tail_loss(sim: torch.Tensor, plan, blocks, lin1: torch.nn.Linear, lin2: torch.nn.Linear, ffn: torch.nn.Linear,
              target: torch.Tensor, seg: "MoleculeSegments", dropout_p: float = 0.0, n_rows: Optional[int] = None,
              loss: str = "bce", readout_dropout_p: float = 0.0) -> torch.Tensor:
    kind = loss_kind(loss)
    n_rows = seg.size if n_rows is None else int(n_rows)
    if ffn.out_features != 1 or n_rows <= 0 or n_rows > seg.size or target.numel() != n_rows:
        raise ValueError("tail_loss needs a one-output linear layer and one target per (leading) molecule")
    if not 0.0 <= readout_dropout_p < 1.0:
        raise ValueError(f"readout dropout probability {readout_dropout_p} outside [0, 1)")
    return _TailFn.apply(sim, lin1.weight, lin1.bias, lin2.weight, lin2.bias, ffn.weight, ffn.bias, target, seg, plan,
                         tuple(blocks), float(dropout_p), n_rows, kind, float(readout_dropout_p))


_SCORE_TAIL = os.environ.get("MKGNN_SCORE_TAIL", "1") != "0"


def tail_score(sim: torch.Tensor, plan, blocks, lin1: torch.nn.Linear, lin2: torch.nn.Linear, ffn: torch.nn.Linear,
               seg: "MoleculeSegments", n_rows: Optional[int] = None) -> Tuple[torch.Tensor, torch.Tensor]:
    params = (lin1.weight, lin1.bias, lin2.weight, lin2.bias, ffn.weight, ffn.bias)
    if torch.is_grad_enabled() and any(t is not None and t.requires_grad for t in (sim, *params)):
        raise RuntimeError("tail_score is forward only: call it under torch.no_grad() (or on detached inputs); "
                           "tail_loss is the operator with gradients")
    lib = _lib.load()
    _lib.require_gpu_tensor(sim, "sim_sc")
    n_rows = seg.size if n_rows is None else int(n_rows)
    if ffn.out_features != 1 or n_rows <= 0 or n_rows > seg.size:
        raise ValueError("tail_score needs a one-output linear layer and 1 <= n_rows <= the batch's molecules")
    n, K = sim.shape
    dev = sim.device
    w1, b1, w2, b2, wh, bh = (None if t is None else t.detach() for t in params)
    w1c, w2c, whc = w1.contiguous(), w2.contiguous(), wh.reshape(-1).contiguous()
    H, G = w1c.shape[0], w2c.shape[0]
    pred = torch.empty(n_rows, dtype=torch.float32, device=dev)
    emb = torch.empty((seg.size, G), dtype=torch.float32, device=dev)
    a, keep = _tail_args(sim, plan, blocks, seg, n_rows, w1c, b1, w2c, b2, whc, bh)
    a.emb, a.emb_stride = emb.data_ptr(), G
    a.pred = pred.data_ptr()
    with torch.cuda.device(dev):
        ws = _tail_workspace(dev, int(lib.mkgnn_tail_score_workspace_bytes(K, H, G, n, seg.size)))
        _lib.check(lib.mkgnn_tail_score(ctypes.byref(a), ws.data_ptr(), ws.numel(), _lib.stream_ptr(dev)), "mkgnn_tail_score")
    del keep
    return pred, emb


_ATOM_CONTRIB = os.environ.get("MKGNN_ATOM_CONTRIB", "1") != "0"


def atom_contributions_reference(h, w1, b1, w2, b2, wh):
    import numpy as np

    def f64(a):
        return None if a is None else (a.detach().cpu().double().numpy() if torch.is_tensor(a) else np.asarray(a, dtype=np.float64))

    h, w1, b1, w2, b2, wh = (f64(a) for a in (h, w1, b1, w2, b2, wh))
    wh = wh.reshape(-1, w2.shape[0])
    if h.ndim != 2 or w1.ndim != 2 or w2.ndim != 2 or h.shape[1] != w1.shape[1] or w2.shape[1] != w1.shape[0]:
        raise ValueError("atom_contributions_reference needs h [N, K], W1 [H, K], W2 [G, H] and Wh [T, G]")
    pre = h @ w1.T
    if b1 is not None:
        pre = pre + b1
    with np.errstate(over="ignore"):
        act = pre / (1.0 + np.exp(-pre))
    emb = act @ w2.T
    if b2 is not None:
        emb = emb + b2
    return emb @ wh.T


def atom_contributions_supported(K: int, H: int, G: int, blocks, T: int) -> bool:
    return 1 <= int(T) <= _lib.ATOM_CONTRIB_MAX_TASKS and tail_supported(K, H, G, blocks)


def atom_contributions(sim: torch.Tensor, plan, blocks, lin1: torch.nn.Linear, lin2: torch.nn.Linear, ffn: torch.nn.Linear,
                       out: Optional[torch.Tensor] = None) -> torch.Tensor:
    params = (lin1.weight, lin1.bias, lin2.weight, lin2.bias, ffn.weight)
    if torch.is_grad_enabled() and any(t is not None and t.requires_grad for t in (sim, *params)):
        raise RuntimeError("atom_contributions is forward only: call it under torch.no_grad() (or on detached inputs)")
    lib = _lib.load()
    _lib.require_gpu_tensor(sim, "sim_sc")
    n, K = sim.shape
    dev = sim.device
    w1, b1, w2, b2, wh = (None if t is None else t.detach() for t in params)
    w1c, w2c = w1.contiguous(), w2.contiguous()
    whc = wh if wh.stride(1) == 1 else wh.contiguous()
    H, G, T = w1c.shape[0], w2c.shape[0], whc.shape[0]
    if whc.dim() != 2 or whc.shape[1] != G or not 1 <= T <= _lib.ATOM_CONTRIB_MAX_TASKS:
        raise ValueError(f"atom_contributions needs a head of 1 to {_lib.ATOM_CONTRIB_MAX_TASKS} outputs on the G = {G} embedding columns")
    if out is None:
        out = torch.empty((n, T), dtype=torch.float32, device=dev)
    elif (out.dtype != torch.float32 or out.device != dev or out.dim() != 2 or out.shape[0] != n or out.shape[1] < T
          or (n > 0 and out.stride(1) != 1)):
        raise ValueError(f"out: a float32 tensor [{n}, >= {T}] of rows on {dev}")
    if n == 0:
        return out[:, :T]
    a = _lib.AtomContribArgs()
    a.sim, a.sim_stride = sim.data_ptr(), _stride0(sim)
    for i, L in enumerate(blocks):
        a.num_kernels[i] = int(L)
    bk = _sel_buckets(plan)
    a.buckets = ctypes.cast(bk, ctypes.c_void_p)
    rin, cin = plan.csr_in
    a.in_rowptr, a.in_col, a.n_atoms = rin.data_ptr(), cin.data_ptr(), n
    a.readout = _params(w1c, b1, w2c, b2)
    a.head_weight, a.head_stride, a.T = whc.data_ptr(), (whc.stride(0) if T > 1 else G), T
    a.contrib, a.contrib_stride = out.data_ptr(), (out.stride(0) if n > 1 else out.shape[1])
    with torch.cuda.device(dev):
        ws = _tail_workspace(dev, int(lib.mkgnn_atom_contributions_workspace_bytes(K, H, G, n)))
        _lib.check(lib.mkgnn_atom_contributions(ctypes.byref(a), ws.data_ptr(), ws.numel(), _lib.stream_ptr(dev)),
                   "mkgnn_atom_contributions")
    del bk
    return out[:, :T]


def atom_contributions_torch(h: torch.Tensor, lin1: torch.nn.Linear, lin2: torch.nn.Linear, ffn: torch.nn.Linear) -> torch.Tensor:
    return torch.nn.functional.linear(lin2(swish(lin1(h))), ffn.weight)


def readout_dropout_mask(rng_pair: torch.Tensor, n_rows: int, H: int, p: float, out: Optional[torch.Tensor] = None) -> torch.Tensor:
    if not 0.0 <= p < 1.0:
        raise ValueError(f"readout dropout probability {p} outside [0, 1)")
    _lib.require_gpu_tensor(rng_pair, "rng_pair")
    if rng_pair.dtype != torch.int64 or rng_pair.numel() != 2 or not rng_pair.is_contiguous():
        raise ValueError("rng_pair: two contiguous int64 values {seed, offset}")
    dev = rng_pair.device
    if out is None:
        out = torch.empty((int(n_rows), int(H)), dtype=torch.float32, device=dev)
    if out.shape != (n_rows, H) or out.dtype != torch.float32 or out.stride(1) != 1 or out.device != dev:
        raise ValueError("out: [n_rows, H] float32 rows on the generator's device")
    lib = _lib.load()
    with torch.cuda.device(dev):
        _lib.check(lib.mkgnn_readout_dropout_mask(rng_pair.data_ptr(), int(n_rows), int(H), float(p), out.data_ptr(),
                                                  _stride0(out) if n_rows > 0 else int(H), _lib.stream_ptr(dev)),
                   "mkgnn_readout_dropout_mask")
    return out
```

Baseline: 5.999 million molecules/s.

## Fold deferred tail projection backward into the conv bank coefficient pre-pass

The tail's projection-backward kernel (dz times W1, producing grad_sim) can now be deferred when the only reader of sim is the last convolution. The convolution backward's coefficient pre-pass then recomputes the needed grad_sim values on the fly from dz and W1 in LDS instead of reading them from gout. The deferred projection still runs on the bank stream for the weight-gradient part, without writing dsim, in parallel with the pre-pass. This is meant to remove a full grad_sim write and read round trip and to overlap work. The cost is more global state, several eligibility checks, and redundant dot products inside the pre-pass.

```diff
diff --git a/include/molkgnn_hip.h b/include/molkgnn_hip.h
--- a/include/molkgnn_hip.h
+++ b/include/molkgnn_hip.h
@@ -190,6 +190,8 @@
 int mkgnn_readout_dropout_mask(const int64_t* rng_pair, int64_t n_rows, int32_t H, float p, float* keep, int64_t keep_stride,
                                void* stream);
 int mkgnn_tail_flush(void* stream);
+int mkgnn_tail_defer_projection(int32_t on);
+int mkgnn_debug_tail_projection_launches(int64_t out[3]);
 size_t mkgnn_tail_score_workspace_bytes(int32_t K, int32_t H, int32_t G, int64_t n_atoms, int64_t n_mols);
 int mkgnn_tail_score(const mkgnn_tail_args* args, void* workspace, size_t workspace_bytes, void* stream);
 
diff --git a/molkgnn_amd/_lib.py b/molkgnn_amd/_lib.py
--- a/molkgnn_amd/_lib.py
+++ b/molkgnn_amd/_lib.py
@@ -179,7 +179,8 @@
            "mkgnn_task_head_workspace_bytes", "mkgnn_task_head_forward", "mkgnn_task_head_backward", "mkgnn_task_head_fused",
            "mkgnn_task_scores", "mkgnn_topk_tasks_workspace_bytes", "mkgnn_topk_update_tasks", "mkgnn_embed_cosine",
            "mkgnn_atom_contributions", "mkgnn_atom_contributions_workspace_bytes", "mkgnn_embed_max_cosine",
-           "mkgnn_embed_max_cosine_workspace_bytes", "mkgnn_select_rows")
+           "mkgnn_embed_max_cosine_workspace_bytes", "mkgnn_select_rows", "mkgnn_tail_defer_projection",
+           "mkgnn_debug_tail_projection_launches")
 
 _lib: Optional[C.CDLL] = None
 TORCH_LIB_PATH = os.path.join(os.path.dirname(LIB_PATH), "libmolkgnn_torch.so")
@@ -257,6 +258,10 @@
     lib.mkgnn_flat_copy.argtypes = [C.c_void_p, C.c_int32, C.c_void_p]
     lib.mkgnn_tail_flush.restype = C.c_int
     lib.mkgnn_tail_flush.argtypes = [C.c_void_p]
+    lib.mkgnn_tail_defer_projection.restype = C.c_int
+    lib.mkgnn_tail_defer_projection.argtypes = [C.c_int32]
+    lib.mkgnn_debug_tail_projection_launches.restype = C.c_int
+    lib.mkgnn_debug_tail_projection_launches.argtypes = [C.POINTER(C.c_int64 * 3)]
     lib.mkgnn_rows_presplit.restype = C.c_int
     lib.mkgnn_rows_presplit.argtypes = [C.c_void_p, C.c_int64, C.c_int64, C.c_int32, C.c_void_p, C.c_void_p, C.c_int64, C.c_void_p]
     lib.mkgnn_rows_split_supported.restype = C.c_int
diff --git a/molkgnn_amd/csrc/kgnn_bwd_stream.hip b/molkgnn_amd/csrc/kgnn_bwd_stream.hip
--- a/molkgnn_amd/csrc/kgnn_bwd_stream.hip
+++ b/molkgnn_amd/csrc/kgnn_bwd_stream.hip
@@ -60,6 +60,13 @@
 template <int OFF> __device__ __forceinline__ void lds_read_h16(uint32_t& dst, uint32_t byte_addr) {
     static_assert(OFF >= 0 && OFF < 65536, "ds_read offset field");
     asm volatile("ds_read_u16 %0, %1 offset:%2" : "=v"(dst) : "v"(byte_addr), "n"(OFF) : "memory");
+}
+
+template <int OFF> __device__ __forceinline__ f32x4 lds_read_raw128_at(uint32_t byte_addr) {
+    static_assert(OFF >= 0 && OFF < 65536 && OFF % 16 == 0, "ds_read offset field");
+    f32x4 v;
+    asm volatile("ds_read_b128 %0, %1 offset:%2" : "=v"(v) : "v"(byte_addr), "n"(OFF) : "memory");
+    return v;
 }
 
 template <typename V> __device__ __forceinline__ void lds_fence(V& v) { asm volatile("s_waitcnt lgkmcnt(0)" : "+v"(v) : : "memory"); }
@@ -119,8 +126,11 @@
 #define MKGNN_PREP_RPB 4
 #endif
 constexpr int PREP_RPB = MKGNN_PREP_RPB;
-template <int NSRC, bool CH>
-__device__ __forceinline__ void coef_prepare_body(const BankStreamArgs& a, const int di) {
+constexpr int PJ_HP = 32, PJ_LZ = PJ_HP + 4, PJ_LMAX = 64;
+template <int NSRC, bool CH, bool PJ = false>
+__device__ __forceinline__ void coef_prepare_body(const BankStreamArgs& a, const int di, [[maybe_unused]] float* pj_w1 = nullptr,
+                                                  [[maybe_unused]] float* pj_dz = nullptr) {
+    static_assert(!PJ || NSRC == 1, "a projected source stands for the focal atom's row");
     const BankStreamDeg& g = a.deg[di];
     const int tid = threadIdx.x;
     const int64_t blk = (int64_t)blockIdx.x - g.prep_blk0;
@@ -147,6 +157,28 @@
 #pragma unroll
         for (int s = 0; s < NSRC; ++s) src[r][s] = a.through_nei ? g.nei[nc * D + s] : g.sel[nc];
     }
+    constexpr int PJ_NST = PJ ? (PREP_RPB * 128 + 255) / 256 : 1, PJ_NW = PJ ? PJ_HP * PJ_LMAX / 256 : 1;
+    [[maybe_unused]] f32x4 pj_st[PJ_NST];
+    [[maybe_unused]] float pj_wv[PJ_NW];
+    [[maybe_unused]] int pj_lc[PREP_RPB];
+    if constexpr (PJ) {
+#pragma unroll
+        for (int i = 0; i < PJ_NST; ++i) {
+            const int e = tid + 256 * i, r = (e >> 7) < PREP_RPB ? (e >> 7) : PREP_RPB - 1;
+            const int64_t rec = blk * PREP_RPB + r;
+            const int64_t rc = rec < nrec ? rec : nrec - 1;
+            const int64_t n = rc / g.nct * 16 + ((e >> 3) & 15);
+            const int64_t id = g.sel[n < g.n ? n : g.n - 1];
+            pj_st[i] = *(const f32x4*)(a.proj_dz + id * PJ_HP + 4 * (e & 7));
+        }
+#pragma unroll
+        for (int i = 0; i < PJ_NW; ++i) {
+            const int e = tid + 256 * i, ec = e < PJ_HP * g.L ? e : PJ_HP * g.L - 1;
+            const int h = ec / g.L, l = ec - h * g.L, hc = h < a.proj_H ? h : a.proj_H - 1;
+            const float w = a.proj_w1[(size_t)hc * a.proj_K + g.off + l];
+            pj_wv[i] = h < a.proj_H ? w : 0.f;
+        }
+    }
 #pragma unroll
     for (int r = 0; r < PREP_RPB; ++r) {
         const int64_t rec = blk * PREP_RPB + r;
@@ -157,16 +189,60 @@
         const int64_t nc = n < g.n ? n : g.n - 1;
         const int l = ct * g.kpt + k, lc = l < g.L ? l : g.L - 1;
         const size_t o = (size_t)nc * g.L + lc;
-        float gs4[NSRC];
-#pragma unroll
-        for (int s = 0; s < NSRC; ++s) gs4[s] = a.gout[src[r][s] * a.gs + g.off + lc];
-        gv[r] = gs4[0];
-#pragma unroll
-        for (int s = 1; s < NSRC; ++s) gv[r] += gs4[s];
+        if constexpr (PJ) pj_lc[r] = lc;
+        if constexpr (!PJ) {
+            float gs4[NSRC];
+#pragma unroll
+            for (int s = 0; s < NSRC; ++s) gs4[s] = a.gout[src[r][s] * a.gs + g.off + lc];
+            gv[r] = gs4[0];
+#pragma unroll
+            for (int s = 1; s < NSRC; ++s) gv[r] += gs4[s];
+        }
         const mkgnn_f32x4 pr = pair_load(g.pair, o);
         idx[r] = pair_index(pr);
         ch[r] = CH ? (int)chp[o] : 1;
         S[r] = pr[0]; C[r] = pr[1]; Ed[r] = pr[2];
+    }
+    if constexpr (PJ) {
+#pragma unroll
+        for (int i = 0; i < PJ_NST; ++i) {
+            const int e = tid + 256 * i;
+            if (e < PREP_RPB * 128) *(f32x4*)&pj_dz[(e >> 3) * PJ_LZ + 4 * (e & 7)] = pj_st[i];
+        }
+#pragma unroll
+        for (int i = 0; i < PJ_NW; ++i) {
+            const int e = tid + 256 * i;
+            if (e < PJ_HP * g.L) pj_w1[e / g.L * PJ_LMAX + e % g.L] = pj_wv[i];
+        }
+        __syncthreads();
+#pragma unroll
+        for (int r = 0; r < PREP_RPB; ++r) {
+            const uint32_t dz_b = (uint32_t)(uintptr_t)(pj_dz + (r * 16 + atom) * PJ_LZ);
+            const uint32_t w_b = (uint32_t)(uintptr_t)(pj_w1 + pj_lc[r]);
+            float acc = 0.f;
+            bs::static_for<0, PJ_HP / 16>([&](auto jhc) {
+                constexpr int jh = decltype(jhc)::value;
+                f32x4 d[4];
+                float w[16];
+                bs::static_for<0, 4>([&](auto qc) {
+                    constexpr int q = decltype(qc)::value;
+                    d[q] = bs::lds_read_raw128_at<4 * (16 * jh + 4 * q)>(dz_b);
+                });
+                bs::static_for<0, 16>([&](auto ic) {
+                    constexpr int i = decltype(ic)::value;
+                    w[i] = bs::lds_read_raw_at<4 * (16 * jh + i) * PJ_LMAX>(w_b);
+                });
+                asm volatile("s_waitcnt lgkmcnt(0)" : "+v"(d[0]), "+v"(d[1]), "+v"(d[2]), "+v"(d[3]), "+v"(w[0]), "+v"(w[1]), "+v"(w[2]),
+                             "+v"(w[3]), "+v"(w[4]), "+v"(w[5]), "+v"(w[6]), "+v"(w[7]), "+v"(w[8]), "+v"(w[9]), "+v"(w[10]), "+v"(w[11]),
+                             "+v"(w[12]), "+v"(w[13]), "+v"(w[14]), "+v"(w[15]) : : "memory");
+#pragma unroll
+                for (int c = 0; c < 4; ++c)
+#pragma unroll
+                    for (int q = 0; q < 4; ++q) acc = fmaf(d[q][c], w[4 * q + c], acc);
+                asm volatile("" : "+v"(acc) : : "memory");
+            });
+            gv[r] = acc;
+        }
     }
     float p0 = 0.f, p1 = 0.f, p2 = 0.f;
     constexpr int NEM = (PREP_RPB + 1) / 2;
@@ -242,6 +318,16 @@
         case 3: coef_prepare_body<3, false>(a, di); break;
         default: coef_prepare_body<4, false>(a, di); break;
     }
+}
+
+__global__ void __launch_bounds__(256) coef_prepare_proj_kernel(BankStreamArgs a) {
+    __shared__ __align__(16) float pj_w1[PJ_HP * PJ_LMAX];
+    __shared__ __align__(16) float pj_dz[PREP_RPB * 16 * PJ_LZ];
+    int di = 0;
+#pragma unroll
+    for (int k = 1; k < 4; ++k) if (a.deg[k].prep_blocks > 0 && (int)blockIdx.x >= a.deg[k].prep_blk0) di = k;
+    if (a.deg[di].chir) coef_prepare_body<1, true, true>(a, di, pj_w1, pj_dz);
+    else coef_prepare_body<1, false, true>(a, di, pj_w1, pj_dz);
 }
 
 constexpr int BANK_COEF_EXP = 18;
@@ -675,6 +761,7 @@
 }
 
 bool bank_stream_rows_split_supported(int F) { return (F + 15) / 16 <= 7 && bwd_split_mode() != 0; }
+bool bank_stream_projection_supported(int H, int HP, int L) { return HP == PJ_HP && H >= 1 && H <= PJ_HP && L >= 0 && L <= PJ_LMAX; }
 bool bank_stream_supported(int d, int F, int E, int L, int64_t n_atoms, int64_t x_stride, const float* e_unit) {
     return stream_forward_supported(d, F, E, L, n_atoms, x_stride, x_stride, e_unit);
 }
@@ -788,6 +875,13 @@
 
 hipError_t launch_coef_prepare(const BankStreamLaunch& p, hipStream_t st) {
     if (p.prep_blocks == 0) return hipSuccess;
+    if (p.a.proj_dz) {
+        if (p.a.through_nei || p.a.proj_HP != PJ_HP || p.a.proj_H < 1 || p.a.proj_H > PJ_HP) return hipErrorInvalidValue;
+        for (int i = 0; i < MKGNN_MAX_DEGREE; ++i) if (p.a.deg[i].prep_blocks > 0 && p.a.deg[i].L > PJ_LMAX) return hipErrorInvalidValue;
+        g_tail_projection_launches[0].fetch_add(1);
+        coef_prepare_proj_kernel<<<p.prep_blocks, 256, 0, st>>>(p.a);
+        return hipGetLastError();
+    }
     coef_prepare_kernel<<<p.prep_blocks, 256, 0, st>>>(p.a);
     return hipGetLastError();
 }
diff --git a/molkgnn_amd/csrc/kgnn_capi.hip b/molkgnn_amd/csrc/kgnn_capi.hip
--- a/molkgnn_amd/csrc/kgnn_capi.hip
+++ b/molkgnn_amd/csrc/kgnn_capi.hip
@@ -651,6 +651,22 @@
     ForkJoin fj;
     e = fj.begin(st, !g_time_bwd.load());
     if (e != hipSuccess) return api_hip_fail("stream fork", e);
+    TailProjection tp;
+    bool project = false;
+    if (pending_tail_projection(&tp)) {
+        project = grad_out == tp.dsim && grad_out_stride == tp.dss && streamed && rows_streamed && !through_nei && defer_bank && fj.p != nullptr &&
+                  any_bank && K == tp.K;
+        for (int i = 0; i < 4 && project; ++i) {
+            const bool same = L[i] == tp.L[i] && bank_a[i].off == tp.off[i] && buckets[i].count == tp.cnt[i] &&
+                              (tp.cnt[i] == 0 || buckets[i].selected_index == tp.sel[i]);
+            const bool wanted = tp.cnt[i] > 0 && tp.L[i] > 0;
+            project = same && (!wanted || bank_use[i]) && bank_stream_projection_supported(tp.H, tp.HP, L[i]);
+        }
+        if (!project) {
+            e = launch_pending_tail_projection(st, true);
+            if (e != hipSuccess) return api_hip_fail("deferred tail projection launch", e);
+        }
+    }
     bool bank_on_main = false;
     for (int i = 0; i < 4; ++i) {
         const int d = i + 1;
@@ -696,6 +712,13 @@
     if (streamed) {
         plan_backward_bank_stream(bank_a, bank_use, e_unit4, coefq4, nchunk4, ntheta4, through_nei, &bsl);
         bsl.x_split = rows_split ? 1 : 0;
+        if (project) { bsl.a.proj_dz = tp.dz; bsl.a.proj_w1 = tp.w1; bsl.a.proj_H = tp.H; bsl.a.proj_HP = tp.HP; bsl.a.proj_K = tp.K; }
+        if (project && switches().tail_project_in_prepass >= 2) {
+            e = fj.refork(1);
+            if (e != hipSuccess) return api_hip_fail("stream fork", e);
+            e = launch_pending_tail_projection(fj.p->aux[0], false);
+            if (e != hipSuccess) return api_hip_fail("deferred tail projection launch", e);
+        }
         { BwdTimer t(st, 0); e = launch_coef_prepare(bsl, st); }
         if (e != hipSuccess) return api_hip_fail("coefficient pre-pass launch", e);
         e = fj.refork(1);
@@ -709,6 +732,10 @@
     if (any_bank) {
         hipStream_t st_bank = fj.stream(1, &e);
         if (e != hipSuccess) return api_hip_fail("stream fork", e);
+        if (project) {
+            e = launch_pending_tail_projection(st_bank, false);
+            if (e != hipSuccess) return api_hip_fail("deferred tail projection launch", e);
+        }
         if (st_bank != st) {
             e = launch_pending_tail_reduce(st_bank);
             if (e != hipSuccess) return api_hip_fail("deferred tail reduction launch", e);
diff --git a/molkgnn_amd/csrc/kgnn_launch.h b/molkgnn_amd/csrc/kgnn_launch.h
--- a/molkgnn_amd/csrc/kgnn_launch.h
+++ b/molkgnn_amd/csrc/kgnn_launch.h
@@ -148,6 +148,7 @@
 int bank_blocks_for(int d, int64_t n);
 hipError_t launch_backward_bank_fused(const BwdArgs a4[4], const bool use[4], int nchunk_out[4], int ntheta_out[4], hipStream_t st);
 bool bank_stream_supported(int d, int F, int E, int L, int64_t n_atoms, int64_t x_stride, const float* e_unit);
+bool bank_stream_projection_supported(int H, int HP, int L);
 bool bank_stream_rows_split_supported(int F);
 struct BankStreamDeg {
     const int64_t* sel; const int64_t* nei; const float* e_unit;
@@ -172,6 +173,8 @@
     uint16_t grp_count[FUSED_MAX_GROUPS];
     uint8_t blk_group[FUSED_MAX_BLOCKS];
     uint16_t blk_rank[FUSED_MAX_BLOCKS];
+    const float* proj_dz; const float* proj_w1;
+    int proj_H, proj_HP, proj_K;
 };
 
 struct TailMidArgs {
@@ -192,6 +195,16 @@
 constexpr int TAIL_B1 = 0, TAIL_W2 = 32, TAIL_B2 = 32 + 1024, TAIL_WH = TAIL_B2 + 32, TAIL_BH = TAIL_WH + 32, TAIL_LOSS = TAIL_BH + 1,
               TAIL_SLAB = (TAIL_LOSS + 1 + 3) / 4 * 4;
 hipError_t launch_pending_tail_reduce(hipStream_t st, bool* launched = nullptr);
+struct TailProjection {
+    const float* dsim; int64_t dss;
+    const float* dz; const float* w1;
+    int H, HP, K;
+    int off[MKGNN_MAX_DEGREE], L[MKGNN_MAX_DEGREE];
+    const int64_t* sel[MKGNN_MAX_DEGREE]; int64_t cnt[MKGNN_MAX_DEGREE];
+};
+bool pending_tail_projection(TailProjection* out);
+hipError_t launch_pending_tail_projection(hipStream_t st, bool full);
+extern std::atomic<long long> g_tail_projection_launches[3];
 int tail_group_size(int64_t n_loss_mols);
 int tail_middle_blocks(int64_t n_loss_mols);
 hipError_t launch_tail_middle(const TailMidArgs& a, int nb, int loss_kind, hipStream_t st);
diff --git a/molkgnn_amd/csrc/kgnn_readout.hip b/molkgnn_amd/csrc/kgnn_readout.hip
--- a/molkgnn_amd/csrc/kgnn_readout.hip
+++ b/molkgnn_amd/csrc/kgnn_readout.hip
@@ -992,6 +992,29 @@
     return e == hipSuccess ? 0 : api_hip_fail(who, e);
 }
 
+struct PendingProject { BlockProjArgs b; int tpw; int64_t nb; size_t lds; bool on; };
+static PendingProject g_pending_project_dev[16];
+static bool g_defer_projection_dev[16];
+static int pending_device() {
+    int dev = 0;
+    if (hipGetDevice(&dev) != hipSuccess || dev < 0 || dev >= 16) dev = 0;
+    return dev;
+}
+static int64_t project_bwd_blocks(const BlockProjArgs& b, int* tpw_out, int64_t nb_of[MKGNN_MAX_DEGREE]) {
+    int64_t tiles_all = 0;
+    for (int i = 0; i < MKGNN_MAX_DEGREE; ++i) if (b.L[i] > 0) tiles_all += (b.cnt[i] + 15) / 16;
+    int tpw = (int)((tiles_all + 4 * (2 * RO_ATOM_BLOCKS - 4) - 1) / (4 * (2 * RO_ATOM_BLOCKS - 4)));
+    if (tpw < 1) tpw = 1;
+    int64_t nb = 0;
+    for (int i = 0; i < MKGNN_MAX_DEGREE; ++i) {
+        const int64_t tiles = (b.cnt[i] + 15) / 16, per = 4 * (int64_t)tpw;
+        nb_of[i] = b.L[i] > 0 ? (tiles + per - 1) / per : 0;
+        nb += nb_of[i];
+    }
+    *tpw_out = tpw;
+    return nb;
+}
+
 struct TailWs { size_t z, dz, slab_atoms, slab_tail, total; int slab_atoms_stride; };
 static TailWs tail_ws(const ReadoutDims& d, int64_t n_atoms, int64_t n_mols) {
     TailWs w;
@@ -1023,7 +1046,8 @@
     int64_t n_focal = 0;
     if (int rc = check_blocks(who, ro, num_kernels, buckets, n_atoms, sim_stride, sim, b, d, &n_focal)) return rc;
     if (!ws || ws_bytes < total) return api_fail("%s: workspace too small (%zu < %zu)", who, ws_bytes, total);
-    hipError_t e = launch_pending_tail_reduce(st);
+    hipError_t e = launch_pending_tail_projection(st, true);
+    if (e == hipSuccess) e = launch_pending_tail_reduce(st);
     if (e == hipSuccess) e = project_blocks(b, d, n_focal, sim, sim_stride, n_atoms, (float*)ws, st);
     return e == hipSuccess ? 0 : api_hip_fail(who, e);
 }
@@ -1078,23 +1102,24 @@
     e = launch_tail_middle(m, nbm, p->loss_kind, st);
     if (e != hipSuccess) return api_hip_fail(who, e);
     b.dz = dz; b.dsim = p->grad_sim; b.dss = p->grad_sim_stride;
-    int64_t tiles_all = 0;
-    for (int i = 0; i < MKGNN_MAX_DEGREE; ++i) if (b.L[i] > 0) tiles_all += (b.cnt[i] + 15) / 16;
-    int tpw = (int)((tiles_all + 4 * (2 * RO_ATOM_BLOCKS - 4) - 1) / (4 * (2 * RO_ATOM_BLOCKS - 4)));
-    if (tpw < 1) tpw = 1;
-    int64_t nb_of[MKGNN_MAX_DEGREE], nb = 0;
-    for (int i = 0; i < MKGNN_MAX_DEGREE; ++i) {
-        const int64_t tiles = (b.cnt[i] + 15) / 16, per = 4 * (int64_t)tpw;
-        nb_of[i] = b.L[i] > 0 ? (tiles + per - 1) / per : 0;
-        nb += nb_of[i];
-    }
+    int tpw = 1;
+    int64_t nb_of[MKGNN_MAX_DEGREE];
+    const int64_t nb = project_bwd_blocks(b, &tpw, nb_of);
     if (nb > 2 * RO_ATOM_BLOCKS) return api_fail("%s: internal: %lld blocks for %d slabs", who, (long long)nb, 2 * RO_ATOM_BLOCKS);
     float* const slab_atoms = (float*)((char*)ws + w.slab_atoms);
     b.slab = slab_atoms; b.slab_stride = w.slab_atoms_stride;
-    if (nb > 0) {
-        const size_t img = (size_t)4 * (16 * (d.HP + 4) + 16 * 68);
-        const size_t lds = ((size_t)d.HP * 68 + (img > 4096 ? img : 4096)) * 4;
-        block_project_bwd_mfma_kernel<2><<<(unsigned)nb, 256, lds, st>>>(b, tpw);
+    const size_t proj_img = (size_t)4 * (16 * (d.HP + 4) + 16 * 68);
+    const size_t proj_lds = ((size_t)d.HP * 68 + (proj_img > 4096 ? proj_img : 4096)) * 4;
+    bool defer_proj = false;
+    {
+        std::lock_guard<std::mutex> lock(g_pending_reduce_mutex);
+        bool& want = g_defer_projection_dev[pending_device()];
+        defer_proj = want && p->defer_reduce && nb > 0 && switches().tail_project_in_prepass != 0;
+        want = false;
+    }
+    if (nb > 0 && !defer_proj) {
+        g_tail_projection_launches[1].fetch_add(1);
+        block_project_bwd_mfma_kernel<2><<<(unsigned)nb, 256, proj_lds, st>>>(b, tpw);
     }
     SlabReduceArgs r{};
     int blk = 0;
@@ -1133,11 +1158,31 @@
         std::lock_guard<std::mutex> lock(g_pending_reduce_mutex);
         PendingReduce* slot = pending_reduce_slot();
         slot->r = r; slot->blk = blk;
+        if (defer_proj) {
+            PendingProject& pp = g_pending_project_dev[pending_device()];
+            pp.b = b; pp.tpw = tpw; pp.nb = nb; pp.lds = proj_lds; pp.on = true;
+        }
         return 0;
+    }
+    if (defer_proj) {
+        g_tail_projection_launches[1].fetch_add(1);
+        block_project_bwd_mfma_kernel<2><<<(unsigned)nb, 256, proj_lds, st>>>(b, tpw);
     }
     if (blk > 0) slab_reduce_kernel<<<blk, 256, 0, st>>>(r);
     e = hipGetLastError();
     return e == hipSuccess ? 0 : api_hip_fail(who, e);
+}
+
+int mkgnn_tail_defer_projection(int32_t on) {
+    std::lock_guard<std::mutex> lock(g_pending_reduce_mutex);
+    g_defer_projection_dev[pending_device()] = on != 0;
+    return 0;
+}
+
+int mkgnn_debug_tail_projection_launches(int64_t out[3]) {
+    if (!out) return api_fail("mkgnn_debug_tail_projection_launches: null pointer");
+    for (int i = 0; i < 3; ++i) out[i] = (int64_t)g_tail_projection_launches[i].load();
+    return 0;
 }
 
 int mkgnn_tail_fused(const mkgnn_tail_args* p, void* ws, size_t ws_bytes, void* stream) {
@@ -1251,11 +1296,36 @@
     if (launched) *launched = true;
     return hipGetLastError();
 }
+
+std::atomic<long long> g_tail_projection_launches[3];
+
+bool pending_tail_projection(TailProjection* out) {
+    std::lock_guard<std::mutex> lock(g_pending_reduce_mutex);
+    const PendingProject& pp = g_pending_project_dev[pending_device()];
+    if (!pp.on) return false;
+    const BlockProjArgs& b = pp.b;
+    out->dsim = b.dsim; out->dss = b.dss; out->dz = b.dz; out->w1 = b.w1; out->H = b.H; out->HP = b.HP; out->K = b.K;
+    for (int i = 0; i < MKGNN_MAX_DEGREE; ++i) { out->off[i] = b.off[i]; out->L[i] = b.L[i]; out->sel[i] = b.sel[i]; out->cnt[i] = b.cnt[i]; }
+    return true;
+}
+
+hipError_t launch_pending_tail_projection(hipStream_t st, bool full) {
+    std::lock_guard<std::mutex> lock(g_pending_reduce_mutex);
+    PendingProject& pp = g_pending_project_dev[pending_device()];
+    if (!pp.on) return hipSuccess;
+    pp.on = false;
+    BlockProjArgs b = pp.b;
+    if (!full) b.dsim = nullptr;
+    g_tail_projection_launches[full ? 1 : 2].fetch_add(1);
+    block_project_bwd_mfma_kernel<2><<<(unsigned)pp.nb, 256, pp.lds, st>>>(b, pp.tpw);
+    return hipGetLastError();
+}
 }
 }
 
 extern "C" int mkgnn_tail_flush(void* stream) {
-    const hipError_t e = launch_pending_tail_reduce((hipStream_t)stream);
+    hipError_t e = launch_pending_tail_projection((hipStream_t)stream, true);
+    if (e == hipSuccess) e = launch_pending_tail_reduce((hipStream_t)stream);
     return e == hipSuccess ? 0 : api_hip_fail("mkgnn_tail_flush", e);
 }
 
diff --git a/molkgnn_amd/csrc/kgnn_switches.h b/molkgnn_amd/csrc/kgnn_switches.h
--- a/molkgnn_amd/csrc/kgnn_switches.h
+++ b/molkgnn_amd/csrc/kgnn_switches.h
@@ -28,6 +28,7 @@
     bool fwd_stream;
     bool bf16_stream;
     bool rows_split;
+    int tail_project_in_prepass;
     bool bn_one_launch;
     char helper_priority;
     int fwd_pp;
@@ -54,7 +55,7 @@
         s.serial = is_set("MKGNN_SERIAL"); s.fork_in_graph = is_set("MKGNN_FORK_IN_GRAPH"); s.no_mfma_bwd = is_set("MKGNN_NO_MFMA_BWD");
         s.fork_mode = not_0("MKGNN_FORK_MODE"); s.bank_fused = not_0("MKGNN_BANK_FUSED"); s.rows_stream = not_0("MKGNN_ROWS_STREAM");
         s.bank_stream = not_0("MKGNN_BANK_STREAM"); s.fwd_stream = not_0("MKGNN_FWD_STREAM"); s.bf16_stream = not_0("MKGNN_BF16_STREAM");
-        s.rows_split = not_0("MKGNN_ROWS_SPLIT");
+        s.rows_split = not_0("MKGNN_ROWS_SPLIT"); s.tail_project_in_prepass = number("MKGNN_TAIL_PROJECT_IN_PREPASS", 2);
         if (const char* e = getenv("MKGNN_BN_ONE_LAUNCH")) s.bn_one_launch = e[0] == '1';
         if (const char* e = getenv("MKGNN_HELPER_PRIORITY")) s.helper_priority = e[0];
         s.fwd_pp = number("MKGNN_FWD_PP", MKGNN_FWD_PP_DEFAULT); s.fwd_pp_env = number("MKGNN_FWD_PP", 0) != 0;
diff --git a/molkgnn_amd/readout.py b/molkgnn_amd/readout.py
--- a/molkgnn_amd/readout.py
+++ b/molkgnn_amd/readout.py
@@ -946,6 +946,7 @@
 
 
 _DEFER_TAIL_REDUCE = False
+_TAIL_PROJECT_NEXT = False
 _TAIL_HELD: list = []
 
 
@@ -1003,6 +1004,8 @@
 
     @staticmethod
     def forward(ctx, sim, w1, b1, w2, b2, wh, bh, target, seg, plan, blocks, p_drop, n_rows, kind=_lib.LOSS_BCE_MEAN, p_readout=0.0):
+        global _TAIL_PROJECT_NEXT
+        project, _TAIL_PROJECT_NEXT = _TAIL_PROJECT_NEXT, False
         lib = _lib.load()
         _lib.require_gpu_tensor(sim, "sim_sc")
         n, K = sim.shape
@@ -1040,6 +1043,8 @@
         ctx.dev = dev
         with torch.cuda.device(dev):
             ws = _tail_workspace(dev, int(lib.mkgnn_tail_workspace_bytes(K, H, G, n, seg.size)))
+            if ctx.deferred and project:
+                _lib.check(lib.mkgnn_tail_defer_projection(1), "mkgnn_tail_defer_projection")
             if p_readout > 0.0:
                 _lib.check(lib.mkgnn_tail_fused_readout_dropout(ctypes.byref(a), float(p_readout), ws.data_ptr(), ws.numel(),
                                                                 _lib.stream_ptr(dev)), "mkgnn_tail_fused_readout_dropout")
@@ -1047,7 +1052,8 @@
                 _lib.check(lib.mkgnn_tail_fused(ctypes.byref(a), ws.data_ptr(), ws.numel(), _lib.stream_ptr(dev)), "mkgnn_tail_fused")
         del keep
         if ctx.deferred:
-            _TAIL_HELD.extend(t.untyped_storage() for t in (loss, gw1, gb1, gw2, gb2, gwh, gbh, rng, used, ws) if t is not None)
+            _TAIL_HELD.extend(t.untyped_storage() for t in (loss, gw1, gb1, gw2, gb2, gwh, gbh, rng, used, ws, gsim, sim, w1c)
+                              if t is not None)
         ctx.unit = (gsim, gw1, gb1, gw2, gb2, gwh.reshape(wh.shape), gbh)
         ctx.pred, ctx.rng_used = pred, used
         return loss
@@ -1068,6 +1074,12 @@
         return (*grads, None, None, None, None, None, None, None, None)
 
 
+def _sole_reader_is_the_convolution(sim: torch.Tensor) -> bool:
+    fn = sim.grad_fn
+    return (fn is not None and type(fn).__name__ == "_KernelSetConvFnBackward" and not sim._backward_hooks
+            and not getattr(sim, "retains_grad", False))
+
+
 def tail_loss(sim: torch.Tensor, plan, blocks, lin1: torch.nn.Linear, lin2: torch.nn.Linear, ffn: torch.nn.Linear,
               target: torch.Tensor, seg: "MoleculeSegments", dropout_p: float = 0.0, n_rows: Optional[int] = None,
               loss: str = "bce", readout_dropout_p: float = 0.0) -> torch.Tensor:
@@ -1077,8 +1089,13 @@
         raise ValueError("tail_loss needs a one-output linear layer and one target per (leading) molecule")
     if not 0.0 <= readout_dropout_p < 1.0:
         raise ValueError(f"readout dropout probability {readout_dropout_p} outside [0, 1)")
-    return _TailFn.apply(sim, lin1.weight, lin1.bias, lin2.weight, lin2.bias, ffn.weight, ffn.bias, target, seg, plan,
-                         tuple(blocks), float(dropout_p), n_rows, kind, float(readout_dropout_p))
+    global _TAIL_PROJECT_NEXT
+    _TAIL_PROJECT_NEXT = bool(_DEFER_TAIL_REDUCE and _sole_reader_is_the_convolution(sim))
+    try:
+        return _TailFn.apply(sim, lin1.weight, lin1.bias, lin2.weight, lin2.bias, ffn.weight, ffn.bias, target, seg, plan,
+                             tuple(blocks), float(dropout_p), n_rows, kind, float(readout_dropout_p))
+    finally:
+        _TAIL_PROJECT_NEXT = False
 
 
 _SCORE_TAIL = os.environ.get("MKGNN_SCORE_TAIL", "1") != "0"
```

Measured after the change: 6.109 million molecules/s, median of 6. 1.8% higher.
